# tum-vision/mem

Measured on AMD Instinct MI355X. Metric: pretrain samples/sec (ViT-B, 224^2 event voxels), higher is better.
Workload: dtype bf16

## Files before the change

include/memhip.h:

```cpp
#ifndef MEMHIP_H
#define MEMHIP_H

#include <stddef.h>
#include <stdint.h>

#ifdef __cplusplus
extern "C" {
#endif

#define MEMHIP_ABI_VERSION 10

#define MEMHIP_OK 0
#define MEMHIP_EINVAL (-1)
#define MEMHIP_EWORKSPACE (-2)
#define MEMHIP_ELAUNCH (-3)
#define MEMHIP_EUNSUPPORTED (-4)

typedef void* memhip_stream_t;

int memhip_abi_version(void);
const char* memhip_last_error(void);
const char* memhip_arch(void);
const char* memhip_build_flags(void);
int memhip_set_option(const char* name, int value);
// ... 175 lines not shown
typedef struct memhip_tn_problem {
  const void* A; int64_t lda;
  const void* B; int64_t ldb;
  float* out; int64_t ldo;
  int32_t R, N, K;
  int32_t reserved0;
} memhip_tn_problem_t;
size_t memhip_gemm_bf16_tn_group_workspace(const memhip_tn_problem_t* problems, int count);
int memhip_gemm_bf16_tn_group(const memhip_tn_problem_t* problems, int count, int accumulate, void* workspace,
                              size_t workspace_bytes, memhip_stream_t stream);

#define MEMHIP_TN_128 0
#define MEMHIP_TN_P8_ATOMIC 1
#define MEMHIP_TN_P8_WS 2
#define MEMHIP_TN_P8_GROUP 3
typedef struct memhip_tn_part {
  int32_t problem;
  int32_t tiles, splits, rows_per_split;
  int32_t wg_begin, quad_begin;
  int64_t ws_offset;
} memhip_tn_part_t;
typedef struct memhip_tn_launch {
  int32_t kind;
  int32_t count;
  int32_t grid, reduce_grid;
  int32_t memset_first;
  int32_t use_atomics;
  int64_t ws_bytes;
  memhip_tn_part_t p[4];
} memhip_tn_launch_t;
typedef struct memhip_tn_plan { int32_t count; int32_t reserved0; memhip_tn_launch_t l[4]; } memhip_tn_plan_t;
int memhip_gemm_bf16_tn_plan(const memhip_tn_problem_t* problems, int count, int accumulate, const void* workspace,
                             size_t workspace_bytes, int stream_cus, memhip_tn_plan_t* out_plan);
size_t memhip_gemm_bf16_tn_plan_workspace(const memhip_tn_problem_t* problems, int count, int device_cus);
int memhip_colsum_bf16(const void* in, int64_t ld, int R, int C, float* out, memhip_stream_t stream);
int memhip_colsum_fold(float* ws, int copies, int N, float* out, memhip_stream_t stream);

int memhip_residual_rows(const float* x, int64_t ldx, const int32_t* rows, const void* y, int64_t ldy, const float* gamma,
                         const float* rowkeep, float keep_prob, int R, int D, float* out, int64_t ldo,
                         memhip_stream_t stream);
int memhip_scatter_rows_f32(const float* src, int64_t lds, const int32_t* rows, int R, int D, float* dst, int64_t ldd,
                            memhip_stream_t stream);

int memhip_layernorm_fwd(const float* x, int64_t ldx, const int32_t* row_idx, int R, int D,
                         const float* gamma, const float* beta, float eps, void* y_bf16, int64_t ldy,
                         float* mean, float* rstd, memhip_stream_t stream);
int memhip_layernorm_bwd(const void* dy_bf16, int64_t lddy, const float* x, int64_t ldx,
                         const int32_t* row_idx, int R, int D, const float* gamma, const float* mean,
                         const float* rstd, float* dres, int64_t lddres, int accumulate, float* dgamma,
                         float* dbeta, memhip_stream_t stream);

int memhip_layerscale_grad(const void* W_bf16, int64_t ldw, const float* dW, int64_t lddw, const float* bias,
                           const float* dbias, const float* gamma, int N, int K, float* dgamma,
                           memhip_stream_t stream);

typedef struct memhip_branch {
  const void* y; int64_t ldy;
  const float* gamma;
  const float* rowmask;
  float keep_prob;
  int32_t rows_per_sample;
  void* dy; int64_t lddy;
  float* dgamma; float* dbias;
  const int32_t* out_map;
  const memhip_dropout_t* dropout;
} memhip_branch_t;
typedef struct memhip_branch_bwd_args {
  const float* dx; int64_t lddx;
  int32_t M, D;
  memhip_branch_t branch;
} memhip_branch_bwd_args_t;
int memhip_branch_bwd(const memhip_branch_bwd_args_t* args, memhip_stream_t stream);
typedef struct memhip_ln_bwd_branch_args {
  const void* dy; int64_t lddy;
  const float* x; int64_t ldx;
  int32_t R, D;
  const float* gamma; const float* mean; const float* rstd;
  float* dres; int64_t lddres;
  float* dgamma; float* dbeta;
  const int32_t* in_map;
  memhip_branch_t branch;
} memhip_ln_bwd_branch_args_t;
int memhip_layernorm_bwd_branch(const memhip_ln_bwd_branch_args_t* args, memhip_stream_t stream);

int memhip_embed_bwd(const float* dx, int64_t lddx, const uint8_t* mask, int B, int L, int D,
                     void* dy_bf16, int64_t lddy, float* dcls, float* dmask_token, memhip_stream_t stream);

int memhip_cross_entropy(void* logits_bf16, int64_t ld, const int64_t* labels, int M, int V,
                         float grad_scale, float* row_loss, int32_t* row_correct, int write_grad,
                         float* out2, memhip_stream_t stream);

int memhip_attn_tokens_padded(int T);
int memhip_relpos_gather(const float* table, const int32_t* index , int T, int TP, int heads,
                         float* bias_pad, float* biasT_pad ,
                         memhip_stream_t stream);
int memhip_attn_fwd(const void* qkv, int64_t ldqkv, int B, int T, int D, int heads, const float* table,
                    int window_h, int window_w, void* out, int64_t ldo, float* lse, memhip_stream_t stream);
int memhip_attn_delta(const void* dout, const void* out, int64_t ldo, int64_t rows, int heads, float* delta,
                      memhip_stream_t stream);
typedef struct memhip_attn_bwd_args {
  const void* qkv; int64_t ldqkv;
  const void* dout; int64_t ldo;
  const void* out; int64_t ldout;
  const float* lse;
  float* delta;
  const float* table;
  int32_t window_h, window_w, B, T, D, heads;
  float scale;
  int32_t reserved0;
  void* dqkv; int64_t lddqkv;
  float* dtable; float* dq_bias; float* dv_bias;
  void* ws; int64_t ws_bytes;
} memhip_attn_bwd_args_t;
int memhip_attn_bwd(const memhip_attn_bwd_args_t* args, memhip_stream_t stream);
int64_t memhip_attn_bwd_workspace(int B, int T, int heads, int window_h, int window_w);

#define MEMHIP_ATTN_16 1
#define MEMHIP_ATTN_SMALL 2
#define MEMHIP_ATTN_WIN 3
#define MEMHIP_ATTN_WIN_DS 4
#define MEMHIP_ATTN_STREAM 5
enum { MEMHIP_ATTN_K_STATS_ZERO, MEMHIP_ATTN_K_DELTA, MEMHIP_ATTN_K_FWD, MEMHIP_ATTN_K_BWD_KV, MEMHIP_ATTN_K_BWD_Q,
       MEMHIP_ATTN_K_FWD16, MEMHIP_ATTN_K_BWD16,
       MEMHIP_ATTN_K_WIN_STATS, MEMHIP_ATTN_K_FWD_WIN, MEMHIP_ATTN_K_BWD_KV_WIN, MEMHIP_ATTN_K_BWD_Q_WIN,
       MEMHIP_ATTN_K_BWD_KVS_WIN, MEMHIP_ATTN_K_BWD_QS_WIN,
       MEMHIP_ATTN_K_FWD_STREAM, MEMHIP_ATTN_K_BWD_KV_STREAM, MEMHIP_ATTN_K_BWD_Q_STREAM };
typedef struct memhip_attn_launch {
  int32_t kernel;
  int32_t grid_x, grid_y, grid_z;
  int32_t block;
  int32_t lds;
} memhip_attn_launch_t;
typedef struct memhip_attn_plan {
  int32_t family;
  int32_t n;
  int32_t ww;
  int32_t vb, dt, fd;
  int32_t spb;
  int32_t nwg;
  int32_t groups;
  int32_t nbz, nbq, nbs;
  int32_t qgroups, qs;
  int32_t stream_spb;
  int32_t lds_over;
  int32_t count;
  memhip_attn_launch_t l[5];
} memhip_attn_plan_t;
int memhip_attn_plan_fwd(int B, int T, int D, int heads, int window_h, int window_w, int stream_cus, memhip_attn_plan_t* out);
int memhip_attn_plan_bwd(int B, int T, int D, int heads, int window_h, int window_w, int has_dtable, int has_dv_bias,
                         int has_out, const void* ws, int64_t ws_bytes, int stream_cus, memhip_attn_plan_t* out);

int memhip_f32_gemm_nt(const memhip_gemm_args_t* args, memhip_stream_t stream);
int memhip_f32_transpose(const float* in, int64_t ldin, int R, int C, float* out, int64_t ldout, memhip_stream_t stream);
int memhip_f32_layernorm_fwd(const float* x, int64_t ldx, const int32_t* row_idx, int R, int D, const float* gamma,
                             const float* beta, float eps, float* y, int64_t ldy, float* mean, float* rstd,
                             memhip_stream_t stream);
int memhip_f32_layernorm_bwd(const float* dy, int64_t lddy, const float* x, int64_t ldx, const int32_t* row_idx, int R, int D,
                             const float* gamma, const float* mean, const float* rstd, float* dres, int64_t lddres,
                             int accumulate, float* dgamma, float* dbeta, memhip_stream_t stream);
int memhip_f32_branch_bwd(const float* dx, int64_t lddx, const float* y, int64_t ldy, const float* gamma, const float* rowmask,
                          float keep_prob, int rows_per_sample, int M, int D, float* dy, int64_t lddy, float* dgamma,
                          float* dbias, memhip_stream_t stream);
int memhip_f32_embed_bwd(const float* dx, int64_t lddx, const uint8_t* mask, int B, int L, int D, float* dy, int64_t lddy,
                         float* dcls, float* dmask_token, memhip_stream_t stream);
int memhip_f32_cross_entropy(float* logits, int64_t ld, const int64_t* labels, int M, int V, float grad_scale,
                             float* row_loss, int32_t* row_correct, int write_grad, float* out2, memhip_stream_t stream);
// ... 141 lines not shown
```

mem_amd/csrc/common.h:

```cpp
#pragma once
#include <hip/hip_runtime.h>
#include <cstdarg>
#include <cstdio>
#include <cstdint>
#include <type_traits>
#include "../../include/memhip.h"

namespace memhip {

extern thread_local char g_err[512];

inline int fail(int code, const char* fmt, ...) {
  va_list ap;
  va_start(ap, fmt);
  vsnprintf(g_err, sizeof(g_err), fmt, ap);
  va_end(ap);
  return code;
}

inline int check_launch(const char* what) {
  hipError_t e = hipGetLastError();
  if (e != hipSuccess) return fail(MEMHIP_ELAUNCH, "%s: %s", what, hipGetErrorString(e));
  return MEMHIP_OK;
}

enum { OPT_GEMM_P8, OPT_GEMM256, OPT_GEMM_SPLIT, OPT_GEMM_P8_HALF, OPT_GEMM_P8_MIN_N, OPT_GEMM256_MIN_N, OPT_TN_P8,
       OPT_RASTER_LDS, OPT_ATTN16, OPT_ATTN16_STAGGER, OPT_ATTN16_STAGGER_FWD, OPT_GEMM_STAGGER, OPT_GEMM_PREFETCH, OPT_RESERVE_CUS, OPT_LN_BWD_GRID, OPT_ATTN_WIN, OPT_GEMM_P8_PAIR, OPT_TN_GROUP, OPT_CONV_WAVES, OPT_RASTER_BANDS, OPT_COUNT_ };
int opt(int id);
int usable_cus(hipStream_t s = nullptr);
int max_cus();

inline hipStream_t as_stream(memhip_stream_t s) { return reinterpret_cast<hipStream_t>(s); }

inline int cdiv(long long a, long long b) { return (int)((a + b - 1) / b); }

template <typename F>
int dispatch_bool(bool b, F&& f) { return b ? f(std::true_type{}) : f(std::false_type{}); }

}

#define MEMHIP_REQUIRE(cond, ...) \
  do { if (!(cond)) return memhip::fail(MEMHIP_EINVAL, __VA_ARGS__); } while (0)
#define MEMHIP_HIP(call) \
  do { hipError_t e_ = (call); if (e_ != hipSuccess) \
    return memhip::fail(MEMHIP_ELAUNCH, "%s: %s", #call, hipGetErrorString(e_)); } while (0)
```

mem_amd/csrc/core.cpp:

```cpp
#include "common.h"
#include <atomic>
#include <mutex>
#include <cstring>

namespace memhip {
thread_local char g_err[512] = "";

static std::atomic<int> g_opt[OPT_COUNT_] = {
     {1},  {1},  {1},  {1},  {512},
     {1024},  {1},  {1},  {1},  {40000},  {0},  {0},  {0},
     {0},  {2048},
     {1},
     {1},
     {1},
     {16},
     {0}};
static const char* const g_opt_name[OPT_COUNT_] = {"gemm_p8", "gemm256", "gemm_split", "gemm_p8_half", "gemm_p8_min_n",
                                                   "gemm256_min_n", "tn_p8", "raster_lds", "attn16", "attn16_stagger", "attn16_stagger_fwd", "gemm_stagger", "gemm_prefetch", "reserve_cus", "ln_bwd_grid", "attn_win", "gemm_p8_pair", "tn_group", "conv_waves", "raster_bands"};
int opt(int id) { return g_opt[id].load(std::memory_order_relaxed); }

struct StreamReserve { std::atomic<bool> used{false}; std::atomic<void*> stream{nullptr}; std::atomic<int> cus{0}; };
static StreamReserve g_reserve[32];
static int stream_reserved(hipStream_t s) {
  for (auto& r : g_reserve)
    if (r.used.load(std::memory_order_acquire) && r.stream.load(std::memory_order_relaxed) == (void*)s)
      return r.cus.load(std::memory_order_relaxed);
  return 0;
}

static int device_cu_count() {
  static std::atomic<int> device_cus{0};
  int n = device_cus.load(std::memory_order_relaxed);
  if (!n) {
    int dev = 0;
    hipDeviceProp_t prop;
    if (hipGetDevice(&dev) != hipSuccess || hipGetDeviceProperties(&prop, dev) != hipSuccess) return 0;
    n = prop.multiProcessorCount > 0 ? prop.multiProcessorCount : 256;
    device_cus.store(n, std::memory_order_relaxed);
  }
  return n;
}

int max_cus() { return device_cu_count(); }

int usable_cus(hipStream_t s) {
  const int n = device_cu_count();
  if (!n) return 0;
  int r = opt(OPT_RESERVE_CUS);
  const int rs = stream_reserved(s);
  r = r > rs ? r : rs;
  r = r < 0 ? 0 : (r + 7) / 8 * 8;
  return n - r >= 8 ? n - r : (n >= 8 ? 8 : n);
}
}

extern "C" {
int memhip_abi_version(void) { return MEMHIP_ABI_VERSION; }
const char* memhip_last_error(void) { return memhip::g_err; }
const char* memhip_arch(void) { return "gfx950"; }
#ifndef MEMHIP_BUILD_FLAGS
#define MEMHIP_BUILD_FLAGS ""
#endif
const char* memhip_build_flags(void) { return MEMHIP_BUILD_FLAGS; }

int memhip_stream_reserve_cus(memhip_stream_t stream, int cus) {
  MEMHIP_REQUIRE(cus >= 0, "stream_reserve_cus: negative count");
  using memhip::g_reserve;
  static std::mutex mu;
  std::lock_guard<std::mutex> lock(mu);
  for (auto& r : g_reserve)
    if (r.used.load(std::memory_order_relaxed) && r.stream.load(std::memory_order_relaxed) == stream) {
      r.cus.store(cus, std::memory_order_relaxed);
      if (cus == 0) r.used.store(false, std::memory_order_release);
      return MEMHIP_OK;
    }
  if (cus == 0) return MEMHIP_OK;
  for (auto& r : g_reserve)
    if (!r.used.load(std::memory_order_relaxed)) {
      r.stream.store(stream, std::memory_order_relaxed);
      r.cus.store(cus, std::memory_order_relaxed);
      r.used.store(true, std::memory_order_release);
      return MEMHIP_OK;
    }
  return memhip::fail(MEMHIP_EINVAL, "stream_reserve_cus: more than 32 streams carry a reservation");
}

int memhip_set_option(const char* name, int value) {
  MEMHIP_REQUIRE(name, "set_option: null name");
  for (int i = 0; i < memhip::OPT_COUNT_; ++i)
    if (!strcmp(name, memhip::g_opt_name[i])) {
      if (i == memhip::OPT_LN_BWD_GRID && value < 1)
        return memhip::fail(MEMHIP_EINVAL, "set_option: ln_bwd_grid=%d must be at least 1", value);
      memhip::g_opt[i].store(value, std::memory_order_relaxed);
      return MEMHIP_OK;
    }
  return memhip::fail(MEMHIP_EINVAL, "set_option: unknown option '%s'", name);
}

int memhip_get_option(const char* name, int* value) {
  MEMHIP_REQUIRE(name && value, "get_option: null argument");
  for (int i = 0; i < memhip::OPT_COUNT_; ++i)
// ... 8 lines not shown
```

mem_amd/csrc/gemm_tn.hip:

```cpp
#include "common.h"
#include "gemm_tn_plan.hpp"

namespace {

using namespace memhip;

constexpr int BM = kTn128Tile, BN = kTn128Tile, BR = kTnStageRows;
constexpr int kThreads = 256;
constexpr int kTileBytes = BR * 128 * 2;
constexpr int kStageBytes = 2 * kTileBytes;

typedef __attribute__((ext_vector_type(8))) __bf16 bf16x8;
typedef __attribute__((ext_vector_type(4))) __bf16 bf16x4;
typedef __attribute__((ext_vector_type(4))) short s16x4;
typedef __attribute__((ext_vector_type(4))) float f32x4;

__device__ __attribute__((aligned(256))) unsigned char g_zero_page[256];

__device__ __forceinline__ void glds16(const void* gsrc, void* lds_dst) {
  __builtin_amdgcn_global_load_lds((const __attribute__((address_space(1))) void*)gsrc,
                                   (__attribute__((address_space(3))) void*)lds_dst, 16, 0, 0);
}

__device__ __forceinline__ void stage_rows(const __bf16* __restrict__ src, long long ld, int row0, int rows_valid,
                                           int col0, int cols_valid, char* lds_tile, int wave, int lane) {
#pragma unroll
  for (int j = 0; j < 4; ++j) {
    const int inst = wave * 4 + j;
    const int r = inst * 4 + (lane >> 4);
    const int cpos = lane & 15;
    const int chunk = (((cpos >> 1) ^ (r & 7)) << 1) | (cpos & 1);
    const int grow = row0 + r, gcol = col0 + chunk * 8;
    const void* g = (grow < rows_valid && gcol < cols_valid)
                        ? (const void*)(src + (long long)grow * ld + gcol)
                        : (const void*)(g_zero_page + cpos * 16);
    glds16(g, lds_tile + inst * 1024);
  }
}

__device__ __forceinline__ bf16x8 read_frag_tr(const char* tile, int ks, int col0, int lane) {
  const int g = lane >> 4, q = (lane >> 2) & 3, p = lane & 3;
  const int colb = col0 + 4 * p;
  const int seg = colb >> 4, inb = (colb & 15) * 2;
  const int r0 = ks * 32 + 4 * g + q, r1 = r0 + 16;
  const char* a0 = tile + r0 * 256 + ((seg ^ (r0 & 7)) << 5) + inb;
  const char* a1 = tile + r1 * 256 + ((seg ^ (r1 & 7)) << 5) + inb;
  const s16x4 lo = __builtin_amdgcn_ds_read_tr16_b64_v4i16((__attribute__((address_space(3))) s16x4*)a0);
  const s16x4 hi = __builtin_amdgcn_ds_read_tr16_b64_v4i16((__attribute__((address_space(3))) s16x4*)a1);
  union { struct { s16x4 l, h; } s; bf16x8 v; } u;
  u.s.l = lo;
  u.s.h = hi;
  return u.v;
}

__global__ __launch_bounds__(kThreads, 2) void gemm_tn_kernel(const __bf16* __restrict__ A, long long lda,
                                                              const __bf16* __restrict__ B, long long ldb,
                                                              int R, int N, int K, float* __restrict__ out,
                                                              long long ldo, int splits, int rows_per_split,
                                                              int use_atomics) {
  extern __shared__ __attribute__((aligned(16))) char smem[];
  const int lane = threadIdx.x & 63;
  const int wave = __builtin_amdgcn_readfirstlane(threadIdx.x >> 6);
  const int wr = wave >> 1, wc = wave & 1;
  const int ntk = (K + BN - 1) / BN;
  const int tiles = ((N + BM - 1) / BM) * ntk;
  const int tile = blockIdx.x % tiles, sp = blockIdx.x / tiles;
  const int n0 = (tile / ntk) * BM, k0 = (tile % ntk) * BN;
  const int rbeg = sp * rows_per_split;
  int rend = rbeg + rows_per_split;
  rend = rend < R ? rend : R;
  if (rbeg >= rend) return;
  const int nst = (rend - rbeg + BR - 1) / BR;

  f32x4 acc[4][4];
#pragma unroll
  for (int i = 0; i < 4; ++i)
#pragma unroll
    for (int j = 0; j < 4; ++j) acc[i][j] = f32x4{0.f, 0.f, 0.f, 0.f};

  stage_rows(A, lda, rbeg, rend, n0, N, smem, wave, lane);
  stage_rows(B, ldb, rbeg, rend, k0, K, smem + kTileBytes, wave, lane);
  __syncthreads();
  int cur = 0;
// ... 101 lines not shown
    attr_done = true;
  }
  hipLaunchKernelGGL(gemm_tn_kernel, dim3(l.grid), dim3(kThreads), 2 * kStageBytes, s, (const __bf16*)q.A, (long long)q.lda,
                     (const __bf16*)q.B, (long long)q.ldb, q.R, q.N, q.K, q.out, (long long)q.ldo, l.p[0].splits,
                     l.p[0].rows_per_split, l.use_atomics);
  return check_launch("gemm_bf16_tn");
}

TnPlan plan_now(const memhip_tn_problem_t* pr, int count, int accumulate, const void* ws, size_t ws_bytes, int stream_cus) {
  const TnWorkspace w = {ws != nullptr, ((uintptr_t)ws & 15) == 0, ws_bytes};
  return tn_plan(pr, count, accumulate, w, stream_cus, TnOptions{opt(OPT_TN_P8), opt(OPT_TN_GROUP)});
}

int run(const memhip_tn_problem_t* pr, int count, int accumulate, void* ws, size_t ws_bytes, hipStream_t s) {
  const TnPlan plan = plan_now(pr, count, accumulate, ws, ws_bytes, usable_cus(s));
  for (int i = 0; i < plan.count; ++i) {
    const TnLaunch& l = plan.l[i];
    const memhip_tn_problem_t& q = pr[l.p[0].problem];
    int rc = MEMHIP_OK;
    switch (l.kind) {
      case MEMHIP_TN_128: rc = tn_128_launch(l, q, s); break;
      case MEMHIP_TN_P8_ATOMIC: rc = tn_p8_launch_atomic(l, q, s); break;
      case MEMHIP_TN_P8_WS: rc = tn_p8_launch_ws(l, q, accumulate, (float*)ws, s); break;
      case MEMHIP_TN_P8_GROUP: rc = tn_p8_launch_group(l, pr, accumulate, (float*)ws, s); break;
    }
    if (rc != MEMHIP_OK) return rc;
  }
  return MEMHIP_OK;
}

int validate_group(const memhip_tn_problem_t* problems, int count) {
  MEMHIP_REQUIRE(problems && count >= 1 && count <= kTnGroupMax, "gemm_tn_group: 1..4 problems, got %d", count);
  for (int i = 0; i < count; ++i) {
    const memhip_tn_problem_t& q = problems[i];
    MEMHIP_REQUIRE(q.R >= 0 && q.N > 0 && q.K > 0, "gemm_tn_group[%d]: bad shape R=%d N=%d K=%d", i, q.R, q.N, q.K);
    MEMHIP_REQUIRE(q.R == 0 || (q.A && q.B && q.out), "gemm_tn_group[%d]: null pointer", i);
    MEMHIP_REQUIRE(q.N % 8 == 0 && q.K % 8 == 0 && q.lda % 8 == 0 && q.ldb % 8 == 0 && ((uintptr_t)q.A & 15) == 0 &&
                       ((uintptr_t)q.B & 15) == 0, "gemm_tn_group[%d]: operands must be 16-byte aligned, N/K/ld %% 8 == 0", i);
  }
  return MEMHIP_OK;
}

}

extern "C" size_t memhip_gemm_bf16_tn_workspace(int R, int N, int K) { return tn_workspace_bytes(R, N, K, max_cus()); }

extern "C" int memhip_gemm_bf16_tn(const void* A, int64_t lda, const void* B, int64_t ldb, int R, int N, int K,
                                   float* out, int64_t ldo, int accumulate, void* workspace,
                                   size_t workspace_bytes, memhip_stream_t stream) {
  MEMHIP_REQUIRE(R >= 0 && N > 0 && K > 0, "gemm_tn: bad shape R=%d N=%d K=%d", R, N, K);
  if (R == 0) return MEMHIP_OK;
  MEMHIP_REQUIRE(A && B && out, "gemm_tn: null pointer");
  MEMHIP_REQUIRE(N % 8 == 0 && K % 8 == 0 && lda % 8 == 0 && ldb % 8 == 0 && ((uintptr_t)A & 15) == 0 &&
                     ((uintptr_t)B & 15) == 0, "gemm_tn: operands must be 16-byte aligned, N/K/ld %% 8 == 0");
  const memhip_tn_problem_t q = {A, lda, B, ldb, out, ldo, R, N, K, 0};
  return run(&q, 1, accumulate, workspace, workspace_bytes, as_stream(stream));
}

extern "C" size_t memhip_gemm_bf16_tn_group_workspace(const memhip_tn_problem_t* problems, int count) {
  return memhip_gemm_bf16_tn_plan_workspace(problems, count, max_cus());
}

extern "C" int memhip_gemm_bf16_tn_group(const memhip_tn_problem_t* problems, int count, int accumulate, void* workspace,
                                         size_t workspace_bytes, memhip_stream_t stream) {
  if (const int rc = validate_group(problems, count)) return rc;
  return run(problems, count, accumulate, workspace, workspace_bytes, as_stream(stream));
}

extern "C" int memhip_gemm_bf16_tn_plan(const memhip_tn_problem_t* problems, int count, int accumulate, const void* workspace,
                                        size_t workspace_bytes, int stream_cus, memhip_tn_plan_t* out_plan) {
  MEMHIP_REQUIRE(out_plan, "gemm_tn plan: bad arguments");
  if (const int rc = validate_group(problems, count)) return rc;
  *out_plan = plan_now(problems, count, accumulate, workspace, workspace_bytes, stream_cus >= 0 ? stream_cus : usable_cus());
  return MEMHIP_OK;
}

extern "C" size_t memhip_gemm_bf16_tn_plan_workspace(const memhip_tn_problem_t* problems, int count, int device_cus) {
  if (!problems || count <= 0) return 0;
  return tn_group_workspace_bytes(problems, count, device_cus);
}

namespace {
__global__ __launch_bounds__(256) void colsum_fold_kernel(float* __restrict__ ws, int copies, int N, float* __restrict__ out) {
  const int n = blockIdx.x * 256 + threadIdx.x;
  if (n >= N) return;
  float s = 0.f;
  for (int k = 0; k < copies; ++k) {
    s += ws[(long long)k * N + n];
    ws[(long long)k * N + n] = 0.f;
  }
  out[n] += s;
}
}

extern "C" int memhip_colsum_fold(float* ws, int copies, int N, float* out, memhip_stream_t stream) {
  MEMHIP_REQUIRE(copies >= 1 && N > 0, "colsum_fold: bad shape");
  MEMHIP_REQUIRE(ws && out, "colsum_fold: null pointer");
  hipLaunchKernelGGL(colsum_fold_kernel, dim3(cdiv(N, 256)), dim3(256), 0, as_stream(stream), ws, copies, N, out);
  return check_launch("colsum_fold");
}

extern "C" int memhip_colsum_bf16(const void* in, int64_t ld, int R, int Cc, float* out, memhip_stream_t stream) {
  MEMHIP_REQUIRE(R >= 0 && Cc > 0 && Cc % 8 == 0 && ld % 8 == 0, "colsum: bad shape");
  if (R == 0) return MEMHIP_OK;
  MEMHIP_REQUIRE(in && out, "colsum: null pointer");
  const int chunks = Cc / 8;
  const int tpr = chunks >= 256 ? 256 : chunks;
  const int gx = cdiv(chunks, tpr);
  int gy = 256 / gx;
  if (gy > 128) gy = 128;
  if (gy < 1) gy = 1;
  int rows_per_block = cdiv(R, gy);
  if (rows_per_block < 64) rows_per_block = 64;
  hipLaunchKernelGGL(colsum_kernel, dim3(gx, cdiv(R, rows_per_block)), dim3(256), 0, as_stream(stream),
                     (const __bf16*)in, (long long)ld, R, Cc, rows_per_block, tpr, out);
  return check_launch("colsum_bf16");
}
```

mem_amd/csrc/misc.hip:

```cpp
#include "common.h"

namespace {

using namespace memhip;

typedef __attribute__((ext_vector_type(4))) __bf16 bf16x4;
typedef __attribute__((ext_vector_type(8))) __bf16 bf16x8;

__global__ __launch_bounds__(256) void cast_kernel(const float* __restrict__ in, __bf16* __restrict__ out,
                                                   long long n4) {
  for (long long i = (long long)blockIdx.x * 256 + threadIdx.x; i < n4; i += (long long)gridDim.x * 256) {
    const float4 v = reinterpret_cast<const float4*>(in)[i];
    bf16x4 o;
    o[0] = (__bf16)v.x; o[1] = (__bf16)v.y; o[2] = (__bf16)v.z; o[3] = (__bf16)v.w;
    reinterpret_cast<bf16x4*>(out)[i] = o;
  }
}

template <typename IN>
__global__ __launch_bounds__(256) void transpose_kernel(const IN* __restrict__ in, long long ldin, int R,
                                                        int Cc, __bf16* __restrict__ out, long long ldout,
                                                        int R_pad, float* __restrict__ cs0, int c0b, int c0e,
                                                        float* __restrict__ cs1, int c1b, int c1e) {
  __shared__ __bf16 tile[64][66];
  const int r0 = blockIdx.x * 64, c0 = blockIdx.y * 64;
  const int t = threadIdx.x;
#pragma unroll
  for (int pass = 0; pass < 2; ++pass) {
    const int rl = (t >> 3) + pass * 32, cl = (t & 7) * 8;
    const int r = r0 + rl;
#pragma unroll
    for (int k = 0; k < 8; ++k) {
      const int c = c0 + cl + k;
      __bf16 v = (__bf16)0.f;
      if (r < R && c < Cc) v = (__bf16)(float)in[(long long)r * ldin + c];
      tile[rl][cl + k] = v;
    }
  }
  __syncthreads();
#pragma unroll
  for (int pass = 0; pass < 2; ++pass) {
    const int cl = (t >> 3) + pass * 32, rl = (t & 7) * 8;
    const int c = c0 + cl;
    bf16x8 o;
    float s = 0.f;
#pragma unroll
    for (int k = 0; k < 8; ++k) { o[k] = tile[rl + k][cl]; s += (float)o[k]; }
    if (c < Cc && r0 + rl < R_pad)
      *reinterpret_cast<bf16x8*>(out + (long long)c * ldout + r0 + rl) = o;
    if (cs0 || cs1) {
      s += __shfl_xor(s, 1); s += __shfl_xor(s, 2); s += __shfl_xor(s, 4);
      if ((t & 7) == 0 && c < Cc) {
        if (cs0 && c >= c0b && c < c0e) atomicAdd(cs0 + (c - c0b), s);
        if (cs1 && c >= c1b && c < c1e) atomicAdd(cs1 + (c - c1b), s);
      }
    }
  }
}

struct TransposeDesc { const float* in; long long ldin; long long R; long long Cc; __bf16* out; long long ldout; };
__global__ __launch_bounds__(256) void transpose_cast_batched_kernel(const TransposeDesc* __restrict__ desc,
                                                                     const int* __restrict__ tile_prefix, int n) {
  __shared__ __bf16 tile[64][66];
  int mi = 0;
  while (mi + 1 < n && (int)blockIdx.x >= tile_prefix[mi + 1]) ++mi;
  const TransposeDesc d = desc[mi];
  const int local = blockIdx.x - tile_prefix[mi];
  const int R = (int)d.R, Cc = (int)d.Cc;
  const int tr = (R + 63) / 64;
  const int r0 = (local % tr) * 64, c0 = (local / tr) * 64;
  const int t = threadIdx.x;
  const int R_pad = (int)(d.ldout < (long long)tr * 64 ? d.ldout : (long long)tr * 64);
#pragma unroll
  for (int pass = 0; pass < 2; ++pass) {
    const int rl = (t >> 3) + pass * 32, cl = (t & 7) * 8;
    const int r = r0 + rl, c = c0 + cl;
    const float* src = d.in + (long long)r * d.ldin + c;
    if (r < R && c + 8 <= Cc && ((d.ldin & 3) == 0) && (((unsigned long long)d.in & 15) == 0)) {
      const float4 a = reinterpret_cast<const float4*>(src)[0], b = reinterpret_cast<const float4*>(src)[1];
      const float v[8] = {a.x, a.y, a.z, a.w, b.x, b.y, b.z, b.w};
#pragma unroll
      for (int k = 0; k < 8; ++k) tile[rl][cl + k] = (__bf16)v[k];
    } else {
#pragma unroll
      for (int k = 0; k < 8; ++k) tile[rl][cl + k] = (r < R && c + k < Cc) ? (__bf16)src[k] : (__bf16)0.f;
    }
  }
  __syncthreads();
#pragma unroll
  for (int pass = 0; pass < 2; ++pass) {
    const int cl = (t >> 3) + pass * 32, rl = (t & 7) * 8;
    const int c = c0 + cl;
    bf16x8 o;
#pragma unroll
    for (int k = 0; k < 8; ++k) o[k] = tile[rl + k][cl];
    if (c < Cc && r0 + rl < R_pad) *reinterpret_cast<bf16x8*>(d.out + (long long)c * d.ldout + r0 + rl) = o;
  }
}

__global__ __launch_bounds__(256) void im2col_kernel(const float* __restrict__ x, int B, int C, int H, int W,
                                                     int ph, int pw, __bf16* __restrict__ out) {
  const int gw = W / pw, gh = H / ph;
  const int K = C * ph * pw, K8 = K >> 3;
  const long long total = (long long)B * gh * gw * K8;
  for (long long i = (long long)blockIdx.x * 256 + threadIdx.x; i < total; i += (long long)gridDim.x * 256) {
    const int k8 = (int)(i % K8);
    const long long row = i / K8;
    const int k = k8 * 8;
    const int c = k / (ph * pw), rem = k - c * ph * pw, py = rem / pw, px = rem - py * pw;
    const int gx = (int)(row % gw);
    const long long t = row / gw;
    const int gy = (int)(t % gh), b = (int)(t / gh);
    const float* src = x + (((long long)b * C + c) * H + gy * ph + py) * W + gx * pw + px;
    const float4 a = reinterpret_cast<const float4*>(src)[0], d = reinterpret_cast<const float4*>(src)[1];
    bf16x8 o;
    o[0] = (__bf16)a.x; o[1] = (__bf16)a.y; o[2] = (__bf16)a.z; o[3] = (__bf16)a.w;
    o[4] = (__bf16)d.x; o[5] = (__bf16)d.y; o[6] = (__bf16)d.z; o[7] = (__bf16)d.w;
    reinterpret_cast<bf16x8*>(out)[i] = o;
  }
}

__global__ __launch_bounds__(256) void fill_cls_kernel(float* __restrict__ x, long long ldx, int B, int T, int D,
                                                       const float* __restrict__ cls) {
  const int b = blockIdx.x;
  for (int c = threadIdx.x; c < D; c += 256) x[(long long)b * T * ldx + c] = cls[c];
}

__global__ __launch_bounds__(256) void relpos_gather_kernel(const float* __restrict__ table,
                                                            const int* __restrict__ idx, int T, int TP, int Hh,
                                                            float* __restrict__ bias, float* __restrict__ biasT) {
  const long long total = (long long)Hh * TP * TP;
  for (long long i = (long long)blockIdx.x * 256 + threadIdx.x; i < total; i += (long long)gridDim.x * 256) {
    const int k = (int)(i % TP);
    const long long t = i / TP;
    const int q = (int)(t % TP), h = (int)(t / TP);
    float v = 0.f;
    if (q < T && k < T) v = table[(long long)idx[q * T + k] * Hh + h];
    bias[i] = v;
    if (biasT) biasT[((long long)h * TP + k) * TP + q] = v;
  }
}


__global__ __launch_bounds__(256) void gemv_acc_kernel(const __bf16* __restrict__ W, long long ldw, int N, int K,
                                                       const float* __restrict__ x, float* __restrict__ y,
                                                       float* __restrict__ x_acc, float* __restrict__ zero) {
  const int lane = threadIdx.x & 63;
  const int n = blockIdx.x * 4 + (threadIdx.x >> 6);
  if (n < N) {
    float s = 0.f;
    for (int k = lane * 8; k < K; k += 512) {
      const bf16x8 w = *reinterpret_cast<const bf16x8*>(W + (long long)n * ldw + k);
      const float4 a = *reinterpret_cast<const float4*>(x + k), b = *reinterpret_cast<const float4*>(x + k + 4);
      s += (float)w[0] * a.x + (float)w[1] * a.y + (float)w[2] * a.z + (float)w[3] * a.w + (float)w[4] * b.x +
           (float)w[5] * b.y + (float)w[6] * b.z + (float)w[7] * b.w;
    }
    for (int o = 32; o > 0; o >>= 1) s += __shfl_xor(s, o);
    if (lane == 0) y[n] += s;
  }
  if (blockIdx.x == 0) {
    for (int k = threadIdx.x; k < K; k += blockDim.x) {
      if (x_acc) x_acc[k] += x[k];
      if (zero) zero[k] = 0.f;
    }
  }
}

}

extern "C" int memhip_cast_f32_bf16(const float* in, void* out, int64_t n, memhip_stream_t stream) {
  MEMHIP_REQUIRE(n >= 0 && n % 4 == 0, "cast: n must be a multiple of 4");
  if (n == 0) return MEMHIP_OK;
  MEMHIP_REQUIRE(in && out, "cast: null pointer");
  const long long n4 = n / 4;
  int blocks = (int)((n4 + 255) / 256);
  if (blocks > 4096) blocks = 4096;
  hipLaunchKernelGGL(cast_kernel, dim3(blocks), dim3(256), 0, as_stream(stream), in, (__bf16*)out, n4);
  return check_launch("cast_f32_bf16");
}

extern "C" int memhip_transpose_cast_f32_bf16(const float* in, int64_t ldin, int R, int Cc, void* out,
                                              int64_t ldout, memhip_stream_t stream) {
  MEMHIP_REQUIRE(R > 0 && Cc > 0 && in && out, "transpose_cast: bad arguments");
  MEMHIP_REQUIRE(ldout % 8 == 0 && ldout >= R, "transpose_cast: ldout");
  const int R_pad = (int)(ldout < (int64_t)cdiv(R, 64) * 64 ? ldout : (int64_t)cdiv(R, 64) * 64);
  hipLaunchKernelGGL(transpose_kernel<float>, dim3(cdiv(R, 64), cdiv(Cc, 64)), dim3(256), 0, as_stream(stream), in,
                     (long long)ldin, R, Cc, (__bf16*)out, (long long)ldout, R_pad, (float*)nullptr, 0, 0,
                     (float*)nullptr, 0, 0);
  return check_launch("transpose_cast");
}

extern "C" int memhip_transpose_cast_batched(const void* desc, const int32_t* tile_prefix, int n, int total_tiles,
                                             memhip_stream_t stream) {
  MEMHIP_REQUIRE(n >= 0 && total_tiles >= 0, "transpose_cast_batched: bad arguments");
  if (n == 0 || total_tiles == 0) return MEMHIP_OK;
  MEMHIP_REQUIRE(desc && tile_prefix, "transpose_cast_batched: null pointer");
  static_assert(sizeof(TransposeDesc) == 48, "descriptor = 6 x 8 bytes");
  hipLaunchKernelGGL(transpose_cast_batched_kernel, dim3(total_tiles), dim3(256), 0, as_stream(stream),
                     (const TransposeDesc*)desc, tile_prefix, n);
  return check_launch("transpose_cast_batched");
}

extern "C" int memhip_transpose_bf16(const void* in, int64_t ldin, int R, int Cc, void* out, int64_t ldout,
                                     int R_pad, float* colsum0, int c0_begin, int c0_end, float* colsum1,
                                     int c1_begin, int c1_end, memhip_stream_t stream) {
  MEMHIP_REQUIRE(R >= 0 && Cc > 0 && in && out, "transpose: bad arguments");
  MEMHIP_REQUIRE(R_pad >= R && R_pad % 64 == 0 && ldout >= R_pad && ldout % 8 == 0,
                 "transpose: R_pad=%d must be a multiple of 64 and <= ldout", R_pad);
  if (R_pad == 0) return MEMHIP_OK;
  hipLaunchKernelGGL(transpose_kernel<__bf16>, dim3(R_pad / 64, cdiv(Cc, 64)), dim3(256), 0, as_stream(stream),
                     (const __bf16*)in, (long long)ldin, R, Cc, (__bf16*)out, (long long)ldout, R_pad, colsum0,
                     c0_begin, c0_end, colsum1, c1_begin, c1_end);
  return check_launch("transpose_bf16");
}

extern "C" int memhip_im2col_bf16(const float* x, int B, int C, int H, int W, int ph, int pw, void* out,
                                  memhip_stream_t stream) {
  MEMHIP_REQUIRE(B >= 0 && C > 0 && ph > 0 && pw > 0 && H % ph == 0 && W % pw == 0, "im2col: bad shape");
  MEMHIP_REQUIRE(pw % 8 == 0 && W % 4 == 0, "im2col: patch width must be a multiple of 8");
  if (B == 0) return MEMHIP_OK;
  MEMHIP_REQUIRE(x && out, "im2col: null pointer");
  const long long total = (long long)B * (H / ph) * (W / pw) * (C * ph * pw / 8);
  int blocks = (int)((total + 255) / 256);
  if (blocks > 8192) blocks = 8192;
  hipLaunchKernelGGL(im2col_kernel, dim3(blocks), dim3(256), 0, as_stream(stream), x, B, C, H, W, ph, pw,
                     (__bf16*)out);
  return check_launch("im2col");
}

__global__ __launch_bounds__(256) void copy_samples_kernel(const float* __restrict__ src, float* __restrict__ dst,
                                                           const int* __restrict__ ids, long long n_per_sample) {
  const long long base = (long long)ids[blockIdx.y] * n_per_sample;
  const float4* s4 = reinterpret_cast<const float4*>(src + base);
  float4* d4 = reinterpret_cast<float4*>(dst + base);
  for (long long i = (long long)blockIdx.x * 256 + threadIdx.x; i < n_per_sample / 4; i += (long long)gridDim.x * 256) d4[i] = s4[i];
}

extern "C" int memhip_copy_samples_f32(const float* src, float* dst, const int32_t* ids, int n, int64_t n_per_sample,
                                       memhip_stream_t stream) {
  MEMHIP_REQUIRE(n >= 0 && n_per_sample > 0 && n_per_sample % 4 == 0, "copy_samples: bad shape");
  if (n == 0) return MEMHIP_OK;
  MEMHIP_REQUIRE(src && dst && ids, "copy_samples: null pointer");
  int gx = (int)((n_per_sample / 4 + 255) / 256);
  if (gx > 64) gx = 64;
  hipLaunchKernelGGL(copy_samples_kernel, dim3(gx, n), dim3(256), 0, as_stream(stream), src, dst, (const int*)ids,
                     (long long)n_per_sample);
  return check_launch("copy_samples");
}

__global__ __launch_bounds__(256) void zero_kernel(uint4* __restrict__ p, long long n16) {
  const long long step = (long long)gridDim.x * 256;
  for (long long i = (long long)blockIdx.x * 256 + threadIdx.x; i < n16; i += step) p[i] = uint4{0u, 0u, 0u, 0u};
}
__global__ __launch_bounds__(256) void zero_ranges_kernel(char* __restrict__ base, const long long* __restrict__ ranges, int n) {
  const long long step = (long long)gridDim.x * 256;
  for (int r = 0; r < n; ++r) {
    uint4* p = reinterpret_cast<uint4*>(base + ranges[2 * r]);
    const long long n16 = ranges[2 * r + 1] >> 4;
    for (long long i = (long long)blockIdx.x * 256 + threadIdx.x; i < n16; i += step) p[i] = uint4{0u, 0u, 0u, 0u};
  }
}

extern "C" int memhip_zero(void* p, int64_t bytes, memhip_stream_t stream) {
  MEMHIP_REQUIRE(bytes >= 0 && bytes % 16 == 0 && ((uintptr_t)p & 15) == 0, "zero: pointer and size must be multiples of 16 bytes");
  if (bytes == 0) return MEMHIP_OK;
  MEMHIP_REQUIRE(p, "zero: null pointer");
  long long g = (bytes / 16 + 255) / 256;
  if (g > 2048) g = 2048;
  hipLaunchKernelGGL(zero_kernel, dim3((unsigned)g), dim3(256), 0, as_stream(stream), (uint4*)p, (long long)(bytes / 16));
  return check_launch("zero");
}

extern "C" int memhip_zero_ranges(void* base, const int64_t* ranges, int n, int64_t total_bytes, memhip_stream_t stream) {
  MEMHIP_REQUIRE(n >= 0 && total_bytes >= 0, "zero_ranges: bad count");
  if (n == 0 || total_bytes == 0) return MEMHIP_OK;
  MEMHIP_REQUIRE(base && ranges && ((uintptr_t)base & 15) == 0, "zero_ranges: null / unaligned pointer");
  long long g = (total_bytes / 16 + 255) / 256;
  if (g > 1024) g = 1024;
  if (g < 1) g = 1;
  hipLaunchKernelGGL(zero_ranges_kernel, dim3((unsigned)g), dim3(256), 0, as_stream(stream), (char*)base, (const long long*)ranges, n);
  return check_launch("zero_ranges");
}

__global__ __launch_bounds__(256) void residual_rows_kernel(const float* __restrict__ x, long long ldx, const int* __restrict__ rows,
                                                            const __bf16* __restrict__ y, long long ldy,
                                                            const float* __restrict__ gamma, const float* __restrict__ rowkeep,
                                                            float keep_prob, int R, int D, float* __restrict__ out, long long ldo) {
  const int per_row = D / 4;
  const float kp = rowkeep ? keep_prob : 1.0f;
  const float rk = __frcp_rn(kp);
  for (long long i = (long long)blockIdx.x * 256 + threadIdx.x; i < (long long)R * per_row; i += (long long)gridDim.x * 256) {
    const int r = (int)(i / per_row), c = (int)(i % per_row) * 4;
    const float rm = rowkeep ? rowkeep[r] : 1.0f;
    const float4 xv = *reinterpret_cast<const float4*>(x + (long long)rows[r] * ldx + c);
    const float xs[4] = {xv.x, xv.y, xv.z, xv.w};
    float o[4];
#pragma unroll
    for (int k = 0; k < 4; ++k) {
      float br = __fmul_rn(gamma ? gamma[c + k] : 1.0f, (float)y[(long long)r * ldy + c + k]);
      const float q0 = br * rk;
      const float q = fmaf(fmaf(-q0, kp, br), rk, q0);
      br = __fmul_rn(q, rm);
      o[k] = __fadd_rn(xs[k], br);
    }
    *reinterpret_cast<float4*>(out + (long long)r * ldo + c) = float4{o[0], o[1], o[2], o[3]};
  }
}

__global__ __launch_bounds__(256) void scatter_rows_kernel(const float* __restrict__ src, long long lds, const int* __restrict__ rows,
                                                           int R, int D, float* __restrict__ dst, long long ldd) {
  const int per_row = D / 4;
  for (long long i = (long long)blockIdx.x * 256 + threadIdx.x; i < (long long)R * per_row; i += (long long)gridDim.x * 256) {
    const int r = (int)(i / per_row), c = (int)(i % per_row) * 4;
    *reinterpret_cast<float4*>(dst + (long long)rows[r] * ldd + c) = *reinterpret_cast<const float4*>(src + (long long)r * lds + c);
  }
}

extern "C" int memhip_residual_rows(const float* x, int64_t ldx, const int32_t* rows, const void* y, int64_t ldy, const float* gamma,
                                    const float* rowkeep, float keep_prob, int R, int D, float* out, int64_t ldo,
                                    memhip_stream_t stream) {
  MEMHIP_REQUIRE(R >= 0 && D > 0 && D % 4 == 0 && ldx % 4 == 0 && ldo % 4 == 0, "residual_rows: bad shape");
  if (R == 0) return MEMHIP_OK;
  MEMHIP_REQUIRE(x && rows && y && out, "residual_rows: null pointer");
  long long n = (long long)R * (D / 4);
  int grid = (int)((n + 255) / 256);
  if (grid > 2048) grid = 2048;
  hipLaunchKernelGGL(residual_rows_kernel, dim3(grid), dim3(256), 0, as_stream(stream), x, (long long)ldx, (const int*)rows,
                     (const __bf16*)y, (long long)ldy, gamma, rowkeep, keep_prob, R, D, out, (long long)ldo);
  return check_launch("residual_rows");
}

extern "C" int memhip_scatter_rows_f32(const float* src, int64_t lds, const int32_t* rows, int R, int D, float* dst, int64_t ldd,
                                       memhip_stream_t stream) {
  MEMHIP_REQUIRE(R >= 0 && D > 0 && D % 4 == 0 && lds % 4 == 0 && ldd % 4 == 0, "scatter_rows: bad shape");
  if (R == 0) return MEMHIP_OK;
  MEMHIP_REQUIRE(src && rows && dst, "scatter_rows: null pointer");
  long long n = (long long)R * (D / 4);
  int grid = (int)((n + 255) / 256);
  if (grid > 2048) grid = 2048;
  hipLaunchKernelGGL(scatter_rows_kernel, dim3(grid), dim3(256), 0, as_stream(stream), src, (long long)lds, (const int*)rows, R, D,
                     dst, (long long)ldd);
  return check_launch("scatter_rows");
}

extern "C" int memhip_fill_cls(float* x, int64_t ldx, int B, int T, int D, const float* cls,
                               memhip_stream_t stream) {
  MEMHIP_REQUIRE(B >= 0 && T > 0 && D > 0, "fill_cls: bad shape");
  if (B == 0) return MEMHIP_OK;
  MEMHIP_REQUIRE(x && cls, "fill_cls: null pointer");
  hipLaunchKernelGGL(fill_cls_kernel, dim3(B), dim3(256), 0, as_stream(stream), x, (long long)ldx, B, T, D, cls);
  return check_launch("fill_cls");
}

extern "C" int memhip_relpos_gather(const float* table, const int32_t* index, int T, int TP, int heads,
                                    float* bias, float* biasT, memhip_stream_t stream) {
  MEMHIP_REQUIRE(T > 0 && TP >= T && heads > 0 && table && index && bias, "relpos_gather: bad arguments");
  const long long total = (long long)heads * TP * TP;
  int blocks = (int)((total + 255) / 256);
  if (blocks > 4096) blocks = 4096;
  hipLaunchKernelGGL(relpos_gather_kernel, dim3(blocks), dim3(256), 0, as_stream(stream), table, index, T, TP,
                     heads, bias, biasT);
  return check_launch("relpos_gather");
}

extern "C" int memhip_gemv_bf16_acc(const void* W, int64_t ldw, int N, int K, const float* x, float* y, float* x_acc,
                                    float* zero, memhip_stream_t stream) {
  MEMHIP_REQUIRE(N >= 0 && K >= 0 && K % 8 == 0 && ldw % 8 == 0, "gemv: K and ldw must be multiples of 8");
  if (N == 0 || K == 0) return MEMHIP_OK;
  MEMHIP_REQUIRE(W && x && y, "gemv: null pointer");
  hipLaunchKernelGGL(gemv_acc_kernel, dim3((N + 3) / 4), dim3(256), 0, as_stream(stream), (const __bf16*)W,
                     (long long)ldw, N, K, x, y, x_acc, zero);
  return check_launch("gemv_bf16_acc");
}
```

mem_amd/csrc/rowops.hip:

```cpp
#include "common.h"
#include "dropout.hpp"

#include <type_traits>

namespace {

using namespace memhip;

typedef __attribute__((ext_vector_type(4))) __bf16 bf16x4;
typedef __attribute__((ext_vector_type(8))) __bf16 bf16x8;

__device__ __forceinline__ float wsum(float v) {
  for (int o = 32; o > 0; o >>= 1) v += __shfl_xor(v, o);
  return v;
}
__device__ __forceinline__ float wmax(float v) {
  for (int o = 32; o > 0; o >>= 1) v = fmaxf(v, __shfl_xor(v, o));
  return v;
}

__device__ __forceinline__ float div_newton(float a, float b, float r) {
  const float q0 = a * r;
  return fmaf(fmaf(-q0, b, a), r, q0);
}

constexpr int kMaxChunks = 8;

template <bool FULL>
__device__ __forceinline__ bool chunk_ok(int i, int nch) {
  if constexpr (FULL) return true;
  else return i < nch;
}

__device__ __forceinline__ int wave_id() { return __builtin_amdgcn_readfirstlane((int)(threadIdx.x >> 6)); }

struct RowWalk {
  int r, smp, off, stride, q, rem, rps;
  __device__ __forceinline__ RowWalk(int r0, int stride_, int rps_) : r(r0), stride(stride_), rps(rps_) {
    smp = r0 / rps; off = r0 - smp * rps;
    q = stride / rps; rem = stride - q * rps;
  }
  __device__ __forceinline__ void next() {
    r += stride; smp += q; off += rem;
    if (off >= rps) { off -= rps; ++smp; }
  }
};

__device__ __forceinline__ void stage_columns(float4* dst, const float* a, const float* b, int nch) {
  for (int i = threadIdx.x; i < nch; i += 256) {
    dst[i] = reinterpret_cast<const float4*>(a)[i];
    dst[nch + i] = b ? reinterpret_cast<const float4*>(b)[i] : float4{1.f, 1.f, 1.f, 1.f};
  }
  __syncthreads();
}

__device__ __forceinline__ int opaque(int v) {
  asm volatile("" : "+v"(v));
  return v;
}

__device__ __forceinline__ float mul_rn(float a, float b) {
#pragma clang fp contract(off)
  return a * b;
}
__device__ __forceinline__ float sub_rn(float a, float b) {
#pragma clang fp contract(off)
  return a - b;
}
__device__ __forceinline__ float ln_dx(float gg, float xh, float m1, float m2) { return __fmaf_rn(-xh, m2, sub_rn(gg, m1)); }
__device__ __forceinline__ float sq2(float a, float b) { return __fmaf_rn(a, a, mul_rn(b, b)); }

template <int NCH, bool FULL>
__global__ __launch_bounds__(256) void ln_fwd_kernel(const float* __restrict__ x, long long ldx,
                                                     const int* __restrict__ row_idx, int R, int D,
                                                     const float* __restrict__ gamma,
                                                     const float* __restrict__ beta, float eps,
                                                     __bf16* __restrict__ y, long long ldy,
                                                     float* __restrict__ mean, float* __restrict__ rstd) {
  extern __shared__ float red[];
  const int lane = threadIdx.x & 63;
  const int r0 = blockIdx.x * 4 + wave_id();
  const bool act = r0 < R;
  const int r = act ? r0 : R - 1;
  const long long src = row_idx ? row_idx[r] : r;
  const float4* xr = reinterpret_cast<const float4*>(x + src * ldx);
  const int nch = D >> 2;
  float4 v[NCH];
#pragma unroll
  for (int c = 0; c < NCH; ++c) {
    const int i = lane + c * 64;
    if (chunk_ok<FULL>(i, nch)) v[c] = xr[i];
  }
  constexpr int NST = (64 * NCH + 255) / 256;
  float4 sg[NST], sb[NST];
#pragma unroll
  for (int k = 0; k < NST; ++k) {
    const int i = min((int)threadIdx.x + k * 256, nch - 1);
    sg[k] = reinterpret_cast<const float4*>(gamma)[i];
    sb[k] = reinterpret_cast<const float4*>(beta)[i];
  }
  __builtin_amdgcn_sched_barrier(0);
  float s = 0.f;
#pragma unroll
  for (int c = 0; c < NCH; ++c)
    if (chunk_ok<FULL>(lane + c * 64, nch)) s += (v[c].x + v[c].y) + (v[c].z + v[c].w);
  const float mu = wsum(s) / (float)D;
  float4* lgb = reinterpret_cast<float4*>(red);
#pragma unroll
  for (int k = 0; k < NST; ++k) {
    const int i = min((int)threadIdx.x + k * 256, nch - 1);
    lgb[i] = sg[k];
    lgb[nch + i] = sb[k];
  }
  float q = 0.f;
#pragma unroll
  for (int c = 0; c < NCH; ++c) {
    if (chunk_ok<FULL>(lane + c * 64, nch)) {
      const float a = v[c].x - mu, b = v[c].y - mu, cc = v[c].z - mu, d = v[c].w - mu;
      q += sq2(a, b) + sq2(cc, d);
    }
  }
  const float var = wsum(q) / (float)D;
  const float rs = 1.0f / sqrtf(var + eps);
  __syncthreads();
  if (!act) return;
  if (lane == 0) { mean[r] = mu; rstd[r] = rs; }
  bf16x4* yr = reinterpret_cast<bf16x4*>(y + (long long)r * ldy);
#pragma unroll
  for (int c = 0; c < NCH; ++c) {
    const int i = lane + c * 64;
    if (chunk_ok<FULL>(i, nch)) {
      const float4 g = lgb[i], b = lgb[nch + i];
      bf16x4 o;
      o[0] = (__bf16)__fmaf_rn(mul_rn(v[c].x - mu, rs), g.x, b.x);
      o[1] = (__bf16)__fmaf_rn(mul_rn(v[c].y - mu, rs), g.y, b.y);
      o[2] = (__bf16)__fmaf_rn(mul_rn(v[c].z - mu, rs), g.z, b.z);
      o[3] = (__bf16)__fmaf_rn(mul_rn(v[c].w - mu, rs), g.w, b.w);
      yr[i] = o;
    }
  }
}

__device__ __forceinline__ void vm_drain() { __builtin_amdgcn_s_waitcnt(0x0F70); }

template <int NCH, bool FULL, bool ACC>
__global__ __launch_bounds__(256) void ln_bwd_kernel(const __bf16* __restrict__ dy, long long lddy,
                                                     const float* __restrict__ x, long long ldx,
                                                     const int* __restrict__ row_idx, int R, int D,
                                                     const float* __restrict__ gamma,
                                                     const float* __restrict__ mean,
                                                     const float* __restrict__ rstd,
                                                     float* __restrict__ dres, long long lddres,
                                                     float* __restrict__ dgamma, float* __restrict__ dbeta) {
  extern __shared__ float red[];
  const int lane = threadIdx.x & 63, wave = wave_id();
  const int nch = D >> 2;
  float4 ag[NCH], ab[NCH];
#pragma unroll
  for (int c = 0; c < NCH; ++c) {
    ag[c] = float4{0, 0, 0, 0};
    ab[c] = float4{0, 0, 0, 0};
  }
  const int rstride = gridDim.x * 4;
  float4 xn[NCH], prev[NCH];
  bf16x4 dn[NCH];
  auto issue = [&](int r, long long src, int lane) {
    const float4* xr = reinterpret_cast<const float4*>(x + src * ldx);
    const bf16x4* dyr = reinterpret_cast<const bf16x4*>(dy + (long long)r * lddy);
#pragma unroll
    for (int c = 0; c < NCH; ++c) {
      const int i = lane + c * 64;
      if (chunk_ok<FULL>(i, nch)) {
        xn[c] = xr[i];
        dn[c] = dyr[i];
      }
    }
  };
  auto issue_prev = [&](long long src, int lane) {
    const float4* o = reinterpret_cast<const float4*>(dres + src * lddres);
#pragma unroll
    for (int c = 0; c < NCH; ++c) {
      const int i = lane + c * 64;
      if (chunk_ok<FULL>(i, nch)) prev[c] = o[i];
    }
  };
  int r = blockIdx.x * 4 + wave;
  long long src = 0;
  float mu = 0.f, rs = 0.f;
  if (r < R) {
    src = row_idx ? row_idx[r] : r;
    issue(r, src, lane);
    if constexpr (ACC) issue_prev(src, lane);
    mu = mean[r]; rs = rstd[r];
  }
  float4* lg = reinterpret_cast<float4*>(red);
  for (int i = threadIdx.x; i < nch; i += 256) lg[i] = reinterpret_cast<const float4*>(gamma)[i];
  __syncthreads();
  int r1 = r + rstride;
  long long src1 = 0;
  if (r1 < R) src1 = row_idx ? row_idx[r1] : r1;
  int r2 = r1 + rstride;
  vm_drain();
  while (r < R) {
    float4 xh[NCH], gg[NCH];
    float s1 = 0.f, s2 = 0.f;
    const int ol = opaque(lane);
    const float4* lgl = lg + ol;
#pragma unroll
    for (int c = 0; c < NCH; ++c) {
      const int i = lane + c * 64;
      if (chunk_ok<FULL>(i, nch)) {
        const float4 xv = xn[c];
        const bf16x4 d4 = dn[c];
        const float4 g = lgl[c * 64];
        const float d0 = (float)d4[0], d1 = (float)d4[1], d2 = (float)d4[2], d3 = (float)d4[3];
        xh[c] = float4{mul_rn(xv.x - mu, rs), mul_rn(xv.y - mu, rs), mul_rn(xv.z - mu, rs), mul_rn(xv.w - mu, rs)};
        gg[c] = float4{mul_rn(d0, g.x), mul_rn(d1, g.y), mul_rn(d2, g.z), mul_rn(d3, g.w)};
        s1 += (gg[c].x + gg[c].y) + (gg[c].z + gg[c].w);
        s2 += (mul_rn(gg[c].x, xh[c].x) + mul_rn(gg[c].y, xh[c].y)) + (mul_rn(gg[c].z, xh[c].z) + mul_rn(gg[c].w, xh[c].w));
        ag[c].x += d0 * xh[c].x; ag[c].y += d1 * xh[c].y; ag[c].z += d2 * xh[c].z; ag[c].w += d3 * xh[c].w;
        ab[c].x += d0; ab[c].y += d1; ab[c].z += d2; ab[c].w += d3;
      }
    }
// ... 99 lines not shown
  int m, mo, smp;
  float k = 1.f;
  find(m, mo, smp);
  if (m < M) {
    issue(m, lane);
    if (rowmask) k = rowmask[smp];
  }
  float4* lg = reinterpret_cast<float4*>(red);
  for (int i = threadIdx.x; i < nch; i += 256)
    lg[i] = gamma ? reinterpret_cast<const float4*>(gamma)[i] : float4{1.f, 1.f, 1.f, 1.f};
  __syncthreads();
  int m1, mo1, smp1;
  find(m1, mo1, smp1);
  vm_drain();
  while (m < M) {
    const int ol = opaque(lane);
    float4 dv[NCH];
    bf16x4 yv[HAS_Y ? NCH : 1];
#pragma unroll
    for (int c = 0; c < NCH; ++c) {
      if (chunk_ok<FULL>(lane + c * 64, nch)) {
        dv[c] = dn[c];
        if constexpr (HAS_Y) yv[c] = yn[c];
      }
    }
    float k1 = 1.f;
    const bool next = m1 < M;
    issue(next ? m1 : m, ol);
    if (next && rowmask) k1 = rowmask[smp1];
    int m2, mo2, smp2;
    find(m2, mo2, smp2);
    bf16x4* orow = reinterpret_cast<bf16x4*>(dyo + (long long)mo * lddy);
    const float4* lgl = lg + ol;
#pragma unroll
    for (int c = 0; c < NCH; ++c) {
      const int i = ol + c * 64;
      if (chunk_ok<FULL>(i, nch)) {
        float4 d = dv[c];
        if (rowmask || out_map) {
          d.x = div_newton(d.x * k, keep, rk); d.y = div_newton(d.y * k, keep, rk);
          d.z = div_newton(d.z * k, keep, rk); d.w = div_newton(d.w * k, keep, rk);
        }
        if constexpr (sizeof...(Drop) > 0) {
          const DropParams dp = (drop, ...);
          const unsigned kb = dropout_keep8(dp, (unsigned)(dp.row0 + m), (unsigned)(i >> 1)) >> ((i & 1) * 4);
          d.x = __fmul_rn(d.x, dropout_mul(dp, kb, 0)); d.y = __fmul_rn(d.y, dropout_mul(dp, kb, 1));
          d.z = __fmul_rn(d.z, dropout_mul(dp, kb, 2)); d.w = __fmul_rn(d.w, dropout_mul(dp, kb, 3));
        }
        if constexpr (HAS_Y) {
          const bf16x4 yy = yv[c];
          ag[c].x += d.x * (float)yy[0]; ag[c].y += d.y * (float)yy[1];
          ag[c].z += d.z * (float)yy[2]; ag[c].w += d.w * (float)yy[3];
        }
        const float4 g = lgl[c * 64];
        bf16x4 o;
        o[0] = (__bf16)(d.x * g.x); o[1] = (__bf16)(d.y * g.y);
        o[2] = (__bf16)(d.z * g.z); o[3] = (__bf16)(d.w * g.w);
        orow[i] = o;
        ab[c].x += (float)o[0]; ab[c].y += (float)o[1]; ab[c].z += (float)o[2]; ab[c].w += (float)o[3];
      }
    }
    m = m1; mo = mo1; k = k1;
    m1 = m2; mo1 = mo2; smp1 = smp2;
  }
  __syncthreads();
  float4* rg = reinterpret_cast<float4*>(red + (size_t)wave * 2 * D);
  float4* rb = reinterpret_cast<float4*>(red + (size_t)wave * 2 * D + D);
#pragma unroll
  for (int c = 0; c < NCH; ++c) {
    const int i = lane + c * 64;
    if (chunk_ok<FULL>(i, nch)) { rg[i] = ag[c]; rb[i] = ab[c]; }
  }
  __syncthreads();
  for (int n = threadIdx.x; n < D; n += 256) {
    float a = 0.f, b = 0.f;
#pragma unroll
    for (int w2 = 0; w2 < 4; ++w2) { a += red[(size_t)w2 * 2 * D + n]; b += red[(size_t)w2 * 2 * D + D + n]; }
    if (dgamma) atomicAdd(dgamma + n, a);
    if (dbias) atomicAdd(dbias + n, b);
  }
}

template <int NCH, bool FULL, bool HAS_Y, class... Drop>
__global__ __launch_bounds__(256) void ln_bwd_branch_kernel(const __bf16* __restrict__ dy, long long lddy,
                                                            const float* __restrict__ x, long long ldx, int R, int D,
                                                            const float* __restrict__ gamma,
                                                            const float* __restrict__ mean, const float* __restrict__ rstd,
                                                            float* __restrict__ dres, long long lddres,
                                                            float* __restrict__ dgamma, float* __restrict__ dbeta,
                                                            const __bf16* __restrict__ yb, long long ldyb,
                                                            const float* __restrict__ gb, const float* __restrict__ rowmask,
                                                            float keep, int rps, __bf16* __restrict__ dyo, long long lddyo,
                                                            float* __restrict__ dgb, float* __restrict__ dbiasb,
                                                            const int* __restrict__ in_map, const int* __restrict__ out_map,
                                                            Drop... drop) {
  extern __shared__ float red[];
  const int lane = threadIdx.x & 63, wave = wave_id();
  const int nch = D >> 2;
  float4 ag[NCH], ab[NCH], bg[HAS_Y ? NCH : 1], bb[NCH];
  const float rk = __frcp_rn(keep);
#pragma unroll
  for (int c = 0; c < NCH; ++c) {
    ag[c] = ab[c] = bb[c] = float4{0, 0, 0, 0};
    if (HAS_Y) bg[c] = float4{0, 0, 0, 0};
  }
  float4 xn[NCH], prev[NCH];
  bf16x4 dn[NCH], yn[HAS_Y ? NCH : 1];
  auto issue_x = [&](int r, int rin, int lane) {
    const float4* xr = reinterpret_cast<const float4*>(x + (long long)r * ldx);
    const bf16x4* dyr = reinterpret_cast<const bf16x4*>(dy + (long long)rin * lddy);
#pragma unroll
    for (int c = 0; c < NCH; ++c) {
      const int i = lane + c * 64;
      if (chunk_ok<FULL>(i, nch)) {
        xn[c] = xr[i];
        dn[c] = dyr[i];
      }
    }
  };
  auto issue_y = [&](int r, int lane) {
    if constexpr (HAS_Y) {
#pragma unroll
      for (int c = 0; c < NCH; ++c) {
        const int i = lane + c * 64;
        if (chunk_ok<FULL>(i, nch)) yn[c] = reinterpret_cast<const bf16x4*>(yb + (long long)r * ldyb)[i];
      }
    }
  };
  auto issue_prev = [&](int r, int lane) {
    const float4* o = reinterpret_cast<const float4*>(dres + (long long)r * lddres);
#pragma unroll
    for (int c = 0; c < NCH; ++c) {
      const int i = lane + c * 64;
      if (chunk_ok<FULL>(i, nch)) prev[c] = o[i];
    }
  };
  const int row0 = blockIdx.x * 4 + wave, rstride = gridDim.x * 4;
  auto resolve = [&](const RowWalk& t, int& rin, int& rout) {
    rin = rout = t.r;
    if (in_map) { const int ci = in_map[t.smp]; rin = ci < 0 ? -1 : ci * t.rps + t.off; }
    if (out_map) { const int co = out_map[t.smp]; rout = co < 0 ? -1 : co * t.rps + t.off; }
  };
  int r, rin, rout;
  float mu = 0.f, rs = 0.f, km = 1.f;
  float4 xh[NCH], gg[NCH];
  bf16x4 yv[HAS_Y ? NCH : 1];
  float s1, s2;
  float4 *lg = reinterpret_cast<float4*>(red), *lgb = lg + nch;
  auto reduce_row = [&](bool has_in, int ol) {
    s1 = s2 = 0.f;
    const float4* lgl = lg + ol;
    if (has_in) {
#pragma unroll
      for (int c = 0; c < NCH; ++c) {
        if (chunk_ok<FULL>(lane + c * 64, nch)) {
          if constexpr (HAS_Y) yv[c] = yn[c];
          const float4 xv = xn[c];
          const bf16x4 d4 = dn[c];
          const float d0 = (float)d4[0], d1 = (float)d4[1], d2 = (float)d4[2], d3 = (float)d4[3];
          xh[c] = float4{mul_rn(xv.x - mu, rs), mul_rn(xv.y - mu, rs), mul_rn(xv.z - mu, rs), mul_rn(xv.w - mu, rs)};
          const float4 gmc = lgl[c * 64];
          gg[c] = float4{mul_rn(d0, gmc.x), mul_rn(d1, gmc.y), mul_rn(d2, gmc.z), mul_rn(d3, gmc.w)};
          s1 += (gg[c].x + gg[c].y) + (gg[c].z + gg[c].w);
          s2 += (mul_rn(gg[c].x, xh[c].x) + mul_rn(gg[c].y, xh[c].y)) + (mul_rn(gg[c].z, xh[c].z) + mul_rn(gg[c].w, xh[c].w));
          ag[c].x += d0 * xh[c].x; ag[c].y += d1 * xh[c].y; ag[c].z += d2 * xh[c].z; ag[c].w += d3 * xh[c].w;
          ab[c].x += d0; ab[c].y += d1; ab[c].z += d2; ab[c].w += d3;
        }
      }
    } else {
#pragma unroll
      for (int c = 0; c < NCH; ++c) {
        if (chunk_ok<FULL>(lane + c * 64, nch)) {
          if constexpr (HAS_Y) yv[c] = yn[c];
          xh[c] = gg[c] = float4{0.f, 0.f, 0.f, 0.f};
        }
      }
    }
  };
  auto store_row = [&](bool has_in, bool has_out, int ol) {
    const float m1 = wsum(s1) / (float)D, m2 = wsum(s2) / (float)D;
    float4* o = reinterpret_cast<float4*>(dres + (long long)r * lddres);
    bf16x4* orow = reinterpret_cast<bf16x4*>(dyo + (long long)(has_out ? rout : 0) * lddyo);
    const float4* lgbl = lgb + ol;
#pragma unroll
    for (int c = 0; c < NCH; ++c) {
      const int i = ol + c * 64;
      if (chunk_ok<FULL>(i, nch)) {
        float4 d{__fmaf_rn(rs, ln_dx(gg[c].x, xh[c].x, m1, m2), prev[c].x), __fmaf_rn(rs, ln_dx(gg[c].y, xh[c].y, m1, m2), prev[c].y),
                 __fmaf_rn(rs, ln_dx(gg[c].z, xh[c].z, m1, m2), prev[c].z), __fmaf_rn(rs, ln_dx(gg[c].w, xh[c].w, m1, m2), prev[c].w)};
        if (has_in) o[i] = d;
        if (!has_out) continue;
        if (rowmask || out_map) {
          d.x = div_newton(d.x * km, keep, rk); d.y = div_newton(d.y * km, keep, rk);
          d.z = div_newton(d.z * km, keep, rk); d.w = div_newton(d.w * km, keep, rk);
        }
        if constexpr (sizeof...(Drop) > 0) {
          const DropParams dp = (drop, ...);
          const unsigned kb = dropout_keep8(dp, (unsigned)(dp.row0 + r), (unsigned)(i >> 1)) >> ((i & 1) * 4);
          d.x = __fmul_rn(d.x, dropout_mul(dp, kb, 0)); d.y = __fmul_rn(d.y, dropout_mul(dp, kb, 1));
          d.z = __fmul_rn(d.z, dropout_mul(dp, kb, 2)); d.w = __fmul_rn(d.w, dropout_mul(dp, kb, 3));
        }
        if constexpr (HAS_Y) {
          bg[c].x += d.x * (float)yv[c][0]; bg[c].y += d.y * (float)yv[c][1];
          bg[c].z += d.z * (float)yv[c][2]; bg[c].w += d.w * (float)yv[c][3];
        }
        const float4 gbc = lgbl[c * 64];
        bf16x4 q;
        q[0] = (__bf16)(d.x * gbc.x); q[1] = (__bf16)(d.y * gbc.y);
        q[2] = (__bf16)(d.z * gbc.z); q[3] = (__bf16)(d.w * gbc.w);
        orow[i] = q;
        bb[c].x += (float)q[0]; bb[c].y += (float)q[1]; bb[c].z += (float)q[2]; bb[c].w += (float)q[3];
      }
    }
  };
  RowWalk w(row0, rstride, rps);
  auto find = [&](int& fr, int& frin, int& frout, int& fsmp) {
    for (;;) {
      fr = w.r; fsmp = w.smp; frin = frout = -1;
      if (fr >= R) return;
      resolve(w, frin, frout);
      w.next();
      if ((frin | frout) >= 0) return;
    }
  };
  int smp;
  find(r, rin, rout, smp);
  if (r < R) {
    issue_x(r, rin, lane); issue_y(r, lane); issue_prev(r, lane);
    mu = mean[rin]; rs = rstd[rin];
    if (rowmask) km = rowmask[smp];
  }
  stage_columns(lg, gamma, gb, nch);
  int r1, rin1, rout1, smp1;
  find(r1, rin1, rout1, smp1);
  vm_drain();
  while (r < R) {
    const int ol = opaque(lane);
    reduce_row(true, ol);
    float mu1 = 0.f, rs1 = 0.f, km1 = 1.f;
    const bool next = r1 < R;
    const int rl = next ? r1 : r, rinl = next ? rin1 : rin;
    issue_x(rl, rinl, ol); issue_y(rl, ol);
    if (next) {
      mu1 = mean[rin1]; rs1 = rstd[rin1];
      if (rowmask) km1 = rowmask[smp1];
    }
    int r2, rin2, rout2, smp2;
    find(r2, rin2, rout2, smp2);
    store_row(true, true, ol);
    __builtin_amdgcn_sched_barrier(0);
    issue_prev(rl, ol);
    r = r1; rin = rin1; rout = rout1; mu = mu1; rs = rs1; km = km1;
    r1 = r2; rin1 = rin2; rout1 = rout2; smp1 = smp2;
  }
  if (in_map || out_map) {
    for (RowWalk v(row0, rstride, rps); v.r < R; v.next()) {
      resolve(v, rin, rout);
      if ((rin >= 0) == (rout >= 0)) continue;
      r = v.r;
      const int ol = opaque(lane);
      issue_prev(r, ol); issue_y(r, ol);
      mu = rs = 0.f;
      if (rin >= 0) {
        issue_x(r, rin, ol);
        mu = mean[rin]; rs = rstd[rin];
      }
      km = rowmask ? rowmask[v.smp] : 1.f;
      reduce_row(rin >= 0, ol);
      store_row(rin >= 0, rout >= 0, ol);
    }
  }
  __syncthreads();
  float4* r0 = reinterpret_cast<float4*>(red + (size_t)wave * 4 * D);
#pragma unroll
  for (int c = 0; c < NCH; ++c) {
    const int i = lane + c * 64;
    if (chunk_ok<FULL>(i, nch)) { r0[i] = ag[c]; r0[nch + i] = ab[c]; r0[2 * nch + i] = HAS_Y ? bg[HAS_Y ? c : 0] : float4{0, 0, 0, 0}; r0[3 * nch + i] = bb[c]; }
  }
  __syncthreads();
  for (int n = threadIdx.x; n < D; n += 256) {
    float a = 0.f, b = 0.f, c2 = 0.f, d2 = 0.f;
#pragma unroll
    for (int w2 = 0; w2 < 4; ++w2) {
      const float* rw = red + (size_t)w2 * 4 * D;
      a += rw[n]; b += rw[D + n]; c2 += rw[2 * D + n]; d2 += rw[3 * D + n];
    }
    atomicAdd(dgamma + n, a);
    atomicAdd(dbeta + n, b);
    if (dgb) atomicAdd(dgb + n, c2);
    if (dbiasb) atomicAdd(dbiasb + n, d2);
  }
}


__global__ __launch_bounds__(256) void layerscale_grad_kernel(const __bf16* __restrict__ W, long long ldw,
                                                              const float* __restrict__ dW, long long lddw,
                                                              const float* __restrict__ b, const float* __restrict__ db,
                                                              const float* __restrict__ gamma, int N, int K,
                                                              float* __restrict__ dgamma) {
  __shared__ float red[4][4];
  const int lane = threadIdx.x & 63, wave = threadIdx.x >> 6;
  const int n0 = blockIdx.x * 4;
  float s[4] = {0.f, 0.f, 0.f, 0.f};
  for (int k0 = 0; k0 < K; k0 += 4096) {
#pragma unroll
    for (int c = 0; c < 4; ++c) {
      const int n = n0 + c < N ? n0 + c : N - 1;
      const __bf16* wr = W + (long long)n * ldw;
      const float* gr = dW + (long long)n * lddw;
#pragma unroll
      for (int u = 0; u < 4; ++u) {
        const int k = k0 + u * 1024 + (int)threadIdx.x * 4;
        if (k < K) {
          const bf16x4 w = *reinterpret_cast<const bf16x4*>(wr + k);
          const float4 g = *reinterpret_cast<const float4*>(gr + k);
          s[c] += (float)w[0] * g.x + (float)w[1] * g.y + (float)w[2] * g.z + (float)w[3] * g.w;
        }
      }
    }
  }
#pragma unroll
  for (int c = 0; c < 4; ++c) {
    const float t = wsum(s[c]);
    if (lane == 0) red[wave][c] = t;
  }
  __syncthreads();
  if (threadIdx.x < 4 && n0 + (int)threadIdx.x < N) {
    const int n = n0 + threadIdx.x;
    float t = (red[0][threadIdx.x] + red[1][threadIdx.x]) + (red[2][threadIdx.x] + red[3][threadIdx.x]);
    if (b && db) t += b[n] * db[n];
    const float g = gamma[n];
    dgamma[n] = g != 0.f ? t / g : 0.f;
  }
}

__global__ __launch_bounds__(256) void embed_bwd_kernel(const float* __restrict__ dx, long long lddx,
                                                        const unsigned char* __restrict__ mask, int B,
                                                        int L, int D, __bf16* __restrict__ dy,
                                                        long long lddy, float* __restrict__ dcls,
                                                        float* __restrict__ dmask) {
  constexpr int U = 7;
  for (int c = threadIdx.x * 4; c < D; c += 256 * 4) {
    float4 cls{0, 0, 0, 0}, am{0, 0, 0, 0};
    for (int b = blockIdx.x; b < B; b += gridDim.x) {
      const float* row0 = dx + (long long)b * (L + 1) * lddx + c;
      const float4 dc = *reinterpret_cast<const float4*>(row0);
      cls.x += dc.x; cls.y += dc.y; cls.z += dc.z; cls.w += dc.w;
      const unsigned char* mk = mask + (long long)b * L;
      __bf16* out = dy + (long long)b * L * lddy + c;
      int p = 0;
      for (; p + U <= L; p += U) {
        float4 d[U];
#pragma unroll
        for (int u = 0; u < U; ++u) d[u] = *reinterpret_cast<const float4*>(row0 + (long long)(1 + p + u) * lddx);
#pragma unroll
        for (int u = 0; u < U; ++u) {
          const float w = (float)mk[p + u], q = 1.0f - w;
          am.x += d[u].x * w; am.y += d[u].y * w; am.z += d[u].z * w; am.w += d[u].w * w;
          bf16x4 o;
          o[0] = (__bf16)(d[u].x * q); o[1] = (__bf16)(d[u].y * q); o[2] = (__bf16)(d[u].z * q); o[3] = (__bf16)(d[u].w * q);
          *reinterpret_cast<bf16x4*>(out + (long long)(p + u) * lddy) = o;
        }
      }
      for (; p < L; ++p) {
        const float4 d = *reinterpret_cast<const float4*>(row0 + (long long)(1 + p) * lddx);
        const float w = (float)mk[p], q = 1.0f - w;
        am.x += d.x * w; am.y += d.y * w; am.z += d.z * w; am.w += d.w * w;
        bf16x4 o;
        o[0] = (__bf16)(d.x * q); o[1] = (__bf16)(d.y * q); o[2] = (__bf16)(d.z * q); o[3] = (__bf16)(d.w * q);
        *reinterpret_cast<bf16x4*>(out + (long long)p * lddy) = o;
      }
    }
    atomicAdd(dcls + c, cls.x); atomicAdd(dcls + c + 1, cls.y);
    atomicAdd(dcls + c + 2, cls.z); atomicAdd(dcls + c + 3, cls.w);
    atomicAdd(dmask + c, am.x); atomicAdd(dmask + c + 1, am.y);
    atomicAdd(dmask + c + 2, am.z); atomicAdd(dmask + c + 3, am.w);
// ... 41 lines not shown
  __syncthreads();
  mx = bc[0];
  amax = si[0];
  float s = 0.f;
#pragma unroll
  for (int c = 0; c < VPT; ++c) {
    const int i = tid + c * 256;
    if (i < nch) {
#pragma unroll
      for (int k = 0; k < 8; ++k) { v[c][k] = __expf(v[c][k] - mx); s += v[c][k]; }
    }
  }
  s = wsum(s);
  __syncthreads();
  if (lane == 0) sm[wave] = s;
  __syncthreads();
  if (tid == 0) bc[1] = (sm[0] + sm[1]) + (sm[2] + sm[3]);
  __syncthreads();
  const float sum = bc[1];
  const long long lab = labels[r];
  if (tid == 0) {
    const bool lab_ok = lab >= 0 && lab < V;
    const float zl = lab_ok ? (float)logits[(long long)r * ld + lab] : __builtin_nanf("");
    row_loss[r] = (mx + __logf(sum)) - zl;
    row_correct[r] = (amax == (int)lab) ? 1 : 0;
  }
  if (write_grad) {
    const float inv = 1.0f / sum;
    __syncthreads();
#pragma unroll
    for (int c = 0; c < VPT; ++c) {
      const int i = tid + c * 256;
      if (i < nch) {
        bf16x8 o;
#pragma unroll
        for (int k = 0; k < 8; ++k) {
          float p = v[c][k] * inv;
          if ((long long)(i * 8 + k) == lab) p -= 1.0f;
          o[k] = (__bf16)(p * grad_scale);
        }
        row[i] = o;
      }
    }
  }
}

__global__ __launch_bounds__(256) void ce_reduce_kernel(const float* __restrict__ row_loss,
                                                        const int* __restrict__ row_correct, int M,
                                                        float* __restrict__ out) {
  __shared__ double sd[4];
  __shared__ int sc[4];
  double s = 0.0;
  int c = 0;
  for (int i = threadIdx.x; i < M; i += 256) { s += (double)row_loss[i]; c += row_correct[i]; }
  for (int o = 32; o > 0; o >>= 1) { s += __shfl_xor(s, o); c += __shfl_xor(c, o); }
  if ((threadIdx.x & 63) == 0) { sd[threadIdx.x >> 6] = s; sc[threadIdx.x >> 6] = c; }
  __syncthreads();
  if (threadIdx.x == 0) {
    const double t = (sd[0] + sd[1]) + (sd[2] + sd[3]);
    const int k = sc[0] + sc[1] + sc[2] + sc[3];
    out[0] = (float)(t / (double)M);
    out[1] = (float)k / (float)M;
  }
}

}

template <int MAXN, class F>
void dispatch_width(int D, F&& f) {
  const int nch = cdiv(D / 4, 64);
  const bool full = D % 256 == 0;
  const auto either = [&](auto N) { if (full) f(N, std::true_type{}); else f(N, std::false_type{}); };
  if (nch <= 1) either(std::integral_constant<int, 1>{});
  else if (nch <= 2) either(std::integral_constant<int, 2>{});
  else if (nch <= 3) either(std::integral_constant<int, 3>{});
  else if (MAXN == 4 || nch <= 4) either(std::integral_constant<int, 4>{});
  else if constexpr (MAXN == 8) {
    if (nch == 5 && full) f(std::integral_constant<int, 5>{}, std::true_type{});
    else if (nch == 8 && full) f(std::integral_constant<int, 8>{}, std::true_type{});
    else f(std::integral_constant<int, 8>{}, std::false_type{});
  }
}

extern "C" int memhip_layernorm_fwd(const float* x, int64_t ldx, const int32_t* row_idx, int R, int D,
                                    const float* gamma, const float* beta, float eps, void* y,
                                    int64_t ldy, float* mean, float* rstd, memhip_stream_t stream) {
  MEMHIP_REQUIRE(R >= 0 && D > 0 && D % 4 == 0 && D <= 64 * 4 * kMaxChunks, "layernorm_fwd: bad R=%d D=%d", R, D);
  if (R == 0) return MEMHIP_OK;
  MEMHIP_REQUIRE(x && gamma && beta && y && mean && rstd, "layernorm_fwd: null pointer");
  MEMHIP_REQUIRE(ldx % 4 == 0 && ldy % 4 == 0, "layernorm_fwd: ld must be a multiple of 4");
  dispatch_width<kMaxChunks>(D, [&](auto N, auto F) {
    hipLaunchKernelGGL((ln_fwd_kernel<decltype(N)::value, decltype(F)::value>), dim3(cdiv(R, 4)), dim3(256), (size_t)2 * D * sizeof(float), as_stream(stream),
                       x, (long long)ldx, row_idx, R, D, gamma, beta, eps, (__bf16*)y, (long long)ldy, mean, rstd);
  });
  return check_launch("layernorm_fwd");
}

extern "C" int memhip_layernorm_bwd(const void* dy, int64_t lddy, const float* x, int64_t ldx,
                                    const int32_t* row_idx, int R, int D, const float* gamma,
                                    const float* mean, const float* rstd, float* dres, int64_t lddres,
                                    int accumulate, float* dgamma, float* dbeta, memhip_stream_t stream) {
  MEMHIP_REQUIRE(R >= 0 && D > 0 && D % 4 == 0 && D <= 64 * 4 * kMaxChunks, "layernorm_bwd: bad R=%d D=%d", R, D);
  if (R == 0) return MEMHIP_OK;
  MEMHIP_REQUIRE(dy && x && gamma && mean && rstd && dres && dgamma && dbeta, "layernorm_bwd: null pointer");
  MEMHIP_REQUIRE(ldx % 4 == 0 && lddy % 4 == 0 && lddres % 4 == 0, "layernorm_bwd: ld must be a multiple of 4");
  int grid = cdiv(R, 4);
  const int cap = opt(OPT_LN_BWD_GRID) * 4 / 3;
  if (grid > cap) grid = cap;
  dispatch_width<kMaxChunks>(D, [&](auto N, auto F) {
    dispatch_bool(accumulate, [&](auto A) {
      hipLaunchKernelGGL((ln_bwd_kernel<decltype(N)::value, decltype(F)::value, decltype(A)::value>), dim3(grid), dim3(256), (size_t)8 * D * sizeof(float), as_stream(stream),
                         (const __bf16*)dy, (long long)lddy, x, (long long)ldx, row_idx, R, D, gamma, mean, rstd, dres,
                         (long long)lddres, dgamma, dbeta);
      return 0;
    });
  });
  return check_launch("layernorm_bwd");
}

template <int NCH, bool FULL, bool HAS_Y, class... Drop>
static void branch_bwd_launch(const memhip_branch_bwd_args_t& a, int grid, memhip_stream_t stream, Drop... drop) {
  const memhip_branch_t& b = a.branch;
  hipLaunchKernelGGL((branch_bwd_kernel<NCH, FULL, HAS_Y, Drop...>), dim3(grid), dim3(256), (size_t)8 * a.D * sizeof(float),
                     as_stream(stream), a.dx, (long long)a.lddx, (const __bf16*)b.y, (long long)b.ldy, b.gamma, b.rowmask,
                     b.keep_prob, b.rows_per_sample > 0 ? b.rows_per_sample : 1, a.M, a.D, (__bf16*)b.dy, (long long)b.lddy,
                     b.dgamma, b.dbias, (const int*)b.out_map, drop...);
}

extern "C" int memhip_branch_bwd(const memhip_branch_bwd_args_t* args, memhip_stream_t stream) {
  MEMHIP_REQUIRE(args, "branch_bwd: null args");
  const memhip_branch_t& b = args->branch;
  const int M = args->M, D = args->D;
  MEMHIP_REQUIRE(M >= 0 && D > 0 && D % 4 == 0, "branch_bwd: bad M=%d D=%d", M, D);
  MEMHIP_REQUIRE(!b.dropout || D % 8 == 0, "branch_bwd_drop: D=%d must be a multiple of 8", D);
  MEMHIP_REQUIRE(!b.out_map || (!b.rowmask && !b.y && b.rows_per_sample > 0), "branch_bwd: out_map excludes rowmask / y");
  if (M == 0) return MEMHIP_OK;
  MEMHIP_REQUIRE(args->dx && b.dy, "branch_bwd: null pointer");
  MEMHIP_REQUIRE(b.y || !b.dgamma, "branch_bwd: dgamma needs y (or use memhip_layerscale_grad)");
  MEMHIP_REQUIRE(args->lddx % 4 == 0 && b.ldy % 4 == 0 && b.lddy % 4 == 0, "branch_bwd: ld must be a multiple of 4");
  MEMHIP_REQUIRE(D <= 64 * 4 * kBrMaxChunks, "branch_bwd: D=%d too large", D);
  int grid = cdiv(M, 4);
  if (grid > 1024) grid = 1024;
  dispatch_width<kBrMaxChunks>(D, [&](auto N, auto F) {
    dispatch_bool(b.y, [&](auto Y) {
      if (b.dropout) branch_bwd_launch<decltype(N)::value, decltype(F)::value, decltype(Y)::value>(*args, grid, stream, drop_params(*b.dropout));
      else branch_bwd_launch<decltype(N)::value, decltype(F)::value, decltype(Y)::value>(*args, grid, stream);
      return 0;
    });
  });
  return check_launch("branch_bwd");
}

extern "C" int memhip_embed_bwd(const float* dx, int64_t lddx, const uint8_t* mask, int B, int L, int D,
                                void* dy, int64_t lddy, float* dcls, float* dmask_token,
                                memhip_stream_t stream) {
  MEMHIP_REQUIRE(B >= 0 && L > 0 && D > 0 && D % 4 == 0, "embed_bwd: bad shape");
  if (B == 0) return MEMHIP_OK;
  MEMHIP_REQUIRE(dx && mask && dy && dcls && dmask_token, "embed_bwd: null pointer");
  hipLaunchKernelGGL(embed_bwd_kernel, dim3(B < 128 ? B : 128), dim3(256), 0, as_stream(stream), dx, (long long)lddx, mask, B,
                     L, D, (__bf16*)dy, (long long)lddy, dcls, dmask_token);
  return check_launch("embed_bwd");
}

extern "C" int memhip_cross_entropy(void* logits, int64_t ld, const int64_t* labels, int M, int V,
                                    float grad_scale, float* row_loss, int32_t* row_correct,
                                    int write_grad, float* out2, memhip_stream_t stream) {
  MEMHIP_REQUIRE(M >= 0 && V > 0 && V % 8 == 0 && V <= 256 * 8 * 8, "cross_entropy: V=%d unsupported", V);
  if (M == 0) return MEMHIP_OK;
  MEMHIP_REQUIRE(logits && labels && row_loss && row_correct && out2, "cross_entropy: null pointer");
  MEMHIP_REQUIRE(ld % 8 == 0, "cross_entropy: ld must be a multiple of 8");
  hipStream_t s = as_stream(stream);
  const int nch = V / 8, vpt = cdiv(nch, 256);
  __bf16* lg = (__bf16*)logits;
  const long long* lab = (const long long*)labels;
#define CE_LAUNCH(N) hipLaunchKernelGGL(ce_kernel<N>, dim3(M), dim3(256), 0, s, lg, (long long)ld, lab, V, \
                                        grad_scale, row_loss, row_correct, write_grad)
  if (vpt <= 1) CE_LAUNCH(1);
  else if (vpt <= 2) CE_LAUNCH(2);
  else if (vpt <= 4) CE_LAUNCH(4);
  else CE_LAUNCH(8);
#undef CE_LAUNCH
  hipLaunchKernelGGL(ce_reduce_kernel, dim3(1), dim3(256), 0, s, row_loss, row_correct, M, out2);
  return check_launch("cross_entropy");
}

template <int NCH, bool FULL, bool HAS_Y, class... Drop>
static void ln_bwd_branch_launch(const memhip_ln_bwd_branch_args_t& a, int grid, memhip_stream_t stream, Drop... drop) {
  const memhip_branch_t& b = a.branch;
  hipLaunchKernelGGL((ln_bwd_branch_kernel<NCH, FULL, HAS_Y, Drop...>), dim3(grid), dim3(256), (size_t)16 * a.D * sizeof(float),
                     as_stream(stream), (const __bf16*)a.dy, (long long)a.lddy, a.x, (long long)a.ldx, a.R, a.D, a.gamma, a.mean,
                     a.rstd, a.dres, (long long)a.lddres, a.dgamma, a.dbeta, (const __bf16*)b.y, (long long)b.ldy, b.gamma,
                     b.rowmask, b.keep_prob, b.rows_per_sample > 0 ? b.rows_per_sample : 1, (__bf16*)b.dy, (long long)b.lddy,
                     b.dgamma, b.dbias, (const int*)a.in_map, (const int*)b.out_map, drop...);
}

extern "C" int memhip_layernorm_bwd_branch(const memhip_ln_bwd_branch_args_t* args, memhip_stream_t stream) {
  MEMHIP_REQUIRE(args, "layernorm_bwd_branch: null args");
  const memhip_ln_bwd_branch_args_t& a = *args;
  const memhip_branch_t& b = a.branch;
  const int R = a.R, D = a.D;
  MEMHIP_REQUIRE(R >= 0 && D > 0 && D % 4 == 0 && D <= 64 * 4 * 4, "layernorm_bwd_branch: D=%d unsupported (<= 1024)", D);
  MEMHIP_REQUIRE(!b.dropout || D % 8 == 0, "layernorm_bwd_branch_drop: D=%d must be a multiple of 8", D);
  MEMHIP_REQUIRE(!(a.in_map || b.out_map) || (!b.rowmask && !b.y && b.rows_per_sample > 0),
                 "layernorm_bwd_branch: sample maps exclude rowmask / y_branch");
  if (R == 0) return MEMHIP_OK;
  MEMHIP_REQUIRE(a.dy && a.x && a.gamma && a.mean && a.rstd && a.dres && a.dgamma && a.dbeta && b.dy,
                 "layernorm_bwd_branch: null pointer");
  MEMHIP_REQUIRE(b.y || !b.dgamma, "layernorm_bwd_branch: dgamma_branch needs y_branch");
  MEMHIP_REQUIRE(a.ldx % 4 == 0 && a.lddy % 4 == 0 && a.lddres % 4 == 0 && b.ldy % 4 == 0 && b.lddy % 4 == 0,
                 "layernorm_bwd_branch: ld must be a multiple of 4");
  int grid = cdiv(R, 4);
  int cap = opt(OPT_LN_BWD_GRID);
  if (D > 768 && cap > 512) cap = 512;
  if (grid > cap) grid = cap;
  dispatch_width<4>(D, [&](auto N, auto F) {
    if (b.dropout)
      dispatch_bool(b.y, [&](auto Y) {
        ln_bwd_branch_launch<decltype(N)::value, decltype(F)::value, decltype(Y)::value>(a, grid, stream, drop_params(*b.dropout));
        return 0;
      });
    else
      dispatch_bool(b.y, [&](auto Y) {
        ln_bwd_branch_launch<decltype(N)::value, decltype(F)::value, decltype(Y)::value>(a, grid, stream);
        return 0;
      });
  });
  return check_launch("layernorm_bwd_branch");
}

extern "C" int memhip_layerscale_grad(const void* W_bf16, int64_t ldw, const float* dW, int64_t lddw, const float* bias,
                                      const float* dbias, const float* gamma, int N, int K, float* dgamma,
                                      memhip_stream_t stream) {
  MEMHIP_REQUIRE(N >= 0 && K > 0 && K % 4 == 0 && ldw % 4 == 0 && lddw % 4 == 0, "layerscale_grad: bad shape");
  if (N == 0) return MEMHIP_OK;
  MEMHIP_REQUIRE(W_bf16 && dW && gamma && dgamma && (!bias == !dbias), "layerscale_grad: null pointer");
  hipLaunchKernelGGL(layerscale_grad_kernel, dim3((N + 3) / 4), dim3(256), 0, as_stream(stream), (const __bf16*)W_bf16,
                     (long long)ldw, dW, (long long)lddw, bias, dbias, gamma, N, K, dgamma);
  return check_launch("layerscale_grad");
}
```

mem_amd/ops.py:

```python
import ctypes as C

import torch

from ._lib import check, declare, f32, f64, i32, i64, lib, ptr, stream_ptr, sz, vp

EPI_BIAS_BF16, EPI_BIAS_GELU, EPI_RESIDUAL, EPI_DGELU, EPI_F32, EPI_PATCH_EMBED, EPI_BIAS_GELU_DG, EPI_MUL_AUX = range(8)
EPI_RESIDUAL_DROP = 8


class Dropout(C.Structure):
    _fields_ = [("key0", C.c_uint32), ("key1", C.c_uint32), ("site", C.c_uint32), ("thr", C.c_uint32), ("scale", f32),
                ("row0", i32)]


def dropout_params(key0, key1, site, p, row0=0):
    assert 0.0 <= p < 1.0, p
    return Dropout(int(key0) & 0xFFFFFFFF, int(key1) & 0xFFFFFFFF, int(site), int(round(p * 65536)), 1.0 / (1.0 - p), int(row0))


def with_row0(d, row0):
    return None if d is None else Dropout(d.key0, d.key1, d.site, d.thr, d.scale, int(row0))


class GemmArgs(C.Structure):
    _fields_ = [("A", vp), ("B", vp), ("lda", i64), ("ldb", i64),
                ("M", i32), ("N", i32), ("K", i32), ("epilogue", i32),
                ("out0", vp), ("ldo0", i64), ("out1", vp), ("ldo1", i64),
                ("bias", vp), ("vec1", vp), ("resid", vp), ("ldr", i64),
                ("aux", vp), ("ldaux", i64), ("rowmask", vp), ("keep_prob", f32),
                ("colscale", f32), ("colscale_n", i32), ("rows_per_sample", i32), ("accumulate", i32),
                ("colsum", vp), ("sample_map", vp), ("colsum_copies", i32), ("reserved0", i32),
                ("dropout", vp)]


class Branch(C.Structure):
    _fields_ = [("y", vp), ("ldy", i64), ("gamma", vp), ("rowmask", vp), ("keep_prob", f32), ("rows_per_sample", i32),
                ("dy", vp), ("lddy", i64), ("dgamma", vp), ("dbias", vp), ("out_map", vp), ("dropout", vp)]


class BranchBwdArgs(C.Structure):
    _fields_ = [("dx", vp), ("lddx", i64), ("M", i32), ("D", i32), ("branch", Branch)]


class LnBwdBranchArgs(C.Structure):
    _fields_ = [("dy", vp), ("lddy", i64), ("x", vp), ("ldx", i64), ("R", i32), ("D", i32), ("gamma", vp), ("mean", vp),
                ("rstd", vp), ("dres", vp), ("lddres", i64), ("dgamma", vp), ("dbeta", vp), ("in_map", vp), ("branch", Branch)]


class AttnBwdArgs(C.Structure):
    _fields_ = [("qkv", vp), ("ldqkv", i64), ("dout", vp), ("ldo", i64), ("out", vp), ("ldout", i64), ("lse", vp), ("delta", vp),
                ("table", vp), ("window_h", i32), ("window_w", i32), ("B", i32), ("T", i32), ("D", i32), ("heads", i32),
                ("scale", f32), ("reserved0", i32), ("dqkv", vp), ("lddqkv", i64), ("dtable", vp), ("dq_bias", vp),
                ("dv_bias", vp), ("ws", vp), ("ws_bytes", i64)]


class NtLaunch(C.Structure):
    _fields_ = [(n, i32) for n in ("kind", "row0", "rows", "tail_rows", "guard", "copy", "grid", "tail_grid")]


class NtPlan(C.Structure):
    _fields_ = [("count", i32), ("l", NtLaunch * 2)]


declare({"memhip_gemm_bf16_nt": (i32, [C.POINTER(GemmArgs), vp]),
         "memhip_branch_bwd": (i32, [C.POINTER(BranchBwdArgs), vp]),
         "memhip_layernorm_bwd_branch": (i32, [C.POINTER(LnBwdBranchArgs), vp]),
         "memhip_attn_bwd": (i32, [C.POINTER(AttnBwdArgs), vp]),
         "memhip_gemm_bf16_nt_plan": (i32, [C.POINTER(GemmArgs), i32, i32, C.POINTER(NtPlan)])})


def _p(t):
    return None if t is None else t.data_ptr()


GEMM_TIMER = None
GEMM_EVENT_POOL = []


def _timer_event():
    return GEMM_EVENT_POOL.pop() if GEMM_EVENT_POOL else torch.cuda.Event(enable_timing=True)


def _timed(code, flops, fn):
    if GEMM_TIMER is None:
        fn()
        return
    e0, e1 = _timer_event(), _timer_event()
    e0.record()
    fn()
    e1.record()
    GEMM_TIMER.append((e0, e1, flops, code))


def gemm_args(A, B, M, N, K, epi, out0=None, out1=None, bias=None, vec1=None, resid=None, aux=None,
              rowmask=None, keep_prob=1.0, colscale=1.0, colscale_n=0, rows_per_sample=1, accumulate=False, colsum=None,
              lda=None, ldb=None, ldo0=None, ldo1=None, ldr=None, ldaux=None, sample_map=None, colsum_copies=0, dropout=None):
    a = GemmArgs()
    a.A, a.B = _p(A), _p(B)
    a.lda = A.stride(0) if lda is None else lda
    a.ldb = B.stride(0) if ldb is None else ldb
    a.M, a.N, a.K, a.epilogue = M, N, K, epi
    a.out0 = _p(out0)
    a.ldo0 = (out0.stride(0) if out0 is not None else 0) if ldo0 is None else ldo0
    a.out1 = _p(out1)
    a.ldo1 = (out1.stride(0) if out1 is not None else 0) if ldo1 is None else ldo1
    a.bias, a.vec1, a.resid = _p(bias), _p(vec1), _p(resid)
    a.ldr = (resid.stride(0) if resid is not None else 0) if ldr is None else ldr
    a.aux = _p(aux)
    a.ldaux = (aux.stride(0) if (aux is not None and aux.dim() > 1) else 0) if ldaux is None else ldaux
    a.rowmask = _p(rowmask)
    a.keep_prob, a.colscale, a.colscale_n = keep_prob, colscale, colscale_n
    a.rows_per_sample, a.accumulate = rows_per_sample, int(accumulate)
    a.colsum = _p(colsum)
    a.sample_map = _p(sample_map)
    a.colsum_copies = colsum_copies
    a.dropout = None if dropout is None else C.addressof(dropout)
    return a


def gemm_nt(A, B, M, N, K, epi, *args, **kw):
    a = gemm_args(A, B, M, N, K, epi, *args, **kw)
    _timed(epi, 2.0 * M * N * K, lambda: check(lib.memhip_gemm_bf16_nt(C.byref(a), stream_ptr()), "gemm_bf16_nt"))


NT_128, NT_G256, NT_P8_256, NT_P8_128, NT_P8_PAIR = range(5)


def gemm_nt_plan(a, stream_cus=None, device_cus=None):
    if stream_cus is None or device_cus is None:
        cus = torch.cuda.get_device_properties(torch.cuda.current_device()).multi_processor_count
        stream_cus = cus if stream_cus is None else stream_cus
        device_cus = cus if device_cus is None else device_cus
    plan = NtPlan()
    check(lib.memhip_gemm_bf16_nt_plan(C.byref(a), stream_cus, device_cus, C.byref(plan)), "gemm_bf16_nt_plan")
    return [plan.l[i] for i in range(plan.count)]


declare({
    "memhip_layernorm_fwd": (i32, [vp, i64, vp, i32, i32, vp, vp, f32, vp, i64, vp, vp, vp]),
    "memhip_layernorm_bwd": (i32, [vp, i64, vp, i64, vp, i32, i32, vp, vp, vp, vp, i64, i32, vp, vp, vp]),
    "memhip_layerscale_grad": (i32, [vp, i64, vp, i64, vp, vp, vp, i32, i32, vp, vp]),
    "memhip_embed_bwd": (i32, [vp, i64, vp, i32, i32, i32, vp, i64, vp, vp, vp]),
    "memhip_cross_entropy": (i32, [vp, i64, vp, i32, i32, f32, vp, vp, i32, vp, vp]),
    "memhip_attn_tokens_padded": (i32, [i32]),
    "memhip_relpos_gather": (i32, [vp, vp, i32, i32, i32, vp, vp, vp]),
    "memhip_attn_fwd": (i32, [vp, i64, i32, i32, i32, i32, vp, i32, i32, vp, i64, vp, vp]),
    "memhip_attn_delta": (i32, [vp, vp, i64, i64, i32, vp, vp]),
    "memhip_attn_bwd_workspace": (i64, [i32, i32, i32, i32, i32]),
    "memhip_cast_f32_bf16": (i32, [vp, vp, i64, vp]),
    "memhip_copy_samples_f32": (i32, [vp, vp, vp, i32, i64, vp]),
    "memhip_zero": (i32, [vp, i64, vp]),
    "memhip_stream_reserve_cus": (i32, [vp, i32]),
    "memhip_zero_ranges": (i32, [vp, vp, i32, i64, vp]),
    "memhip_transpose_cast_f32_bf16": (i32, [vp, i64, i32, i32, vp, i64, vp]),
    "memhip_transpose_bf16": (i32, [vp, i64, i32, i32, vp, i64, i32, vp, i32, i32, vp, i32, i32, vp]),
    "memhip_im2col_bf16": (i32, [vp, i32, i32, i32, i32, i32, i32, vp, vp]),
    "memhip_fill_cls": (i32, [vp, i64, i32, i32, i32, vp, vp]),
    "memhip_gemv_bf16_acc": (i32, [vp, i64, i32, i32, vp, vp, vp, vp, vp]),
    "memhip_nchw_to_padded_nhwc4": (i32, [vp, i32, i32, i32, i32, vp, vp, vp, i64, i32, vp]),
    "memhip_argmax_rows": (i32, [vp, i32, i64, i32, i32, vp, vp, vp, vp, i32, vp]),
    "memhip_tok_flag_samples": (i32, [vp, vp, i32, i32, f32, vp, vp, vp, vp]),
    "memhip_tok_gather_images_f32": (i32, [vp, i32, i32, i32, vp, vp, vp, vp, i32, i32, vp, vp, vp]),
    "memhip_tok_scatter_ids": (i32, [vp, vp, vp, i32, i32, i32, vp, vp]),
    "memhip_grad_norm_workspace": (sz, []),
    "memhip_grad_norm": (i32, [vp, i64, vp, vp, sz, vp]),
    "memhip_adamw": (i32, [vp, vp, vp, vp, i64, vp, f64, f64, f64, f64, f64, i32, vp, f64, vp]),
    "memhip_transpose_cast_batched": (i32, [vp, vp, i32, i32, vp]),
    "memhip_adamw_groups": (i32, [vp, vp, vp, vp, i64, vp, vp, i32, f64, f64, f64, i32, vp, f64, vp]),
    "memhip_dropout_mask": (i32, [C.POINTER(Dropout), i32, i32, i32, vp, vp]),
    "memhip_dropout_rows_f32": (i32, [C.POINTER(Dropout), vp, i64, i32, i32, vp]),
})


def dropout_mask(d, row0, rows, cols, out):
    check(lib.memhip_dropout_mask(C.byref(d), row0, rows, cols, ptr(out), stream_ptr()), "dropout_mask")


def dropout_rows(d, x, rows, D):
    check(lib.memhip_dropout_rows_f32(C.byref(d), ptr(x), x.stride(0), rows, D, stream_ptr()), "dropout_rows_f32")


def layernorm_fwd(x, gamma, beta, y, mean, rstd, R, D, eps=1e-6, row_idx=None):
    check(lib.memhip_layernorm_fwd(ptr(x), x.stride(0), ptr(row_idx), R, D, ptr(gamma), ptr(beta), eps,
                                   ptr(y), y.stride(0), ptr(mean), ptr(rstd), stream_ptr()), "layernorm_fwd")


def layernorm_bwd(dy, x, gamma, mean, rstd, dres, dgamma, dbeta, R, D, accumulate=True, row_idx=None):
    check(lib.memhip_layernorm_bwd(ptr(dy), dy.stride(0), ptr(x), x.stride(0), ptr(row_idx), R, D, ptr(gamma),
                                   ptr(mean), ptr(rstd), ptr(dres), dres.stride(0), int(accumulate),
                                   ptr(dgamma), ptr(dbeta), stream_ptr()), "layernorm_bwd")


def _branch(y, gamma, rowmask, keep_prob, rows_per_sample, dy, dgamma, dbias, out_map, dropout):
    return Branch(_p(y), y.stride(0) if y is not None else 0, _p(gamma), _p(rowmask), keep_prob, rows_per_sample, _p(dy),
                  dy.stride(0), _p(dgamma), _p(dbias), _p(out_map), None if dropout is None else C.addressof(dropout))


def layernorm_bwd_branch(dy, x, gamma, mean, rstd, dres, dgamma, dbeta, R, D, y_b, gamma_b, dy_b, dgamma_b, dbias_b,
                         rowmask=None, keep_prob=1.0, rows_per_sample=1, in_map=None, out_map=None, dropout=None):
    a = LnBwdBranchArgs(_p(dy), dy.stride(0), _p(x), x.stride(0), R, D, _p(gamma), _p(mean), _p(rstd), _p(dres), dres.stride(0),
                        _p(dgamma), _p(dbeta), _p(in_map),
                        _branch(y_b, gamma_b, rowmask, keep_prob, rows_per_sample, dy_b, dgamma_b, dbias_b, out_map, dropout))
    check(lib.memhip_layernorm_bwd_branch(C.byref(a), stream_ptr()), "layernorm_bwd_branch")


def layerscale_grad(W16, dW, bias, dbias, gamma, N, K, dgamma):
    check(lib.memhip_layerscale_grad(ptr(W16), W16.stride(0), ptr(dW), dW.stride(0), ptr(bias), ptr(dbias), ptr(gamma),
                                     N, K, ptr(dgamma), stream_ptr()), "layerscale_grad")


def branch_bwd(dx, y, gamma, dy, dgamma, dbias, M, D, rowmask=None, keep_prob=1.0, rows_per_sample=1, out_map=None, dropout=None):
    a = BranchBwdArgs(_p(dx), dx.stride(0), M, D,
                      _branch(y, gamma, rowmask, keep_prob, rows_per_sample, dy, dgamma, dbias, out_map, dropout))
    check(lib.memhip_branch_bwd(C.byref(a), stream_ptr()), "branch_bwd")


def gemv_acc(W, N, K, x, y, x_acc=None, zero=None):
    check(lib.memhip_gemv_bf16_acc(ptr(W), W.stride(0), N, K, ptr(x), ptr(y), ptr(x_acc), ptr(zero), stream_ptr()),
          "gemv_bf16_acc")


CONV_MODES = ("bf16", "fp32", "fp16x2")
_CONV_MODE = {torch.bfloat16: 0, torch.float32: 1, torch.float16: 2}
_F16X2 = 2


class ConvArgs(C.Structure):
    _fields_ = [("mode", i32), ("reserved0", i32), ("in", vp), ("in_plane", i64), ("weight", vp), ("w_plane", i64),
                ("bias", vp), ("add", vp), ("add_plane", i64), ("out", vp), ("out_plane", i64)] + \
               [(n, i32) for n in ("B", "H", "W", "Cin", "Cout", "ksize", "stride", "pad", "relu", "out_padded", "out_f32",
                                   "reserved1")] + [("n_active", vp)]


declare({"memhip_conv2d_nhwc": (i32, [C.POINTER(ConvArgs), vp])})


def conv_args(mode, B, H, W, Cin, Cout, ksize, stride, pad, x=None, weight=None, bias=None, out=None, relu=False, add=None,
              out_padded=True, out_f32=False, n_active=None, planes=(0, 0, 0, 0)):
    return ConvArgs(mode, 0, x, planes[0], weight, planes[1], bias, add, planes[2], out, planes[3], B, H, W, Cin, Cout, ksize,
                    stride, pad, int(relu), int(out_padded), int(out_f32), 0, n_active)


def conv2d_nhwc(x_pad, weight, bias, out, B, H, W, Cin, Cout, ksize, stride, pad, relu=False, add=None, out_padded=True,
                n_active=None):
    mode = _CONV_MODE[x_pad.dtype]
    out_f32 = mode == _F16X2 and out.dtype == torch.float32
    assert weight.dtype == x_pad.dtype and (out_f32 or out.dtype == x_pad.dtype) and (add is None or add.dtype == x_pad.dtype)
    planes = (0, 0, 0, 0) if mode != _F16X2 else (x_pad.stride(0), weight.stride(0), 0 if add is None else add.stride(0),
                                             0 if out_f32 else out.stride(0))
    a = conv_args(mode, B, H, W, Cin, Cout, ksize, stride, pad, _p(x_pad), _p(weight), _p(bias), _p(out), relu, _p(add),
                  out_padded and not out_f32, out_f32, _p(n_active), planes)
    check(lib.memhip_conv2d_nhwc(C.byref(a), stream_ptr()), "conv2d_nhwc")


def nchw_to_padded_nhwc4(x, out, mean=None, std=None):
    B, Cc, H, W = x.shape
    mode = _CONV_MODE[out.dtype]
    check(lib.memhip_nchw_to_padded_nhwc4(ptr(x), B, Cc, H, W, ptr(mean), ptr(std), ptr(out), out.stride(0) if mode == _F16X2 else 0,
                                          mode, stream_ptr()), "nchw_to_padded_nhwc4")


def argmax_rows(logits, M, N, ids, gap=None, rms=None, n_samples=None, rows_per_sample=0):
    check(lib.memhip_argmax_rows(ptr(logits), _CONV_MODE[logits.dtype], logits.stride(0), M, N, ptr(ids), ptr(gap), ptr(rms),
                                 ptr(n_samples), rows_per_sample, stream_ptr()), "argmax_rows")


def tok_flag_samples(gap, rms, B, hw, kappa, lst, count, stats=None):
    check(lib.memhip_tok_flag_samples(ptr(gap), ptr(rms), B, hw, float(kappa), ptr(lst), ptr(count), ptr(stats), stream_ptr()),
          "tok_flag_samples")


def tok_gather_images(x, mean, std, lst, count, offset, R, out, n_round):
    _, Cc, H, W = x.shape
    check(lib.memhip_tok_gather_images_f32(ptr(x), Cc, H, W, ptr(mean), ptr(std), ptr(lst), ptr(count), offset, R, ptr(out),
                                           ptr(n_round), stream_ptr()), "tok_gather_images_f32")


def tok_scatter_ids(ids_in, lst, n_round, offset, R, hw, ids_out):
    check(lib.memhip_tok_scatter_ids(ptr(ids_in), ptr(lst), ptr(n_round), offset, R, hw, ptr(ids_out), stream_ptr()),
          "tok_scatter_ids")


def embed_bwd(dx, mask_u8, B, L, D, dy, dcls, dmask_token):
    check(lib.memhip_embed_bwd(ptr(dx), dx.stride(0), ptr(mask_u8), B, L, D, ptr(dy), dy.stride(0), ptr(dcls),
                               ptr(dmask_token), stream_ptr()), "embed_bwd")
# ... 593 lines not shown
```

mem_amd/vit_engine.py:

```python
import math
from collections import namedtuple

import torch

from . import ops

ALIGN = 1024

Branch = namedtuple("Branch", "n rows gemm_rows ridx smap cmap rowmask keep_prob")


def _pad(n, a):
    return (n + a - 1) // a * a


def flat_layout(shapes, skip, order, aliases=()):
    decays = lambda n: not (len(shapes[n]) == 1 or n.endswith(".bias") or n in skip)
    segs, buckets, flags, off = {}, [], [], 0
    for bname, entries in order:
        b0 = off
        for e in entries:
            if isinstance(e, tuple):
                (n, k), flag = e, 0
            elif e in shapes:
                n, k, flag = e, math.prod(shapes[e]), int(decays(e))
            else:
                continue
            segs[n] = (off, k)
            size = _pad(k, ALIGN)
            flags += [flag] * (size // ALIGN)
            off += size
        buckets.append((bname, b0, off))
    for alias, seg, o, k in aliases:
        segs[alias] = (segs[seg][0] + o, k)
    missing = [n for n in shapes if n not in segs]
    assert not missing, f"parameters not placed in the flat buffer: {missing}"
    return segs, buckets, off, flags, [n for n in shapes if decays(n)]


def check_export(export, depth, what="export"):
    if export is None:
        return ()
    export = tuple(int(i) for i in export)
    for k, i in enumerate(export):
        if not 0 <= i < depth:
            raise ValueError(f"{what}: block index {i} outside [0, {depth})")
        if i in export[:k]:
            raise ValueError(f"{what}: block index {i} given twice")
        if k and i < export[k - 1]:
            raise ValueError(f"{what}: block indices must ascend, {i} follows {export[k - 1]}")
    return export


class FlatParams:

    def _pack_flat(self, named, skip, order, aliases=()):
        self.segs, self.buckets, self.nflat, flags, self.decay_names = flat_layout(
            {n: tuple(p.shape) for n, p in named.items()}, skip, order, aliases)
        self.flat_p = torch.zeros(self.nflat, dtype=torch.float32, device=self.dev)
        self.flat_g = torch.zeros(self.nflat, dtype=torch.float32, device=self.dev)
        self.wd_flags = torch.tensor(flags, dtype=torch.uint8, device=self.dev)
        self.named = named
        for n, p in named.items():
            o, k = self.segs[n]
            view = self.flat_p[o:o + k].view(p.shape)
            view.copy_(p.data)
            p.data = view
        self.attach_grads()

    def attach_grads(self):
        for n, p in self.named.items():
            o, k = self.segs[n]
            g = p.grad
            if g is None or g.data_ptr() != self.flat_g.data_ptr() + 4 * o:
                p.grad = self.flat_g[o:o + k].view(p.shape)

    def P(self, name):
        o, k = self.segs[name]
        return self.flat_p[o:o + k]

    def G(self, name):
        o, k = self.segs[name]
        return self.flat_g[o:o + k]


class ViTEngine(FlatParams):
    def __init__(self, model):
        self.model = model
# ... 16 lines not shown
        self.Kpe = self.C * self.ph * self.pw
        assert self.D % 64 == 0 and self.hidden % 64 == 0 and self.Kpe % 64 == 0, "GEMM K dims must be multiples of 64"
        self.has_pos = model.pos_embed is not None
        self.drop_rate = float(getattr(model, "drop_rate", 0.0))
        self.window = tuple(pe.patch_shape)
        self.nrd = (2 * self.window[0] - 1) * (2 * self.window[1] - 1) + 3
        if model.rel_pos_bias is not None:
            self.rel = "shared"
        elif getattr(model.blocks[0].attn, "relative_position_bias_table", None) is not None:
            self.rel = "block"
        else:
            self.rel = "none"
        self.TP = ops.attn_tokens_padded(self.T)
        self._pack_parameters()
        self._build_static()
        if hasattr(model, "register_state_dict_pre_hook"):
            model.register_state_dict_pre_hook(lambda *_a, **_k: self.wait_optimizer())
        self.B = 0
        self.Mm_cap = 0
        self.cur = None
        self.B_stash = 0
        self.step_masks = None
        self.weights_dirty = True
        self.w16_version = 0
        self._zero_plans = {}
        self.grad_hook = None
        self.hook_on_side = True
        self.accumulate_grads = False
        self.overlap_optimizer = False
        self._opt_stream = None
        self._opt_ev = None
        self._opt_done = None
        self.wgrad_side_stream = True
        self.wgrad_group = 2
        self.fwd_two_streams = False
        self._side = None
        self._ev_pool, self._ev_i = [], 0
        self.dp_skip = True
        self.tail_rows = True
        self._dp_stage = None

    def _pack_parameters(self):
        m, D = self.model, self.D
        order, aliases = [], []
        head = ["lm_head.weight", "lm_head.bias", "head.weight", "head.bias", "fc_norm.weight", "fc_norm.bias", "norm.weight",
                "norm.bias"]
        head += [n for n, _ in m.named_parameters() if n.startswith(tuple(getattr(m, "_TAIL_PREFIXES", ()))) and n not in head]
        order.append(("head", head))
        for i in reversed(range(self.depth)):
            pre = f"blocks.{i}."
            qkvb = pre + "attn.qkvbias3"
            aliases += [(pre + "attn.q_bias", qkvb, 0, D), (pre + "attn.v_bias", qkvb, 2 * D, D)]
            names = [pre + n for n in ("mlp.fc2.weight", "mlp.fc2.bias", "gamma_2", "mlp.fc1.weight", "mlp.fc1.bias",
                                       "norm2.weight", "norm2.bias", "attn.proj.weight", "attn.proj.bias", "gamma_1",
                                       "attn.qkv.weight")]
            names += [(qkvb, 3 * D)] + [pre + n for n in ("attn.relative_position_bias_table", "norm1.weight", "norm1.bias")]
            order.append((f"block{i}", names))
        order.append(("embed", ["rel_pos_bias.relative_position_bias_table", "patch_embed.proj.weight",
                                "patch_embed.proj.bias", "mask_token", "cls_token", "pos_embed"]))
        self._pack_flat(dict(m.named_parameters()), m.no_weight_decay(), order, aliases)
        self.flat_w16 = torch.zeros(self.nflat, dtype=torch.bfloat16, device=self.dev)
        self.no_decay_names = [n for n in self.named if n not in set(self.decay_names)]

    def W16(self, name, rows, cols):
        o, k = self.segs[name]
        return self.flat_w16[o:o + k].view(rows, cols)

    def _build_static(self):
        D, Hd, V, dev = self.D, self.hidden, self.V, self.dev
        bf = torch.bfloat16
        self.wT = {}
        for i in range(self.depth):
            self.wT[i] = dict(qkv=torch.empty((D, 3 * D), dtype=bf, device=dev),
                              proj=torch.empty((D, D), dtype=bf, device=dev),
                              fc1=torch.empty((D, Hd), dtype=bf, device=dev),
                              fc2=torch.empty((Hd, D), dtype=bf, device=dev))
        self.wT_lm = torch.empty((D, V), dtype=bf, device=dev) if self.head_kind == "mlm" else None
        self.zero_table = torch.zeros((self.nrd, self.heads), dtype=torch.float32, device=dev)
        self.zero_vec = torch.zeros(D, dtype=torch.float32, device=dev)
        self.head_end = self.buckets[0][2]
        self._tdesc = None
        self.set_gelu_dg(True)
        self.fuse_ln_branch = True
        self.gn_ws = torch.zeros(1024, dtype=torch.float64, device=dev)
        self.gnorm = torch.zeros(1, dtype=torch.float32, device=dev)
        self.loss_acc = torch.zeros(2, dtype=torch.float32, device=dev)

    def _matrix_grad_names(self):
        names = [f"blocks.{i}.{n}" for i in range(self.depth) for n in ("attn.qkv.weight", "attn.proj.weight", "mlp.fc1.weight",
                                                                       "mlp.fc2.weight")]
        names.append("patch_embed.proj.weight")
        if self.head_kind == "mlm":
            names.append("lm_head.weight")
        return names

    def _zero_small_grads(self, start=0):
        key = ("zr", start)
        if key not in self._zero_plans:
            import numpy as np
            mats = sorted(self.segs[n] for n in self._matrix_grad_names())
            ranges, pos = [], start
            for o, k in mats:
                end = o + _pad(k, ALIGN)
                if end <= start:
                    continue
                if o > pos:
                    ranges.append((pos * 4, (o - pos) * 4))
                pos = max(pos, end)
            if pos < self.nflat:
                ranges.append((pos * 4, (self.nflat - pos) * 4))
            arr = np.asarray(ranges, dtype=np.int64).reshape(-1, 2)
            self._zero_plans[key] = (torch.from_numpy(arr).to(self.dev), len(ranges), int(arr[:, 1].sum()) if len(ranges) else 0)
        dev, n, total = self._zero_plans[key]
        ops.zero_ranges(self.flat_g, dev, n, total)

    def _zero_grad_of(self, name):
        o, k = self.segs[name]
        ops.zero_(self.flat_g[o:o + _pad(k, ALIGN)])

    def set_gelu_dg(self, on):
        self.epi_gelu, self.epi_dgelu = (ops.EPI_BIAS_GELU_DG, ops.EPI_MUL_AUX) if on else (ops.EPI_BIAS_GELU, ops.EPI_DGELU)

    def ensure_batch(self, B, Mm_max, keep=True):
        if B > self.B:
            self._alloc_forward(B)
        if keep and self.B_stash < self.B:
            self._alloc_stash()
        if Mm_max > self.Mm_cap or (self.head_kind == "mlm" and not hasattr(self, "hN")):
            self._alloc_head(min(self.B * self.L, _pad(Mm_max + Mm_max // 16 + 1, 256)))

    def _alloc_head(self, Mm_cap):
        dev, bf, f32 = self.dev, torch.bfloat16, torch.float32
        D, V = self.D, self.V
        e = lambda *s, dt=bf: torch.empty(s, dtype=dt, device=dev)
        if self.head_kind == "mlm":
            self.hN = e(Mm_cap, D)
            self.meanN, self.rstdN = e(Mm_cap, dt=f32), e(Mm_cap, dt=f32)
            self.logits = e(Mm_cap, V)
            self.row_loss, self.row_ok = e(Mm_cap, dt=f32), torch.empty(Mm_cap, dtype=torch.int32, device=dev)
            self.dhN = e(Mm_cap, D)
            self.x_tail, self.dxc = e(max(Mm_cap, 1), D, dt=f32), e(max(Mm_cap, 1), D, dt=f32)
            self.y_tail = torch.zeros((_pad(max(Mm_cap, 1), 256), D), dtype=bf, device=dev)
        self.Mm_cap = Mm_cap

    def _act_set(self, B):
        dev, bf, f32 = self.dev, torch.bfloat16, torch.float32
        D, Hd, M = self.D, self.hidden, B * self.T
        Ma = M + 256
        e = lambda *s, dt=bf: torch.empty(s, dtype=dt, device=dev)
        z = lambda *s, dt=bf: torch.zeros(s, dtype=dt, device=dev)
        return dict(h1=z(Ma, D), qkv=z(Ma, 3 * D), ao=z(Ma, D), h2=z(Ma, D), hpre=z(Ma, Hd),
                    a=z(Ma, Hd), lse=e(B, self.heads, self.TP, dt=f32),
                    mean1=e(M, dt=f32), rstd1=e(M, dt=f32), mean2=e(M, dt=f32), rstd2=e(M, dt=f32))

    def _alloc_forward(self, B):
        dev, f32 = self.dev, torch.float32
        D, T = self.D, self.T
        M = B * T
        self.patches = torch.empty((B * self.L, self.Kpe), dtype=torch.bfloat16, device=dev)
        self.x = [torch.zeros((M + T, D), dtype=f32, device=dev) for _ in range(3)]
        self.act = [self._act_set(B)]
        if self.head_kind != "mlm":
            self.zero_mask = torch.zeros(B * self.L, dtype=torch.uint8, device=dev)
        for name in ("dx", "dY", "dh_small", "dY2", "dbig", "dqkv", "dao", "delta_ws", "_tn_ws", "bias_scr", "cs_ws", "dYpe"):
            if hasattr(self, name):
                delattr(self, name)
# ... 58 lines not shown
        self._tprefix = torch.from_numpy(prefix).to(self.dev)
        self._tn, self._ttiles = len(items), int(prefix[-1])
        self._tbucket = {}
        locs = []
        for i in range(self.depth):
            locs.append((f"block{i}", 4 * i, 4))
        if self.head_kind == "mlm":
            locs.append(("head", 4 * self.depth, 1))
        loc_prefix = []
        for name, k0, n in locs:
            pl = (prefix[k0:k0 + n + 1] - prefix[k0]).astype(np.int32)
            self._tbucket[name] = (k0, n, len(loc_prefix), int(pl[-1]))
            loc_prefix += list(pl)
        self._tprefix_loc = torch.from_numpy(np.asarray(loc_prefix, dtype=np.int32)).to(self.dev)

    def table(self, i):
        if self.rel == "shared":
            return self.P("rel_pos_bias.relative_position_bias_table")
        if self.rel == "block":
            return self.P(f"blocks.{i}.attn.relative_position_bias_table")
        return self.zero_table

    def dtable(self, i):
        if self.rel == "shared":
            return self.G("rel_pos_bias.relative_position_bias_table")
        if self.rel == "block":
            return self.G(f"blocks.{i}.attn.relative_position_bias_table")
        return None

    CS_COPIES = 8

    def _dp_plan(self, dp_masks, B):
        import numpy as np
        if dp_masks is None or not self.dp_skip:
            return None
        probs = [float(b.drop_prob) for b in self.model.blocks for _ in range(2)]
        if max(probs) == 0.0:
            return None
        mk = dp_masks.detach().cpu().numpy() if isinstance(dp_masks, torch.Tensor) else np.asarray(dp_masks)
        mk = mk.reshape(2 * self.depth, B) != 0
        J, T = 2 * self.depth, self.T
        W = 3 * B + 256
        host = np.zeros((J, W), dtype=np.int32)
        host[:, B + 256:2 * B + 256] = -1
        kept_n = []
        for j in range(J):
            if probs[j] == 0.0:
                kept_n.append(None)
                continue
            k = np.flatnonzero(mk[j]).astype(np.int32)
            d = np.flatnonzero(~mk[j]).astype(np.int32)
            host[j, :len(k)] = k
            host[j, len(k):B + 256] = B
            host[j, B + 256 + k] = np.arange(len(k), dtype=np.int32)
            host[j, 2 * B + 256:2 * B + 256 + len(d)] = d
            kept_n.append(len(k))
        if self._dp_stage is None or self._dp_stage_w != J * W:
            from .utils import HostStager
            self._dp_stage, self._dp_stage_w = HostStager(J * W * 4, self.dev), J * W
            self._dp_ar = torch.arange(T, dtype=torch.int32, device=self.dev)
        dev = self._dp_stage.put(host).view(torch.int32).view(J, W)
        ridx = (dev[:, :B, None] * T + self._dp_ar[None, None, :]).view(J, B * T)
        return dict(n=kept_n, kidx=dev[:, :B + 256], cmap=dev[:, B + 256:2 * B + 256], drop=dev[:, 2 * B + 256:], ridx=ridx, B=B)

    def _branches(self, B, plan, dp_masks):
        T, out = self.T, []
        for j in range(2 * self.depth):
            drop_prob = self.model.blocks[j // 2].drop_prob
            if plan is not None and plan["n"][j] is not None:
                n = plan["n"][j]
                out.append(Branch(n, n * T, _pad(n * T, 256), plan["ridx"][j], plan["kidx"][j], plan["cmap"][j], None,
                                  1.0 - drop_prob))
            else:
                rowmask = dp_masks[j] if (dp_masks is not None and drop_prob > 0.0) else None
                out.append(Branch(B, B * T, B * T, None, None, None, rowmask, 1.0 - drop_prob))
        return out

    def _drop(self, site, row0=0):
        key = self.cur["drop_key"] if self.cur else None
        if key is None:
            return None
        return ops.dropout_params(key[0], key[1], site, self.drop_rate, row0)

    def _copy_dropped(self, plan, j, src, dst, B):
        nd = B - plan["n"][j]
        if nd > 0:
            ops.copy_samples(src, dst, plan["drop"][j], nd, self.T * self.D)

    def forward(self, x, mask_u8, rows_idx, labels=None, dp_masks=None, all_tokens=False, labels_event=None):
        assert x.is_cuda and x.dtype == torch.float32 and x.is_contiguous()
        B = x.shape[0]
        assert tuple(x.shape[1:]) == (self.C, self.H, self.W), \
            f"Input image size ({x.shape[2]}*{x.shape[3]}) doesn't match model ({self.H}*{self.W})."
        Mm = rows_idx.numel()
        self.ensure_batch(B, Mm)
        use_tail = (self.tail_rows and not all_tokens and self.depth >= 1 and 0 < Mm and 4 * Mm <= 3 * B * self.T)
        xl = self.forward_trunk(x, mask_u8, dp_masks, tail_rows=rows_idx if use_tail else None)
        D, Hd, T, L, V = self.D, self.hidden, self.T, self.L, self.V
        M = B * T
        self.cur.update(Mm=Mm, rows=rows_idx, labels=labels)
        self._wait_params("head")
        if self.cur.get("tail") is not None:
            ops.layernorm_fwd(self.x_tail, self.P("norm.weight"), self.P("norm.bias"), self.hN, self.meanN, self.rstdN, Mm, D)
        else:
            ops.layernorm_fwd(xl, self.P("norm.weight"), self.P("norm.bias"), self.hN, self.meanN, self.rstdN, Mm, D,
                              row_idx=rows_idx)
        ops.gemm_nt(self.hN, self.W16("lm_head.weight", V, D), Mm, V, D, ops.EPI_BIAS_BF16, out0=self.logits,
                    bias=self.P("lm_head.bias"))
        if labels is not None:
            if labels_event is not None:
                torch.cuda.current_stream().wait_event(labels_event)
            ops.cross_entropy(self.logits, labels, Mm, V, 1.0 / Mm, self.row_loss, self.row_ok, self.loss_acc,
                              write_grad=True)
        return self.logits[:Mm]

    def _split_point(self, B, num_cu=256):
        ntn = max(1, self.D // 256)
        tile_rows = -(-B * self.T // 256)
        rounds = tile_rows * ntn // num_cu
        if rounds < 1:
            return 0
        bs = (rounds * num_cu // ntn) * 256 // self.T
        return bs if 0 < bs < B and (B - bs) * self.T >= 4096 else 0

    def _branch(self, j, b0, b1):
        br = self.cur["branch"][j]
        if b0 == 0 and b1 == self.cur["B"]:
            return br
        assert br.smap is None, "stochastic-depth work skipping runs the whole batch on one stream"
        rows = (b1 - b0) * self.T
        return br._replace(n=b1 - b0, rows=rows, gemm_rows=rows, rowmask=None if br.rowmask is None else br.rowmask[b0:b1])

    def _block_fwd(self, i, b0, b1):
        D, Hd, T = self.D, self.hidden, self.T
        r0, r1 = b0 * T, b1 * T
        pre = f"blocks.{i}."
        xs = self.cur["x"]
        a = self.cur["act"][i]
        B, plan = self.cur["B"], self.cur["plan"]
        ba, bm = self._branch(2 * i, b0, b1), self._branch(2 * i + 1, b0, b1)
        xin, xmid, xout = xs[2 * i][r0:r1], xs[2 * i + 1][r0:r1], xs[2 * i + 2][r0:r1]
        g1 = self.P(pre + "gamma_1") if (pre + "gamma_1") in self.segs else None
        g2 = self.P(pre + "gamma_2") if (pre + "gamma_2") in self.segs else None
        tail = self.cur["tail"] if (i == self.depth - 1 and b0 == 0 and b1 == B) else None
        if ba.smap is not None:
            self._copy_dropped(plan, 2 * i, xin, xmid, B)
        if ba.n > 0:
            rs = slice(r0, r1) if ba.smap is None else slice(None)
            h1, qkv, ao = a["h1"][rs], a["qkv"][rs], a["ao"][rs]
            ops.layernorm_fwd(xin, self.P(pre + "norm1.weight"), self.P(pre + "norm1.bias"), h1, a["mean1"][r0:r1],
                              a["rstd1"][r0:r1], ba.rows, D, row_idx=ba.ridx)
            ops.gemm_nt(h1, self.W16(pre + "attn.qkv.weight", 3 * D, D), ba.gemm_rows, 3 * D, D, ops.EPI_BIAS_BF16,
                        out0=qkv, bias=self.P(pre + "attn.qkvbias3"), colscale=self.scale, colscale_n=D)
            ops.attn_fwd(qkv, ba.n, T, D, self.heads, self.table(i), self.window, ao, a["lse"][b0:b1])
            da = self._drop(2 * i, r0)
            ops.gemm_nt(ao, self.W16(pre + "attn.proj.weight", D, D), ba.gemm_rows, D, D,
                        ops.EPI_RESIDUAL if da is None else ops.EPI_RESIDUAL_DROP, out0=None,
                        bias=self.P(pre + "attn.proj.bias"), vec1=g1, resid=xmid, aux=xin, ldaux=D, rowmask=ba.rowmask,
                        keep_prob=ba.keep_prob, rows_per_sample=T, sample_map=ba.smap, dropout=da)
        if tail is not None:
            self._mlp_fwd_tail(i, a, xs[2 * i + 1], g2, bm.keep_prob, tail)
            return
        if bm.smap is not None:
            self._copy_dropped(plan, 2 * i + 1, xmid, xout, B)
        if bm.n > 0:
            rs = slice(r0, r1) if bm.smap is None else slice(None)
            h2, hpre, aa = a["h2"][rs], a["hpre"][rs], a["a"][rs]
            ops.layernorm_fwd(xmid, self.P(pre + "norm2.weight"), self.P(pre + "norm2.bias"), h2, a["mean2"][r0:r1],
                              a["rstd2"][r0:r1], bm.rows, D, row_idx=bm.ridx)
            ops.gemm_nt(h2, self.W16(pre + "mlp.fc1.weight", Hd, D), bm.gemm_rows, Hd, D, self.epi_gelu, out0=hpre,
                        out1=aa, bias=self.P(pre + "mlp.fc1.bias"))
            dm = self._drop(2 * i + 1, r0)
            ops.gemm_nt(aa, self.W16(pre + "mlp.fc2.weight", D, Hd), bm.gemm_rows, D, Hd,
                        ops.EPI_RESIDUAL if dm is None else ops.EPI_RESIDUAL_DROP, out0=None,
                        bias=self.P(pre + "mlp.fc2.bias"), vec1=g2, resid=xout, aux=xmid, ldaux=D, rowmask=bm.rowmask,
                        keep_prob=bm.keep_prob, rows_per_sample=T, sample_map=bm.smap, dropout=dm)

    def _mlp_fwd_tail(self, i, a, xmid, g2, keep, tail):
        D, Hd = self.D, self.hidden
        pre = f"blocks.{i}."
        rows, Mm = tail["rows"], tail["Mm"]
        Mp = _pad(Mm, 256)
        assert self._drop(0) is None, "the tail-row form of the last block is pretraining-only: no element-wise dropout"
        ops.layernorm_fwd(xmid, self.P(pre + "norm2.weight"), self.P(pre + "norm2.bias"), a["h2"], a["mean2"], a["rstd2"],
                          Mm, D, row_idx=rows)
        ops.gemm_nt(a["h2"], self.W16(pre + "mlp.fc1.weight", Hd, D), Mp, Hd, D, self.epi_gelu, out0=a["hpre"],
                    out1=a["a"], bias=self.P(pre + "mlp.fc1.bias"))
        ops.gemm_nt(a["a"], self.W16(pre + "mlp.fc2.weight", D, Hd), Mp, D, Hd, ops.EPI_BIAS_BF16, out0=self.y_tail,
                    bias=self.P(pre + "mlp.fc2.bias"))
        ops.residual_rows(xmid, rows, self.y_tail, g2, tail["rowkeep"], keep, Mm, D, self.x_tail)

    def forward_trunk(self, x, mask_u8=None, dp_masks=None, tail_rows=None, drop_key=None, keep=True, export=None,
                      streams=None):
        export = check_export(export, self.depth)
        assert (not export and streams is None) or (self.head_kind == "cls" and tail_rows is None), \
            "per-block exports serve the finetuning trunk: no mlm head, no tail-row form"
        assert drop_key is None or (self.drop_rate > 0.0 and tail_rows is None), "dropout: finetuning trunk only"
        assert keep or (self.head_kind == "cls" and tail_rows is None), \
            "forward-only mode (keep=False) serves the finetuning trunk: no mlm head, no tail-row form"
        assert x.is_cuda and x.dtype == torch.float32 and x.is_contiguous()
        B = x.shape[0]
        assert tuple(x.shape[1:]) == (self.C, self.H, self.W), \
            f"Input image size ({x.shape[2]}*{x.shape[3]}) doesn't match model ({self.H}*{self.W})."
        self.ensure_batch(B, self.Mm_cap, keep=keep)
        if self.weights_dirty:
            self.sync_weights()
        if self.fwd_two_streams:
            self.wait_optimizer()
        self._wait_params("embed")
        if mask_u8 is None:
            mask_u8 = self.zero_mask[: B * self.L]
        D, Hd, T, L = self.D, self.hidden, self.T, self.L
        M = B * T
        plan = self._dp_plan(dp_masks, B)
        if plan is not None:
            dp_masks = None
        nx = 2 * self.depth + 1
        self.cur = dict(B=B, M=M, Mm=0, mask=mask_u8, rows=None, dp=dp_masks, labels=None, plan=plan, tail=None, drop_key=drop_key,
                        keep=bool(keep), x=self.x if keep else [self.x[j % 3] for j in range(nx)],
                        act=self.act if keep else [self.act[0]] * self.depth, branch=self._branches(B, plan, dp_masks),
                        maps=dict(zip(export, self._map_buffers(len(export), B))) if export else None, streams=streams, dmaps=None)
        if tail_rows is not None and not self.fwd_two_streams:
            jm, lastb = 2 * self.depth - 1, self.model.blocks[self.depth - 1]
            keepvec = None
            if lastb.drop_prob > 0.0:
                if plan is not None and plan["n"][jm] is not None:
                    keepvec = (plan["cmap"][jm] >= 0).to(torch.float32)
                elif dp_masks is not None:
                    keepvec = dp_masks[jm]
            rowkeep = None
            if keepvec is not None:
                rowkeep = keepvec.index_select(0, torch.div(tail_rows, T, rounding_mode="floor").long()).contiguous()
            self.cur["tail"] = dict(rows=tail_rows, Mm=tail_rows.numel(), rowkeep=rowkeep)
        if self.head_kind == "cls" and not self.accumulate_grads and self.head_end:
            ops.zero_(self.flat_g[: self.head_end])
        ops.im2col(x, B, self.C, self.H, self.W, self.ph, self.pw, self.patches)
        x0 = self.x[0]
        if not keep and plan is not None:
            ops.zero_(x0[M:M + T])
        ops.fill_cls(x0, B, T, D, self.P("cls_token"))
        ops.gemm_nt(self.patches, self.W16("patch_embed.proj.weight", D, self.Kpe), B * L, D, self.Kpe,
                    ops.EPI_PATCH_EMBED, bias=self.P("patch_embed.proj.bias"),
                    vec1=self.P("mask_token") if "mask_token" in self.segs else self.zero_vec,
                    resid=x0, aux=mask_u8, rows_per_sample=L, ldaux=0)
        if self.has_pos:
            x0[:M].view(B, T, D).add_(self.P("pos_embed").view(1, T, D))
        dpos = self._drop(2 * self.depth)
        if dpos is not None:
            ops.dropout_rows(dpos, x0, M, D)
        bs = self._split_point(B) if (self.fwd_two_streams and ops.GEMM_TIMER is None and plan is None) else 0
        split = 0 < bs < B
        if split:
            if self._side is None:
                self._side = torch.cuda.Stream(device=self.dev)
            e0 = torch.cuda.Event()
            e0.record()
            self._side.wait_event(e0)
            for i in range(self.depth):
                self._block_fwd(i, 0, bs)
                self._export_block(i, 0, bs)
                with torch.cuda.stream(self._side):
                    self._block_fwd(i, bs, B)
                    self._export_block(i, bs, B)
            e1 = torch.cuda.Event()
            e1.record(self._side)
            torch.cuda.current_stream().wait_event(e1)
        else:
            for i in range(self.depth):
                self._wait_params(f"block{i}")
                self._block_fwd(i, 0, B)
                self._export_block(i, 0, B)
        return self.cur["x"][2 * self.depth][:M]

    def _export_block(self, i, b0, b1):
        c = self.cur
        if c["maps"] is None and c["streams"] is None:
            return
        xout, T = c["x"][2 * i + 2], self.T
        if c["maps"] is not None and i in c["maps"]:
            ops.tokens_to_maps(xout, c["B"], T, out=c["maps"][i], b0=b0, b1=b1)
        if c["streams"] is not None:
            c["streams"][i][b0 * T:b1 * T].copy_(xout[b0 * T:b1 * T])

    def _tn_ws_at_least(self, need):
        if need > self._tn_ws.numel():
            self._tn_ws = torch.empty(need, dtype=torch.uint8, device=self.dev)

# ... 117 lines not shown
            self.logits[:Mm].copy_(dlogits)
        if not self.accumulate_grads:
            self._zero_small_grads()
        dx = self.dx
        ops.zero_(dx[:M])
        dl = self.logits
        self._side_begin()
        ops.gemm_nt(dl, self.wT_lm, Mm, D, V, ops.EPI_BIAS_BF16, out0=self.dhN)
        self._on_side(lambda: self._wgrad(dl, self.hN, Mm, V, D, "lm_head.weight", bias_grads=((self.G("lm_head.bias"), 0, V),)))
        if c.get("tail") is not None:
            ops.layernorm_bwd(self.dhN, self.x_tail, self.P("norm.weight"), self.meanN, self.rstdN, self.dxc,
                              self.G("norm.weight"), self.G("norm.bias"), Mm, D, accumulate=False)
            ops.scatter_rows(self.dxc, c["rows"], Mm, D, dx)
        else:
            ops.layernorm_bwd(self.dhN, self.x[2 * self.depth], self.P("norm.weight"), self.meanN, self.rstdN, dx,
                              self.G("norm.weight"), self.G("norm.bias"), Mm, D, accumulate=False, row_idx=c["rows"])
        self._backward_trunk()

    def backward_trunk(self, dxl, dmaps=None):
        c = self.cur
        if not c.get("keep", True):
            raise RuntimeError("backward_trunk after forward_trunk(keep=False): a forward-only pass keeps no activations "
                               "(the blocks shared one buffer set); run the forward with keep=True to train the trunk")
        M, D = c["M"], self.D
        if not self.accumulate_grads:
            self._zero_small_grads(self.head_end)
        if dxl is None:
            ops.zero_(self.dx[:M])
        else:
            self.dx[:M].copy_(dxl.reshape(M, D))
        if dmaps is not None:
            B, n = c["B"], c["B"] * D * self.L
            for i, g in dmaps.items():
                if not 0 <= i < self.depth:
                    raise ValueError(f"dmaps: block index {i} outside [0, {self.depth})")
                assert g.is_cuda and g.dtype == torch.float32 and g.is_contiguous() and g.numel() == n, \
                    f"dmaps[{i}]: contiguous fp32 [{B}, {D}, {self.window[0]}, {self.window[1]}]"
        c["dmaps"] = dmaps or None
        self._side_begin()
        self._backward_trunk()

    def _inject_dmap(self, i):
        dm = self.cur.get("dmaps")
        if dm is not None and i in dm:
            ops.maps_to_tokens_add(dm[i], self.dx, self.cur["B"], self.T)

    def _attn_branch_bwd(self, i, scr):
        pre = f"blocks.{i}."
        ba = self.cur["branch"][2 * i]
        self._before_overwrite("dY2")
        ops.branch_bwd(self.dx, None, self.P(pre + "gamma_1") if (pre + "gamma_1") in self.segs else None, self.dY2, None, scr,
                       self.cur["M"], self.D, rowmask=ba.rowmask, keep_prob=ba.keep_prob, rows_per_sample=self.T,
                       out_map=ba.cmap, dropout=self._drop(2 * i))

    def _mlp_bwd_tail(self, i, a, pre, has_g, keep, tail, scr):
        D, Hd = self.D, self.hidden
        rows, Mm, rk = tail["rows"], tail["Mm"], tail["rowkeep"]
        Mp = _pad(Mm, 256)
        assert self._drop(0) is None, "the tail-row form of the last block is pretraining-only: no element-wise dropout"
        dx, dY = self.dx, self.dY
        self._before_overwrite("dY")
        ops.branch_bwd(self.dxc, None, self.P(pre + "gamma_2") if has_g else None, dY, None, self.G(pre + "mlp.fc2.bias"),
                       Mm, D, rowmask=rk, keep_prob=keep, rows_per_sample=1)
        if Mp > Mm:
            ops.zero_(dY[Mm:Mp])
        self._before_overwrite("dbig")
        ops.gemm_nt(dY, self.wT[i]["fc2"], Mp, Hd, D, self.epi_dgelu, out0=self.dbig, aux=a["hpre"],
                    colsum=self.cs_ws, colsum_copies=self.CS_COPIES)
        ops.colsum_fold(self.cs_ws, self.CS_COPIES, Hd, self.G(pre + "mlp.fc1.bias"))
        self._on_side(lambda: self._wg_mlp(pre, a, has_g, Mm, dY))
        ops.gemm_nt(self.dbig, self.wT[i]["fc1"], Mp, D, Hd, ops.EPI_BIAS_BF16, out0=self.dh_small)
        ops.layernorm_bwd(self.dh_small, self.x[2 * i + 1], self.P(pre + "norm2.weight"), a["mean2"], a["rstd2"], dx,
                          self.G(pre + "norm2.weight"), self.G(pre + "norm2.bias"), Mm, D, accumulate=True, row_idx=rows)
        self._attn_branch_bwd(i, scr)

    def _backward_trunk(self):
        c = self.cur
        B, M, br = c["B"], c["M"], c["branch"]
        D, Hd, T = self.D, self.hidden, self.T
        dx, dY, dY2 = self.dx, self.dY, self.dY2
        self._bucket_ready(0)
        ops.zero_(self.bias_scr)
        fuse = D <= 1024 and self.fuse_ln_branch
        self._inject_dmap(self.depth - 1)
        for i in reversed(range(self.depth)):
            pre = f"blocks.{i}."
            a = self.act[i]
            ba, bm = br[2 * i], br[2 * i + 1]
            xin, xmid = self.x[2 * i], self.x[2 * i + 1]
            has_g = (pre + "gamma_1") in self.segs
            table, dtable = self.table(i), self.dtable(i)
            scr = self.bias_scr[i & 1]
            tail = c["tail"] if i == self.depth - 1 else None
            if tail is not None:
                self._mlp_bwd_tail(i, a, pre, has_g, bm.keep_prob, tail, scr)
            else:
                if i == self.depth - 1 or not fuse:
                    self._before_overwrite("dY")
                    ops.branch_bwd(dx, None, self.P(pre + "gamma_2") if has_g else None, dY, None, self.G(pre + "mlp.fc2.bias"),
                                   M, D, rowmask=bm.rowmask, keep_prob=bm.keep_prob, rows_per_sample=T, out_map=bm.cmap,
                                   dropout=self._drop(2 * i + 1))
                if bm.n == 0 and not self.accumulate_grads:
                    self._zero_grad_of(pre + "mlp.fc1.weight")
                    self._zero_grad_of(pre + "mlp.fc2.weight")
                if bm.n > 0:
                    self._before_overwrite("dbig")
                    if bm.gemm_rows > bm.rows:
                        ops.zero_(dY[bm.rows:bm.gemm_rows])
                    ops.gemm_nt(dY, self.wT[i]["fc2"], bm.gemm_rows, Hd, D, self.epi_dgelu, out0=self.dbig, aux=a["hpre"],
                                colsum=self.cs_ws, colsum_copies=self.CS_COPIES)
                    ops.colsum_fold(self.cs_ws, self.CS_COPIES, Hd, self.G(pre + "mlp.fc1.bias"))
                    self._on_side(lambda: self._wg_mlp(pre, a, has_g, bm.rows, dY))
                    ops.gemm_nt(self.dbig, self.wT[i]["fc1"], bm.gemm_rows, D, Hd, ops.EPI_BIAS_BF16, out0=self.dh_small)
                if fuse:
                    self._before_overwrite("dY2")
                    ops.layernorm_bwd_branch(self.dh_small, xmid, self.P(pre + "norm2.weight"), a["mean2"], a["rstd2"], dx,
                                             self.G(pre + "norm2.weight"), self.G(pre + "norm2.bias"), M, D, None,
                                             self.P(pre + "gamma_1") if has_g else None, dY2, None, scr,
                                             rowmask=ba.rowmask, keep_prob=ba.keep_prob, rows_per_sample=T,
                                             in_map=bm.cmap, out_map=ba.cmap, dropout=self._drop(2 * i))
                else:
                    if bm.n > 0:
                        ops.layernorm_bwd(self.dh_small, xmid, self.P(pre + "norm2.weight"), a["mean2"], a["rstd2"], dx,
                                          self.G(pre + "norm2.weight"), self.G(pre + "norm2.bias"), bm.rows, D, accumulate=True,
                                          row_idx=bm.ridx)
                    self._attn_branch_bwd(i, scr)
            if ba.n == 0 and not self.accumulate_grads:
                self._zero_grad_of(pre + "attn.proj.weight")
                self._zero_grad_of(pre + "attn.qkv.weight")
            if ba.n > 0:
                ops.gemm_nt(dY2, self.wT[i]["proj"], ba.gemm_rows, D, D, ops.EPI_BIAS_BF16, out0=self.dao)
            ops.gemv_acc(self.wT[i]["proj"], D, D, scr, self.G(pre + "attn.v_bias"),
                         x_acc=self.G(pre + "attn.proj.bias"), zero=self.bias_scr[(i & 1) ^ 1])
            if ba.n > 0:
                def wg_proj(grouped=False):
                    if not grouped:
                        self._wgrad(dY2, a["ao"], ba.rows, D, D, pre + "attn.proj.weight")
                    self._side_read_done("dY2")
                    if has_g:
                        ops.layerscale_grad(self.W16(pre + "attn.proj.weight", D, D), self.G(pre + "attn.proj.weight").view(D, D),
                                            self.P(pre + "attn.proj.bias"), self.G(pre + "attn.proj.bias"),
                                            self.P(pre + "gamma_1"), D, D, self.G(pre + "gamma_1"))
                if not self.wgrad_group:
                    self._on_side(wg_proj)
                self._before_overwrite("dqkv")
                ops.attn_bwd(a["qkv"], self.dao, a["lse"], self.delta_ws, table, self.window, ba.n, T, D, self.heads,
                             self.scale, self.dqkv, dtable, dq_bias=self.G(pre + "attn.q_bias"), out=a["ao"],
                             ws=self._attn_ws(ba.n))

                def wg_qkv():
                    if self.wgrad_group:
                        self._wgrad_group([(dY2, a["ao"], ba.rows, D, D, pre + "attn.proj.weight"),
                                           (self.dqkv, a["h1"], ba.rows, 3 * D, D, pre + "attn.qkv.weight")])
                        wg_proj(grouped=True)
                    else:
                        self._wgrad(self.dqkv, a["h1"], ba.rows, 3 * D, D, pre + "attn.qkv.weight")
                    self._side_read_done("dqkv")
                self._on_side(wg_qkv)
                ops.gemm_nt(self.dqkv, self.wT[i]["qkv"], ba.gemm_rows, D, 3 * D, ops.EPI_BIAS_BF16, out0=self.dh_small)
            if i > 0:
                self._inject_dmap(i - 1)
            if fuse and i > 0:
                pb, bb = f"blocks.{i - 1}.", br[2 * i - 1]
                self._before_overwrite("dY")
                ops.layernorm_bwd_branch(self.dh_small, xin, self.P(pre + "norm1.weight"), a["mean1"], a["rstd1"], dx,
                                         self.G(pre + "norm1.weight"), self.G(pre + "norm1.bias"), M, D, None,
                                         self.P(pb + "gamma_2") if (pb + "gamma_2") in self.segs else None, dY, None,
                                         self.G(pb + "mlp.fc2.bias"), rowmask=bb.rowmask, keep_prob=bb.keep_prob,
                                         rows_per_sample=T, in_map=ba.cmap, out_map=bb.cmap, dropout=self._drop(2 * i - 1))
            elif ba.n > 0:
                ops.layernorm_bwd(self.dh_small, xin, self.P(pre + "norm1.weight"), a["mean1"], a["rstd1"], dx,
                                  self.G(pre + "norm1.weight"), self.G(pre + "norm1.bias"), ba.rows, D, accumulate=True,
                                  row_idx=ba.ridx)
            self._bucket_ready(self.depth - i)
        self._backward_embed(c, B, M)

    def _backward_embed(self, c, B, M):
        D, T, L = self.D, self.T, self.L
        dx = self.dx
        dpos = self._drop(2 * self.depth)
        if dpos is not None:
            ops.dropout_rows(dpos, dx, M, D)
        if self.has_pos:
            if self.accumulate_grads:
                self.G("pos_embed").view(T, D).add_(dx[:M].view(B, T, D).sum(0))
            else:
                self.G("pos_embed").view(T, D).copy_(dx[:M].view(B, T, D).sum(0))
        ops.embed_bwd(dx, c["mask"], B, L, D, self.dYpe, self.G("cls_token"),
                      self.G("mask_token") if "mask_token" in self.segs else self.zero_vec)
        self._on_side(lambda: self._wgrad(self.dYpe, self.patches, B * L, D, self.Kpe, "patch_embed.proj.weight",
                                          bias_grads=((self.G("patch_embed.proj.bias"), 0, D),)))
        self._side_join()
        if self.grad_hook:
            self.grad_hook(self.depth + 1)

    def grad_norm(self, end=None):
        n = self.nflat if end is None else end
        ops.grad_norm(self.flat_g[:n], n, self.gnorm, self.gn_ws)
        return self.gnorm

    def weights_updated(self, end=None):
        if end is None or end >= self.nflat:
            self.weights_dirty = True
        elif not self.weights_dirty:
            assert end <= self.head_end, "partial weight update: the head bucket only (no transposed copies to refresh)"
            ops.cast_f32_bf16(self.flat_p[:end], self.flat_w16[:end], end)
            self.w16_version += 1

    def adamw_step(self, m, v, lr, wd, step, betas=(0.9, 0.95), eps=1e-8, max_norm=0.0):
        if not (self.overlap_optimizer and self.head_kind == "mlm" and not self.fwd_two_streams):
            self.wait_optimizer()
            ops.adamw(self.flat_p, self.flat_g, m, v, self.nflat, self.wd_flags, lr, betas[0], betas[1], eps, wd, step,
                      gnorm=self.gnorm, max_norm=max_norm or 0.0)
            self.weights_dirty = True
            return
        self.wait_optimizer()
        if self._tdesc is None:
            self._build_transpose_descs()
        if self._opt_stream is None:
            self._opt_stream = torch.cuda.Stream(device=self.dev)
            self._opt_events = {b[0]: torch.cuda.Event() for b in self.buckets}
            self._opt_events["__done__"] = torch.cuda.Event()
            self._opt_start = torch.cuda.Event()
        main, st = torch.cuda.current_stream(), self._opt_stream
        self._opt_start.record(main)
        with torch.cuda.stream(st):
            st.wait_event(self._opt_start)
            for name, b0, b1 in reversed(self.buckets):
                if b1 == b0:
                    self._opt_events[name].record(st)
                    continue
                ops.adamw(self.flat_p[b0:b1], self.flat_g[b0:b1], m[b0:b1], v[b0:b1], b1 - b0,
                          self.wd_flags[b0 // ALIGN: b1 // ALIGN], lr, betas[0], betas[1], eps, wd, step,
                          gnorm=self.gnorm, max_norm=max_norm or 0.0)
                ops.cast_f32_bf16(self.flat_p[b0:b1], self.flat_w16[b0:b1], b1 - b0)
                self._opt_events[name].record(st)
            for name, (k0, n, p0, tiles) in self._tbucket.items():
                ops.transpose_cast_batched(self._tdesc[k0:k0 + n], self._tprefix_loc[p0:p0 + n + 1], n, tiles)
            self._opt_events["__done__"].record(st)
        self._opt_ev = self._opt_events
        self._opt_done = self._opt_events["__done__"]
        self.weights_dirty = False
        self.w16_version += 1

    def _wait_params(self, bucket):
        if self._opt_ev is not None:
            torch.cuda.current_stream().wait_event(self._opt_ev[bucket])

    def wait_optimizer(self):
        if self._opt_done is not None:
            torch.cuda.current_stream().wait_event(self._opt_done)
            self._opt_ev = None
# ... 2 lines not shown
```

Measured before the change: 7565.

## Piggyback small row tasks onto layernorm kernels as extra blocks

Introduces a row-task list (copy samples, zero, colsum fold, gemv accumulate) that executes in extra blocks appended to the layernorm forward and layernorm-backward-branch grids. In the forward pass, copies of dropped samples ride along with the layernorm launch. In the backward pass, colsum folding, the bias gemv and pad zeroing can ride along under an opt-in option value. The aim is to remove separate small kernel launches and their serialization gaps, at the cost of more kernel variants and divergent block roles.

```diff
diff --git a/include/memhip.h b/include/memhip.h
--- a/include/memhip.h
+++ b/include/memhip.h
@@ -281,6 +281,29 @@
   memhip_branch_t branch;
 } memhip_ln_bwd_branch_args_t;
 int memhip_layernorm_bwd_branch(const memhip_ln_bwd_branch_args_t* args, memhip_stream_t stream);
+
+enum { MEMHIP_ROW_TASK_COPY_SAMPLES = 0, MEMHIP_ROW_TASK_ZERO = 1, MEMHIP_ROW_TASK_COLSUM_FOLD = 2, MEMHIP_ROW_TASK_GEMV_ACC = 3 };
+#define MEMHIP_ROW_TASKS_MAX 4
+struct memhip_row_task {
+  int32_t kind;
+  int32_t nblocks;
+  const void* src;
+  void* dst;
+  const void* vec;
+  void* acc;
+  void* clear;
+  int64_t n;
+  int64_t ld;
+  int32_t count;
+  int32_t reserved0;
+};
+typedef struct memhip_row_task memhip_row_task_t;
+int memhip_row_task_blocks(const memhip_row_task_t* task);
+int memhip_layernorm_fwd_tasks(const float* x, int64_t ldx, const int32_t* row_idx, int R, int D,
+                               const float* gamma, const float* beta, float eps, void* y_bf16, int64_t ldy,
+                               float* mean, float* rstd, const memhip_row_task_t* tasks, int ntasks, memhip_stream_t stream);
+int memhip_layernorm_bwd_branch_tasks(const memhip_ln_bwd_branch_args_t* args, const memhip_row_task_t* tasks, int ntasks,
+                                      memhip_stream_t stream);
 
 int memhip_embed_bwd(const float* dx, int64_t lddx, const uint8_t* mask, int B, int L, int D,
                      void* dy_bf16, int64_t lddy, float* dcls, float* dmask_token, memhip_stream_t stream);
diff --git a/mem_amd/csrc/common.h b/mem_amd/csrc/common.h
--- a/mem_amd/csrc/common.h
+++ b/mem_amd/csrc/common.h
@@ -25,7 +25,7 @@
 }
 
 enum { OPT_GEMM_P8, OPT_GEMM256, OPT_GEMM_SPLIT, OPT_GEMM_P8_HALF, OPT_GEMM_P8_MIN_N, OPT_GEMM256_MIN_N, OPT_TN_P8,
-       OPT_RASTER_LDS, OPT_ATTN16, OPT_ATTN16_STAGGER, OPT_ATTN16_STAGGER_FWD, OPT_GEMM_STAGGER, OPT_GEMM_PREFETCH, OPT_RESERVE_CUS, OPT_LN_BWD_GRID, OPT_ATTN_WIN, OPT_GEMM_P8_PAIR, OPT_TN_GROUP, OPT_CONV_WAVES, OPT_RASTER_BANDS, OPT_COUNT_ };
+       OPT_RASTER_LDS, OPT_ATTN16, OPT_ATTN16_STAGGER, OPT_ATTN16_STAGGER_FWD, OPT_GEMM_STAGGER, OPT_GEMM_PREFETCH, OPT_RESERVE_CUS, OPT_LN_BWD_GRID, OPT_ATTN_WIN, OPT_GEMM_P8_PAIR, OPT_TN_GROUP, OPT_CONV_WAVES, OPT_RASTER_BANDS, OPT_ROW_TASKS, OPT_COUNT_ };
 int opt(int id);
 int usable_cus(hipStream_t s = nullptr);
 int max_cus();
diff --git a/mem_amd/csrc/core.cpp b/mem_amd/csrc/core.cpp
--- a/mem_amd/csrc/core.cpp
+++ b/mem_amd/csrc/core.cpp
@@ -14,9 +14,10 @@
      {1},
      {1},
      {16},
-     {0}};
+     {0},
+     {1}};
 static const char* const g_opt_name[OPT_COUNT_] = {"gemm_p8", "gemm256", "gemm_split", "gemm_p8_half", "gemm_p8_min_n",
-                                                   "gemm256_min_n", "tn_p8", "raster_lds", "attn16", "attn16_stagger", "attn16_stagger_fwd", "gemm_stagger", "gemm_prefetch", "reserve_cus", "ln_bwd_grid", "attn_win", "gemm_p8_pair", "tn_group", "conv_waves", "raster_bands"};
+                                                   "gemm256_min_n", "tn_p8", "raster_lds", "attn16", "attn16_stagger", "attn16_stagger_fwd", "gemm_stagger", "gemm_prefetch", "reserve_cus", "ln_bwd_grid", "attn_win", "gemm_p8_pair", "tn_group", "conv_waves", "raster_bands", "row_tasks"};
 int opt(int id) { return g_opt[id].load(std::memory_order_relaxed); }
 
 struct StreamReserve { std::atomic<bool> used{false}; std::atomic<void*> stream{nullptr}; std::atomic<int> cus{0}; };
diff --git a/mem_amd/csrc/gemm_tn.hip b/mem_amd/csrc/gemm_tn.hip
--- a/mem_amd/csrc/gemm_tn.hip
+++ b/mem_amd/csrc/gemm_tn.hip
@@ -1,4 +1,5 @@
 #include "common.h"
+#include "row_tasks.hpp"
 #include "gemm_tn_plan.hpp"
 
 namespace {
@@ -266,21 +267,14 @@
 
 namespace {
 __global__ __launch_bounds__(256) void colsum_fold_kernel(float* __restrict__ ws, int copies, int N, float* __restrict__ out) {
-  const int n = blockIdx.x * 256 + threadIdx.x;
-  if (n >= N) return;
-  float s = 0.f;
-  for (int k = 0; k < copies; ++k) {
-    s += ws[(long long)k * N + n];
-    ws[(long long)k * N + n] = 0.f;
-  }
-  out[n] += s;
+  colsum_fold_block(blockIdx.x, ws, copies, N, out);
 }
 }
 
 extern "C" int memhip_colsum_fold(float* ws, int copies, int N, float* out, memhip_stream_t stream) {
   MEMHIP_REQUIRE(copies >= 1 && N > 0, "colsum_fold: bad shape");
   MEMHIP_REQUIRE(ws && out, "colsum_fold: null pointer");
-  hipLaunchKernelGGL(colsum_fold_kernel, dim3(cdiv(N, 256)), dim3(256), 0, as_stream(stream), ws, copies, N, out);
+  hipLaunchKernelGGL(colsum_fold_kernel, dim3(colsum_fold_blocks(N)), dim3(256), 0, as_stream(stream), ws, copies, N, out);
   return check_launch("colsum_fold");
 }
 
diff --git a/mem_amd/csrc/misc.hip b/mem_amd/csrc/misc.hip
--- a/mem_amd/csrc/misc.hip
+++ b/mem_amd/csrc/misc.hip
@@ -1,4 +1,5 @@
 #include "common.h"
+#include "row_tasks.hpp"
 
 namespace {
 
@@ -145,25 +146,7 @@
 __global__ __launch_bounds__(256) void gemv_acc_kernel(const __bf16* __restrict__ W, long long ldw, int N, int K,
                                                        const float* __restrict__ x, float* __restrict__ y,
                                                        float* __restrict__ x_acc, float* __restrict__ zero) {
-  const int lane = threadIdx.x & 63;
-  const int n = blockIdx.x * 4 + (threadIdx.x >> 6);
-  if (n < N) {
-    float s = 0.f;
-    for (int k = lane * 8; k < K; k += 512) {
-      const bf16x8 w = *reinterpret_cast<const bf16x8*>(W + (long long)n * ldw + k);
-      const float4 a = *reinterpret_cast<const float4*>(x + k), b = *reinterpret_cast<const float4*>(x + k + 4);
-      s += (float)w[0] * a.x + (float)w[1] * a.y + (float)w[2] * a.z + (float)w[3] * a.w + (float)w[4] * b.x +
-           (float)w[5] * b.y + (float)w[6] * b.z + (float)w[7] * b.w;
-    }
-    for (int o = 32; o > 0; o >>= 1) s += __shfl_xor(s, o);
-    if (lane == 0) y[n] += s;
-  }
-  if (blockIdx.x == 0) {
-    for (int k = threadIdx.x; k < K; k += blockDim.x) {
-      if (x_acc) x_acc[k] += x[k];
-      if (zero) zero[k] = 0.f;
-    }
-  }
+  gemv_acc_block(blockIdx.x, W, ldw, N, K, x, y, x_acc, zero);
 }
 
 }
@@ -230,10 +213,7 @@
 
 __global__ __launch_bounds__(256) void copy_samples_kernel(const float* __restrict__ src, float* __restrict__ dst,
                                                            const int* __restrict__ ids, long long n_per_sample) {
-  const long long base = (long long)ids[blockIdx.y] * n_per_sample;
-  const float4* s4 = reinterpret_cast<const float4*>(src + base);
-  float4* d4 = reinterpret_cast<float4*>(dst + base);
-  for (long long i = (long long)blockIdx.x * 256 + threadIdx.x; i < n_per_sample / 4; i += (long long)gridDim.x * 256) d4[i] = s4[i];
+  copy_samples_block(blockIdx.x, gridDim.x, blockIdx.y, src, dst, ids, n_per_sample);
 }
 
 extern "C" int memhip_copy_samples_f32(const float* src, float* dst, const int32_t* ids, int n, int64_t n_per_sample,
@@ -241,16 +221,13 @@
   MEMHIP_REQUIRE(n >= 0 && n_per_sample > 0 && n_per_sample % 4 == 0, "copy_samples: bad shape");
   if (n == 0) return MEMHIP_OK;
   MEMHIP_REQUIRE(src && dst && ids, "copy_samples: null pointer");
-  int gx = (int)((n_per_sample / 4 + 255) / 256);
-  if (gx > 64) gx = 64;
-  hipLaunchKernelGGL(copy_samples_kernel, dim3(gx, n), dim3(256), 0, as_stream(stream), src, dst, (const int*)ids,
+  hipLaunchKernelGGL(copy_samples_kernel, dim3(copy_samples_gx(n_per_sample), n), dim3(256), 0, as_stream(stream), src, dst, (const int*)ids,
                      (long long)n_per_sample);
   return check_launch("copy_samples");
 }
 
 __global__ __launch_bounds__(256) void zero_kernel(uint4* __restrict__ p, long long n16) {
-  const long long step = (long long)gridDim.x * 256;
-  for (long long i = (long long)blockIdx.x * 256 + threadIdx.x; i < n16; i += step) p[i] = uint4{0u, 0u, 0u, 0u};
+  zero_block(blockIdx.x, gridDim.x, p, n16);
 }
 __global__ __launch_bounds__(256) void zero_ranges_kernel(char* __restrict__ base, const long long* __restrict__ ranges, int n) {
   const long long step = (long long)gridDim.x * 256;
@@ -265,9 +242,7 @@
   MEMHIP_REQUIRE(bytes >= 0 && bytes % 16 == 0 && ((uintptr_t)p & 15) == 0, "zero: pointer and size must be multiples of 16 bytes");
   if (bytes == 0) return MEMHIP_OK;
   MEMHIP_REQUIRE(p, "zero: null pointer");
-  long long g = (bytes / 16 + 255) / 256;
-  if (g > 2048) g = 2048;
-  hipLaunchKernelGGL(zero_kernel, dim3((unsigned)g), dim3(256), 0, as_stream(stream), (uint4*)p, (long long)(bytes / 16));
+  hipLaunchKernelGGL(zero_kernel, dim3(zero_blocks(bytes)), dim3(256), 0, as_stream(stream), (uint4*)p, (long long)(bytes / 16));
   return check_launch("zero");
 }
 
@@ -368,7 +343,7 @@
   MEMHIP_REQUIRE(N >= 0 && K >= 0 && K % 8 == 0 && ldw % 8 == 0, "gemv: K and ldw must be multiples of 8");
   if (N == 0 || K == 0) return MEMHIP_OK;
   MEMHIP_REQUIRE(W && x && y, "gemv: null pointer");
-  hipLaunchKernelGGL(gemv_acc_kernel, dim3((N + 3) / 4), dim3(256), 0, as_stream(stream), (const __bf16*)W,
+  hipLaunchKernelGGL(gemv_acc_kernel, dim3(gemv_acc_blocks(N)), dim3(256), 0, as_stream(stream), (const __bf16*)W,
                      (long long)ldw, N, K, x, y, x_acc, zero);
   return check_launch("gemv_bf16_acc");
 }
diff --git a/mem_amd/csrc/row_tasks.hpp b/mem_amd/csrc/row_tasks.hpp
--- /dev/null
+++ b/mem_amd/csrc/row_tasks.hpp
@@ -0,0 +1,104 @@
+#pragma once
+#include "common.h"
+
+namespace memhip {
+
+typedef __attribute__((ext_vector_type(8))) __bf16 task_bf16x8;
+
+__device__ __forceinline__ void copy_samples_block(int bx, int gx, int by, const float* __restrict__ src, float* __restrict__ dst,
+                                                   const int* __restrict__ ids, long long n_per_sample) {
+  const long long base = (long long)ids[by] * n_per_sample;
+  const float4* s4 = reinterpret_cast<const float4*>(src + base);
+  float4* d4 = reinterpret_cast<float4*>(dst + base);
+  for (long long i = (long long)bx * 256 + threadIdx.x; i < n_per_sample / 4; i += (long long)gx * 256) d4[i] = s4[i];
+}
+
+__device__ __forceinline__ void zero_block(int b, int nb, uint4* __restrict__ p, long long n16) {
+  const long long step = (long long)nb * 256;
+  for (long long i = (long long)b * 256 + threadIdx.x; i < n16; i += step) p[i] = uint4{0u, 0u, 0u, 0u};
+}
+
+__device__ __forceinline__ void colsum_fold_block(int b, float* __restrict__ ws, int copies, int N, float* __restrict__ out) {
+  const int n = b * 256 + threadIdx.x;
+  if (n >= N) return;
+  float s = 0.f;
+  for (int k = 0; k < copies; ++k) {
+    s += ws[(long long)k * N + n];
+    ws[(long long)k * N + n] = 0.f;
+  }
+  out[n] += s;
+}
+
+__device__ __forceinline__ void gemv_acc_block(int b, const __bf16* __restrict__ W, long long ldw, int N, int K,
+                                               const float* __restrict__ x, float* __restrict__ y,
+                                               float* __restrict__ x_acc, float* __restrict__ zero) {
+  const int lane = threadIdx.x & 63;
+  const int n = b * 4 + (threadIdx.x >> 6);
+  if (n < N) {
+    float s = 0.f;
+    for (int k = lane * 8; k < K; k += 512) {
+      const task_bf16x8 w = *reinterpret_cast<const task_bf16x8*>(W + (long long)n * ldw + k);
+      const float4 a = *reinterpret_cast<const float4*>(x + k), b2 = *reinterpret_cast<const float4*>(x + k + 4);
+      s += (float)w[0] * a.x + (float)w[1] * a.y + (float)w[2] * a.z + (float)w[3] * a.w + (float)w[4] * b2.x +
+           (float)w[5] * b2.y + (float)w[6] * b2.z + (float)w[7] * b2.w;
+    }
+    for (int o = 32; o > 0; o >>= 1) s += __shfl_xor(s, o);
+    if (lane == 0) y[n] += s;
+  }
+  if (b == 0) {
+    for (int k = threadIdx.x; k < K; k += 256) {
+      if (x_acc) x_acc[k] += x[k];
+      if (zero) zero[k] = 0.f;
+    }
+  }
+}
+
+struct RowTaskList {
+  memhip_row_task_t t[MEMHIP_ROW_TASKS_MAX];
+  int n;
+};
+
+__device__ __forceinline__ void run_row_task(const memhip_row_task_t& t, int b) {
+  switch (t.kind) {
+    case MEMHIP_ROW_TASK_COPY_SAMPLES: {
+      const int gx = t.nblocks / t.count, by = b / gx;
+      copy_samples_block(b - by * gx, gx, by, (const float*)t.src, (float*)t.dst, (const int*)t.vec, t.n);
+      break;
+    }
+    case MEMHIP_ROW_TASK_ZERO: zero_block(b, t.nblocks, (uint4*)t.dst, t.n >> 4); break;
+    case MEMHIP_ROW_TASK_COLSUM_FOLD: colsum_fold_block(b, (float*)t.dst, t.count, (int)t.n, (float*)t.acc); break;
+    case MEMHIP_ROW_TASK_GEMV_ACC:
+      gemv_acc_block(b, (const __bf16*)t.src, t.ld, t.count, (int)t.n, (const float*)t.vec, (float*)t.dst, (float*)t.acc,
+                     (float*)t.clear);
+      break;
+    default: break;
+  }
+}
+
+__device__ __forceinline__ void run_row_tasks(const RowTaskList& L, int b) {
+  static_assert(MEMHIP_ROW_TASKS_MAX == 4, "one step per task below");
+#define MEMHIP_ROW_TASK_STEP(k)                                      \
+  if (k >= L.n) return;                                              \
+  if (b < L.t[k].nblocks) { run_row_task(L.t[k], b); return; }       \
+  b -= L.t[k].nblocks;
+  MEMHIP_ROW_TASK_STEP(0)
+  MEMHIP_ROW_TASK_STEP(1)
+  MEMHIP_ROW_TASK_STEP(2)
+  MEMHIP_ROW_TASK_STEP(3)
+#undef MEMHIP_ROW_TASK_STEP
+}
+
+inline int copy_samples_gx(long long n_per_sample) {
+  const long long gx = (n_per_sample / 4 + 255) / 256;
+  return gx > 64 ? 64 : (int)gx;
+}
+inline int zero_blocks(long long bytes) {
+  const long long g = (bytes / 16 + 255) / 256;
+  return g > 2048 ? 2048 : (int)g;
+}
+inline int colsum_fold_blocks(int N) { return cdiv(N, 256); }
+inline int gemv_acc_blocks(int N) { return (N + 3) / 4; }
+
+int row_task_check(const memhip_row_task_t& t, int* blocks);
+
+}
diff --git a/mem_amd/csrc/rowops.hip b/mem_amd/csrc/rowops.hip
--- a/mem_amd/csrc/rowops.hip
+++ b/mem_amd/csrc/rowops.hip
@@ -1,5 +1,6 @@
 #include "common.h"
 #include "dropout.hpp"
+#include "row_tasks.hpp"
 
 #include <type_traits>
 
@@ -71,15 +72,15 @@
 __device__ __forceinline__ float sq2(float a, float b) { return __fmaf_rn(a, a, mul_rn(b, b)); }
 
 template <int NCH, bool FULL>
-__global__ __launch_bounds__(256) void ln_fwd_kernel(const float* __restrict__ x, long long ldx,
-                                                     const int* __restrict__ row_idx, int R, int D,
-                                                     const float* __restrict__ gamma,
-                                                     const float* __restrict__ beta, float eps,
-                                                     __bf16* __restrict__ y, long long ldy,
-                                                     float* __restrict__ mean, float* __restrict__ rstd) {
+__device__ __forceinline__ void ln_fwd_body(int bid, const float* __restrict__ x, long long ldx,
+                                            const int* __restrict__ row_idx, int R, int D,
+                                            const float* __restrict__ gamma,
+                                            const float* __restrict__ beta, float eps,
+                                            __bf16* __restrict__ y, long long ldy,
+                                            float* __restrict__ mean, float* __restrict__ rstd) {
   extern __shared__ float red[];
   const int lane = threadIdx.x & 63;
-  const int r0 = blockIdx.x * 4 + wave_id();
+  const int r0 = bid * 4 + wave_id();
   const bool act = r0 < R;
   const int r = act ? r0 : R - 1;
   const long long src = row_idx ? row_idx[r] : r;
@@ -139,6 +140,29 @@
       yr[i] = o;
     }
   }
+}
+
+template <int NCH, bool FULL>
+__global__ __launch_bounds__(256) void ln_fwd_kernel(const float* __restrict__ x, long long ldx,
+                                                     const int* __restrict__ row_idx, int R, int D,
+                                                     const float* __restrict__ gamma,
+                                                     const float* __restrict__ beta, float eps,
+                                                     __bf16* __restrict__ y, long long ldy,
+                                                     float* __restrict__ mean, float* __restrict__ rstd) {
+  ln_fwd_body<NCH, FULL>(blockIdx.x, x, ldx, row_idx, R, D, gamma, beta, eps, y, ldy, mean, rstd);
+}
+
+template <int NCH, bool FULL>
+__global__ __launch_bounds__(256) void ln_fwd_tasks_kernel(const float* __restrict__ x, long long ldx,
+                                                           const int* __restrict__ row_idx, int R, int D,
+                                                           const float* __restrict__ gamma,
+                                                           const float* __restrict__ beta, float eps,
+                                                           __bf16* __restrict__ y, long long ldy,
+                                                           float* __restrict__ mean, float* __restrict__ rstd,
+                                                           int main_grid, RowTaskList tasks) {
+  const int bid = blockIdx.x;
+  if (bid >= main_grid) { run_row_tasks(tasks, bid - main_grid); return; }
+  ln_fwd_body<NCH, FULL>(bid, x, ldx, row_idx, R, D, gamma, beta, eps, y, ldy, mean, rstd);
 }
 
 __device__ __forceinline__ void vm_drain() { __builtin_amdgcn_s_waitcnt(0x0F70); }
@@ -404,18 +428,18 @@
 }
 
 template <int NCH, bool FULL, bool HAS_Y, class... Drop>
-__global__ __launch_bounds__(256) void ln_bwd_branch_kernel(const __bf16* __restrict__ dy, long long lddy,
-                                                            const float* __restrict__ x, long long ldx, int R, int D,
-                                                            const float* __restrict__ gamma,
-                                                            const float* __restrict__ mean, const float* __restrict__ rstd,
-                                                            float* __restrict__ dres, long long lddres,
-                                                            float* __restrict__ dgamma, float* __restrict__ dbeta,
-                                                            const __bf16* __restrict__ yb, long long ldyb,
-                                                            const float* __restrict__ gb, const float* __restrict__ rowmask,
-                                                            float keep, int rps, __bf16* __restrict__ dyo, long long lddyo,
-                                                            float* __restrict__ dgb, float* __restrict__ dbiasb,
-                                                            const int* __restrict__ in_map, const int* __restrict__ out_map,
-                                                            Drop... drop) {
+__device__ __forceinline__ void ln_bwd_branch_body(int bid, int nblk, const __bf16* __restrict__ dy, long long lddy,
+                                                   const float* __restrict__ x, long long ldx, int R, int D,
+                                                   const float* __restrict__ gamma,
+                                                   const float* __restrict__ mean, const float* __restrict__ rstd,
+                                                   float* __restrict__ dres, long long lddres,
+                                                   float* __restrict__ dgamma, float* __restrict__ dbeta,
+                                                   const __bf16* __restrict__ yb, long long ldyb,
+                                                   const float* __restrict__ gb, const float* __restrict__ rowmask,
+                                                   float keep, int rps, __bf16* __restrict__ dyo, long long lddyo,
+                                                   float* __restrict__ dgb, float* __restrict__ dbiasb,
+                                                   const int* __restrict__ in_map, const int* __restrict__ out_map,
+                                                   Drop... drop) {
   extern __shared__ float red[];
   const int lane = threadIdx.x & 63, wave = wave_id();
   const int nch = D >> 2;
@@ -457,7 +481,7 @@
       if (chunk_ok<FULL>(i, nch)) prev[c] = o[i];
     }
   };
-  const int row0 = blockIdx.x * 4 + wave, rstride = gridDim.x * 4;
+  const int row0 = bid * 4 + wave, rstride = nblk * 4;
   auto resolve = [&](const RowWalk& t, int& rin, int& rout) {
     rin = rout = t.r;
     if (in_map) { const int ci = in_map[t.smp]; rin = ci < 0 ? -1 : ci * t.rps + t.off; }
@@ -614,6 +638,43 @@
   }
 }
 
+template <int NCH, bool FULL, bool HAS_Y, class... Drop>
+__global__ __launch_bounds__(256) void ln_bwd_branch_kernel(const __bf16* __restrict__ dy, long long lddy,
+                                                            const float* __restrict__ x, long long ldx, int R, int D,
+                                                            const float* __restrict__ gamma,
+                                                            const float* __restrict__ mean, const float* __restrict__ rstd,
+                                                            float* __restrict__ dres, long long lddres,
+                                                            float* __restrict__ dgamma, float* __restrict__ dbeta,
+                                                            const __bf16* __restrict__ yb, long long ldyb,
+                                                            const float* __restrict__ gb, const float* __restrict__ rowmask,
+                                                            float keep, int rps, __bf16* __restrict__ dyo, long long lddyo,
+                                                            float* __restrict__ dgb, float* __restrict__ dbiasb,
+                                                            const int* __restrict__ in_map, const int* __restrict__ out_map,
+                                                            Drop... drop) {
+  ln_bwd_branch_body<NCH, FULL, HAS_Y, Drop...>(blockIdx.x, gridDim.x, dy, lddy, x, ldx, R, D, gamma, mean, rstd, dres, lddres, dgamma,
+                                                dbeta, yb, ldyb, gb, rowmask, keep, rps, dyo, lddyo, dgb, dbiasb, in_map, out_map,
+                                                drop...);
+}
+
+template <int NCH, bool FULL, bool HAS_Y, class... Drop>
+__global__ __launch_bounds__(256) void ln_bwd_branch_tasks_kernel(const __bf16* __restrict__ dy, long long lddy,
+                                                                  const float* __restrict__ x, long long ldx, int R, int D,
+                                                                  const float* __restrict__ gamma,
+                                                                  const float* __restrict__ mean, const float* __restrict__ rstd,
+                                                                  float* __restrict__ dres, long long lddres,
+                                                                  float* __restrict__ dgamma, float* __restrict__ dbeta,
+                                                                  const __bf16* __restrict__ yb, long long ldyb,
+                                                                  const float* __restrict__ gb, const float* __restrict__ rowmask,
+                                                                  float keep, int rps, __bf16* __restrict__ dyo, long long lddyo,
+                                                                  float* __restrict__ dgb, float* __restrict__ dbiasb,
+                                                                  const int* __restrict__ in_map, const int* __restrict__ out_map,
+                                                                  int main_grid, RowTaskList tasks, Drop... drop) {
+  const int bid = blockIdx.x;
+  if (bid >= main_grid) { run_row_tasks(tasks, bid - main_grid); return; }
+  ln_bwd_branch_body<NCH, FULL, HAS_Y, Drop...>(bid, main_grid, dy, lddy, x, ldx, R, D, gamma, mean, rstd, dres, lddres, dgamma, dbeta,
+                                                yb, ldyb, gb, rowmask, keep, rps, dyo, lddyo, dgb, dbiasb, in_map, out_map, drop...);
+}
+
 
 __global__ __launch_bounds__(256) void layerscale_grad_kernel(const __bf16* __restrict__ W, long long ldw,
                                                               const float* __restrict__ dW, long long lddw,
@@ -821,18 +882,118 @@
   }
 }
 
+namespace memhip {
+int row_task_check(const memhip_row_task_t& t, int* blocks) {
+  MEMHIP_REQUIRE(t.n > 0, "row task: n=%lld must be positive", (long long)t.n);
+  switch (t.kind) {
+    case MEMHIP_ROW_TASK_COPY_SAMPLES:
+      MEMHIP_REQUIRE(t.count > 0 && t.n % 4 == 0, "row task copy_samples: bad shape");
+      MEMHIP_REQUIRE(t.src && t.dst && t.vec, "row task copy_samples: null pointer");
+      *blocks = copy_samples_gx(t.n) * t.count;
+      MEMHIP_REQUIRE((long long)copy_samples_gx(t.n) * t.count < (1ll << 24), "row task copy_samples: too many samples");
+      return MEMHIP_OK;
+    case MEMHIP_ROW_TASK_ZERO:
+      MEMHIP_REQUIRE(t.dst, "row task zero: null pointer");
+      MEMHIP_REQUIRE(t.n % 16 == 0 && ((uintptr_t)t.dst & 15) == 0, "row task zero: pointer and size must be multiples of 16 bytes");
+      *blocks = zero_blocks(t.n);
+      return MEMHIP_OK;
+    case MEMHIP_ROW_TASK_COLSUM_FOLD:
+      MEMHIP_REQUIRE(t.count >= 1 && t.n < (1ll << 31), "row task colsum_fold: bad shape");
+      MEMHIP_REQUIRE(t.dst && t.acc, "row task colsum_fold: null pointer");
+      *blocks = colsum_fold_blocks((int)t.n);
+      return MEMHIP_OK;
+    case MEMHIP_ROW_TASK_GEMV_ACC:
+      MEMHIP_REQUIRE(t.count > 0 && t.n < (1ll << 31) && t.n % 8 == 0 && t.ld % 8 == 0, "row task gemv_acc: K and ldw must be multiples of 8");
+      MEMHIP_REQUIRE(t.src && t.vec && t.dst, "row task gemv_acc: null pointer");
+      *blocks = gemv_acc_blocks(t.count);
+      return MEMHIP_OK;
+    default:
+      return fail(MEMHIP_EINVAL, "row task: unknown kind %d", t.kind);
+  }
+}
+}
+
+extern "C" int memhip_row_task_blocks(const memhip_row_task_t* task) {
+  int blocks = 0;
+  if (!task) { fail(MEMHIP_EINVAL, "row_task_blocks: null task"); return 0; }
+  return row_task_check(*task, &blocks) == MEMHIP_OK ? blocks : 0;
+}
+
+static int row_tasks_gather(const char* who, const memhip_row_task_t* tasks, int ntasks, RowTaskList* L, int* extra) {
+  MEMHIP_REQUIRE(ntasks >= 0 && ntasks <= MEMHIP_ROW_TASKS_MAX, "%s: ntasks=%d outside [0, %d]", who, ntasks, MEMHIP_ROW_TASKS_MAX);
+  MEMHIP_REQUIRE(ntasks == 0 || tasks, "%s: null task list", who);
+  *L = RowTaskList{};
+  L->n = ntasks;
+  long long sum = 0;
+  for (int k = 0; k < ntasks; ++k) {
+    int want = 0;
+    MEMHIP_REQUIRE(tasks[k].nblocks > 0, "%s: task %d: nblocks=%d must be positive", who, k, tasks[k].nblocks);
+    if (const int rc = row_task_check(tasks[k], &want)) return rc;
+    MEMHIP_REQUIRE(tasks[k].nblocks == want, "%s: task %d: nblocks=%d, the stand-alone form launches %d (memhip_row_task_blocks)", who, k,
+                   tasks[k].nblocks, want);
+    L->t[k] = tasks[k];
+    sum += want;
+  }
+  MEMHIP_REQUIRE(sum < (1ll << 24), "%s: %lld task workgroups", who, sum);
+  *extra = (int)sum;
+  return MEMHIP_OK;
+}
+
+static int row_tasks_standalone(const RowTaskList& L, memhip_stream_t stream) {
+  for (int k = 0; k < L.n; ++k) {
+    const memhip_row_task_t& t = L.t[k];
+    int rc = MEMHIP_OK;
+    switch (t.kind) {
+      case MEMHIP_ROW_TASK_COPY_SAMPLES:
+        rc = memhip_copy_samples_f32((const float*)t.src, (float*)t.dst, (const int32_t*)t.vec, t.count, t.n, stream);
+        break;
+      case MEMHIP_ROW_TASK_ZERO: rc = memhip_zero(t.dst, t.n, stream); break;
+      case MEMHIP_ROW_TASK_COLSUM_FOLD: rc = memhip_colsum_fold((float*)t.dst, t.count, (int)t.n, (float*)t.acc, stream); break;
+      case MEMHIP_ROW_TASK_GEMV_ACC:
+        rc = memhip_gemv_bf16_acc(t.src, t.ld, t.count, (int)t.n, (const float*)t.vec, (float*)t.dst, (float*)t.acc, (float*)t.clear, stream);
+        break;
+    }
+    if (rc) return rc;
+  }
+  return MEMHIP_OK;
+}
+
+static int layernorm_fwd_launch(const float* x, int64_t ldx, const int32_t* row_idx, int R, int D, const float* gamma, const float* beta,
+                                float eps, void* y, int64_t ldy, float* mean, float* rstd, const RowTaskList* L, int extra,
+                                memhip_stream_t stream) {
+  MEMHIP_REQUIRE(R >= 0 && D > 0 && D % 4 == 0 && D <= 64 * 4 * kMaxChunks, "layernorm_fwd: bad R=%d D=%d", R, D);
+  if (R == 0) return L ? row_tasks_standalone(*L, stream) : MEMHIP_OK;
+  MEMHIP_REQUIRE(x && gamma && beta && y && mean && rstd, "layernorm_fwd: null pointer");
+  MEMHIP_REQUIRE(ldx % 4 == 0 && ldy % 4 == 0, "layernorm_fwd: ld must be a multiple of 4");
+  const int grid = cdiv(R, 4);
+  dispatch_width<kMaxChunks>(D, [&](auto N, auto F) {
+    if (L)
+      hipLaunchKernelGGL((ln_fwd_tasks_kernel<decltype(N)::value, decltype(F)::value>), dim3(grid + extra), dim3(256), (size_t)2 * D * sizeof(float), as_stream(stream),
+                         x, (long long)ldx, row_idx, R, D, gamma, beta, eps, (__bf16*)y, (long long)ldy, mean, rstd, grid, *L);
+    else
+      hipLaunchKernelGGL((ln_fwd_kernel<decltype(N)::value, decltype(F)::value>), dim3(grid), dim3(256), (size_t)2 * D * sizeof(float), as_stream(stream),
+                         x, (long long)ldx, row_idx, R, D, gamma, beta, eps, (__bf16*)y, (long long)ldy, mean, rstd);
+  });
+  return check_launch("layernorm_fwd");
+}
+
 extern "C" int memhip_layernorm_fwd(const float* x, int64_t ldx, const int32_t* row_idx, int R, int D,
                                     const float* gamma, const float* beta, float eps, void* y,
                                     int64_t ldy, float* mean, float* rstd, memhip_stream_t stream) {
-  MEMHIP_REQUIRE(R >= 0 && D > 0 && D % 4 == 0 && D <= 64 * 4 * kMaxChunks, "layernorm_fwd: bad R=%d D=%d", R, D);
-  if (R == 0) return MEMHIP_OK;
-  MEMHIP_REQUIRE(x && gamma && beta && y && mean && rstd, "layernorm_fwd: null pointer");
-  MEMHIP_REQUIRE(ldx % 4 == 0 && ldy % 4 == 0, "layernorm_fwd: ld must be a multiple of 4");
-  dispatch_width<kMaxChunks>(D, [&](auto N, auto F) {
-    hipLaunchKernelGGL((ln_fwd_kernel<decltype(N)::value, decltype(F)::value>), dim3(cdiv(R, 4)), dim3(256), (size_t)2 * D * sizeof(float), as_stream(stream),
-                       x, (long long)ldx, row_idx, R, D, gamma, beta, eps, (__bf16*)y, (long long)ldy, mean, rstd);
-  });
-  return check_launch("layernorm_fwd");
+  return layernorm_fwd_launch(x, ldx, row_idx, R, D, gamma, beta, eps, y, ldy, mean, rstd, nullptr, 0, stream);
+}
+
+extern "C" int memhip_layernorm_fwd_tasks(const float* x, int64_t ldx, const int32_t* row_idx, int R, int D,
+                                          const float* gamma, const float* beta, float eps, void* y, int64_t ldy,
+                                          float* mean, float* rstd, const memhip_row_task_t* tasks, int ntasks,
+                                          memhip_stream_t stream) {
+  RowTaskList L;
+  int extra = 0;
+  if (const int rc = row_tasks_gather("layernorm_fwd_tasks", tasks, ntasks, &L, &extra)) return rc;
+  if (ntasks > 0 && opt(OPT_ROW_TASKS))
+    return layernorm_fwd_launch(x, ldx, row_idx, R, D, gamma, beta, eps, y, ldy, mean, rstd, &L, extra, stream);
+  if (const int rc = layernorm_fwd_launch(x, ldx, row_idx, R, D, gamma, beta, eps, y, ldy, mean, rstd, nullptr, 0, stream)) return rc;
+  return row_tasks_standalone(L, stream);
 }
 
 extern "C" int memhip_layernorm_bwd(const void* dy, int64_t lddy, const float* x, int64_t ldx,
@@ -924,16 +1085,24 @@
 }
 
 template <int NCH, bool FULL, bool HAS_Y, class... Drop>
-static void ln_bwd_branch_launch(const memhip_ln_bwd_branch_args_t& a, int grid, memhip_stream_t stream, Drop... drop) {
+static void ln_bwd_branch_launch(const memhip_ln_bwd_branch_args_t& a, int grid, const RowTaskList* L, int extra, memhip_stream_t stream,
+                                 Drop... drop) {
   const memhip_branch_t& b = a.branch;
-  hipLaunchKernelGGL((ln_bwd_branch_kernel<NCH, FULL, HAS_Y, Drop...>), dim3(grid), dim3(256), (size_t)16 * a.D * sizeof(float),
-                     as_stream(stream), (const __bf16*)a.dy, (long long)a.lddy, a.x, (long long)a.ldx, a.R, a.D, a.gamma, a.mean,
-                     a.rstd, a.dres, (long long)a.lddres, a.dgamma, a.dbeta, (const __bf16*)b.y, (long long)b.ldy, b.gamma,
-                     b.rowmask, b.keep_prob, b.rows_per_sample > 0 ? b.rows_per_sample : 1, (__bf16*)b.dy, (long long)b.lddy,
-                     b.dgamma, b.dbias, (const int*)a.in_map, (const int*)b.out_map, drop...);
-}
-
-extern "C" int memhip_layernorm_bwd_branch(const memhip_ln_bwd_branch_args_t* args, memhip_stream_t stream) {
+  if (L)
+    hipLaunchKernelGGL((ln_bwd_branch_tasks_kernel<NCH, FULL, HAS_Y, Drop...>), dim3(grid + extra), dim3(256), (size_t)16 * a.D * sizeof(float),
+                       as_stream(stream), (const __bf16*)a.dy, (long long)a.lddy, a.x, (long long)a.ldx, a.R, a.D, a.gamma, a.mean,
+                       a.rstd, a.dres, (long long)a.lddres, a.dgamma, a.dbeta, (const __bf16*)b.y, (long long)b.ldy, b.gamma,
+                       b.rowmask, b.keep_prob, b.rows_per_sample > 0 ? b.rows_per_sample : 1, (__bf16*)b.dy, (long long)b.lddy,
+                       b.dgamma, b.dbias, (const int*)a.in_map, (const int*)b.out_map, grid, *L, drop...);
+  else
+    hipLaunchKernelGGL((ln_bwd_branch_kernel<NCH, FULL, HAS_Y, Drop...>), dim3(grid), dim3(256), (size_t)16 * a.D * sizeof(float),
+                       as_stream(stream), (const __bf16*)a.dy, (long long)a.lddy, a.x, (long long)a.ldx, a.R, a.D, a.gamma, a.mean,
+                       a.rstd, a.dres, (long long)a.lddres, a.dgamma, a.dbeta, (const __bf16*)b.y, (long long)b.ldy, b.gamma,
+                       b.rowmask, b.keep_prob, b.rows_per_sample > 0 ? b.rows_per_sample : 1, (__bf16*)b.dy, (long long)b.lddy,
+                       b.dgamma, b.dbias, (const int*)a.in_map, (const int*)b.out_map, drop...);
+}
+
+static int layernorm_bwd_branch_launch(const memhip_ln_bwd_branch_args_t* args, const RowTaskList* L, int extra, memhip_stream_t stream) {
   MEMHIP_REQUIRE(args, "layernorm_bwd_branch: null args");
   const memhip_ln_bwd_branch_args_t& a = *args;
   const memhip_branch_t& b = a.branch;
@@ -942,7 +1111,7 @@
   MEMHIP_REQUIRE(!b.dropout || D % 8 == 0, "layernorm_bwd_branch_drop: D=%d must be a multiple of 8", D);
   MEMHIP_REQUIRE(!(a.in_map || b.out_map) || (!b.rowmask && !b.y && b.rows_per_sample > 0),
                  "layernorm_bwd_branch: sample maps exclude rowmask / y_branch");
-  if (R == 0) return MEMHIP_OK;
+  if (R == 0) return L ? row_tasks_standalone(*L, stream) : MEMHIP_OK;
   MEMHIP_REQUIRE(a.dy && a.x && a.gamma && a.mean && a.rstd && a.dres && a.dgamma && a.dbeta && b.dy,
                  "layernorm_bwd_branch: null pointer");
   MEMHIP_REQUIRE(b.y || !b.dgamma, "layernorm_bwd_branch: dgamma_branch needs y_branch");
@@ -955,16 +1124,30 @@
   dispatch_width<4>(D, [&](auto N, auto F) {
     if (b.dropout)
       dispatch_bool(b.y, [&](auto Y) {
-        ln_bwd_branch_launch<decltype(N)::value, decltype(F)::value, decltype(Y)::value>(a, grid, stream, drop_params(*b.dropout));
+        ln_bwd_branch_launch<decltype(N)::value, decltype(F)::value, decltype(Y)::value>(a, grid, L, extra, stream, drop_params(*b.dropout));
         return 0;
       });
     else
       dispatch_bool(b.y, [&](auto Y) {
-        ln_bwd_branch_launch<decltype(N)::value, decltype(F)::value, decltype(Y)::value>(a, grid, stream);
+        ln_bwd_branch_launch<decltype(N)::value, decltype(F)::value, decltype(Y)::value>(a, grid, L, extra, stream);
         return 0;
       });
   });
   return check_launch("layernorm_bwd_branch");
+}
+
+extern "C" int memhip_layernorm_bwd_branch(const memhip_ln_bwd_branch_args_t* args, memhip_stream_t stream) {
+  return layernorm_bwd_branch_launch(args, nullptr, 0, stream);
+}
+
+extern "C" int memhip_layernorm_bwd_branch_tasks(const memhip_ln_bwd_branch_args_t* args, const memhip_row_task_t* tasks, int ntasks,
+                                                 memhip_stream_t stream) {
+  RowTaskList L;
+  int extra = 0;
+  if (const int rc = row_tasks_gather("layernorm_bwd_branch_tasks", tasks, ntasks, &L, &extra)) return rc;
+  if (ntasks > 0 && opt(OPT_ROW_TASKS)) return layernorm_bwd_branch_launch(args, &L, extra, stream);
+  if (const int rc = layernorm_bwd_branch_launch(args, nullptr, 0, stream)) return rc;
+  return row_tasks_standalone(L, stream);
 }
 
 extern "C" int memhip_layerscale_grad(const void* W_bf16, int64_t ldw, const float* dW, int64_t lddw, const float* bias,
diff --git a/mem_amd/ops.py b/mem_amd/ops.py
--- a/mem_amd/ops.py
+++ b/mem_amd/ops.py
@@ -62,7 +62,19 @@
     _fields_ = [("count", i32), ("l", NtLaunch * 2)]
 
 
+class RowTask(C.Structure):
+    _fields_ = [("kind", i32), ("nblocks", i32), ("src", vp), ("dst", vp), ("vec", vp), ("acc", vp), ("clear", vp), ("n", i64),
+                ("ld", i64), ("count", i32), ("reserved0", i32)]
+
+
+ROW_TASK_COPY_SAMPLES, ROW_TASK_ZERO, ROW_TASK_COLSUM_FOLD, ROW_TASK_GEMV_ACC = range(4)
+ROW_TASKS_MAX = 4
+
+
 declare({"memhip_gemm_bf16_nt": (i32, [C.POINTER(GemmArgs), vp]),
+         "memhip_row_task_blocks": (i32, [C.POINTER(RowTask)]),
+         "memhip_layernorm_fwd_tasks": (i32, [vp, i64, vp, i32, i32, vp, vp, f32, vp, i64, vp, vp, C.POINTER(RowTask), i32, vp]),
+         "memhip_layernorm_bwd_branch_tasks": (i32, [C.POINTER(LnBwdBranchArgs), C.POINTER(RowTask), i32, vp]),
          "memhip_branch_bwd": (i32, [C.POINTER(BranchBwdArgs), vp]),
          "memhip_layernorm_bwd_branch": (i32, [C.POINTER(LnBwdBranchArgs), vp]),
          "memhip_attn_bwd": (i32, [C.POINTER(AttnBwdArgs), vp]),
@@ -180,7 +192,40 @@
     check(lib.memhip_dropout_rows_f32(C.byref(d), ptr(x), x.stride(0), rows, D, stream_ptr()), "dropout_rows_f32")
 
 
-def layernorm_fwd(x, gamma, beta, y, mean, rstd, R, D, eps=1e-6, row_idx=None):
+def _row_task(kind, src=None, dst=None, vec=None, acc=None, clear=None, n=0, ld=0, count=0):
+    t = RowTask(kind, 0, _p(src), _p(dst), _p(vec), _p(acc), _p(clear), n, ld, count, 0)
+    t.nblocks = lib.memhip_row_task_blocks(C.byref(t))
+    if t.nblocks <= 0:
+        check(-1, "row_task_blocks")
+    return t
+
+
+def task_copy_samples(src, dst, ids_i32, n, n_per_sample):
+    return _row_task(ROW_TASK_COPY_SAMPLES, src=src, dst=dst, vec=ids_i32, n=n_per_sample, count=n)
+
+
+def task_zero(t):
+    assert t.is_contiguous()
+    return _row_task(ROW_TASK_ZERO, dst=t, n=t.numel() * t.element_size())
+
+
+def task_colsum_fold(ws, copies, N, out):
+    return _row_task(ROW_TASK_COLSUM_FOLD, dst=ws, acc=out, n=N, count=copies)
+
+
+def task_gemv_acc(W, N, K, x, y, x_acc=None, zero=None):
+    return _row_task(ROW_TASK_GEMV_ACC, src=W, dst=y, vec=x, acc=x_acc, clear=zero, n=K, ld=W.stride(0), count=N)
+
+
+def _task_array(tasks):
+    return (RowTask * len(tasks))(*tasks)
+
+
+def layernorm_fwd(x, gamma, beta, y, mean, rstd, R, D, eps=1e-6, row_idx=None, tasks=None):
+    if tasks:
+        check(lib.memhip_layernorm_fwd_tasks(ptr(x), x.stride(0), ptr(row_idx), R, D, ptr(gamma), ptr(beta), eps, ptr(y), y.stride(0),
+                                             ptr(mean), ptr(rstd), _task_array(tasks), len(tasks), stream_ptr()), "layernorm_fwd_tasks")
+        return
     check(lib.memhip_layernorm_fwd(ptr(x), x.stride(0), ptr(row_idx), R, D, ptr(gamma), ptr(beta), eps,
                                    ptr(y), y.stride(0), ptr(mean), ptr(rstd), stream_ptr()), "layernorm_fwd")
 
@@ -197,10 +242,14 @@
 
 
 def layernorm_bwd_branch(dy, x, gamma, mean, rstd, dres, dgamma, dbeta, R, D, y_b, gamma_b, dy_b, dgamma_b, dbias_b,
-                         rowmask=None, keep_prob=1.0, rows_per_sample=1, in_map=None, out_map=None, dropout=None):
+                         rowmask=None, keep_prob=1.0, rows_per_sample=1, in_map=None, out_map=None, dropout=None, tasks=None):
     a = LnBwdBranchArgs(_p(dy), dy.stride(0), _p(x), x.stride(0), R, D, _p(gamma), _p(mean), _p(rstd), _p(dres), dres.stride(0),
                         _p(dgamma), _p(dbeta), _p(in_map),
                         _branch(y_b, gamma_b, rowmask, keep_prob, rows_per_sample, dy_b, dgamma_b, dbias_b, out_map, dropout))
+    if tasks:
+        check(lib.memhip_layernorm_bwd_branch_tasks(C.byref(a), _task_array(tasks), len(tasks), stream_ptr()),
+              "layernorm_bwd_branch_tasks")
+        return
     check(lib.memhip_layernorm_bwd_branch(C.byref(a), stream_ptr()), "layernorm_bwd_branch")
 
 
diff --git a/mem_amd/vit_engine.py b/mem_amd/vit_engine.py
--- a/mem_amd/vit_engine.py
+++ b/mem_amd/vit_engine.py
@@ -3,7 +3,7 @@
 
 import torch
 
-from . import ops
+from . import _lib, ops
 
 ALIGN = 1024
 
@@ -186,6 +186,7 @@
         self._tdesc = None
         self.set_gelu_dg(True)
         self.fuse_ln_branch = True
+        self._row_tasks = True
         self.gn_ws = torch.zeros(1024, dtype=torch.float64, device=dev)
         self.gnorm = torch.zeros(1, dtype=torch.float32, device=dev)
         self.loss_acc = torch.zeros(2, dtype=torch.float32, device=dev)
@@ -410,10 +411,13 @@
             return None
         return ops.dropout_params(key[0], key[1], site, self.drop_rate, row0)
 
-    def _copy_dropped(self, plan, j, src, dst, B):
+    def _copy_dropped(self, plan, j, src, dst, B, ride=False):
         nd = B - plan["n"][j]
         if nd > 0:
+            if ride:
+                return [ops.task_copy_samples(src, dst, plan["drop"][j], nd, self.T * self.D)]
             ops.copy_samples(src, dst, plan["drop"][j], nd, self.T * self.D)
+        return None
 
     def forward(self, x, mask_u8, rows_idx, labels=None, dp_masks=None, all_tokens=False, labels_event=None):
         assert x.is_cuda and x.dtype == torch.float32 and x.is_contiguous()
@@ -471,13 +475,14 @@
         g1 = self.P(pre + "gamma_1") if (pre + "gamma_1") in self.segs else None
         g2 = self.P(pre + "gamma_2") if (pre + "gamma_2") in self.segs else None
         tail = self.cur["tail"] if (i == self.depth - 1 and b0 == 0 and b1 == B) else None
+        ride = None
         if ba.smap is not None:
-            self._copy_dropped(plan, 2 * i, xin, xmid, B)
+            ride = self._copy_dropped(plan, 2 * i, xin, xmid, B, ride=self._row_tasks and ba.n > 0)
         if ba.n > 0:
             rs = slice(r0, r1) if ba.smap is None else slice(None)
             h1, qkv, ao = a["h1"][rs], a["qkv"][rs], a["ao"][rs]
             ops.layernorm_fwd(xin, self.P(pre + "norm1.weight"), self.P(pre + "norm1.bias"), h1, a["mean1"][r0:r1],
-                              a["rstd1"][r0:r1], ba.rows, D, row_idx=ba.ridx)
+                              a["rstd1"][r0:r1], ba.rows, D, row_idx=ba.ridx, tasks=ride)
             ops.gemm_nt(h1, self.W16(pre + "attn.qkv.weight", 3 * D, D), ba.gemm_rows, 3 * D, D, ops.EPI_BIAS_BF16,
                         out0=qkv, bias=self.P(pre + "attn.qkvbias3"), colscale=self.scale, colscale_n=D)
             ops.attn_fwd(qkv, ba.n, T, D, self.heads, self.table(i), self.window, ao, a["lse"][b0:b1])
@@ -489,13 +494,14 @@
         if tail is not None:
             self._mlp_fwd_tail(i, a, xs[2 * i + 1], g2, bm.keep_prob, tail)
             return
+        ride = None
         if bm.smap is not None:
-            self._copy_dropped(plan, 2 * i + 1, xmid, xout, B)
+            ride = self._copy_dropped(plan, 2 * i + 1, xmid, xout, B, ride=self._row_tasks and bm.n > 0)
         if bm.n > 0:
             rs = slice(r0, r1) if bm.smap is None else slice(None)
             h2, hpre, aa = a["h2"][rs], a["hpre"][rs], a["a"][rs]
             ops.layernorm_fwd(xmid, self.P(pre + "norm2.weight"), self.P(pre + "norm2.bias"), h2, a["mean2"][r0:r1],
-                              a["rstd2"][r0:r1], bm.rows, D, row_idx=bm.ridx)
+                              a["rstd2"][r0:r1], bm.rows, D, row_idx=bm.ridx, tasks=ride)
             ops.gemm_nt(h2, self.W16(pre + "mlp.fc1.weight", Hd, D), bm.gemm_rows, Hd, D, self.epi_gelu, out0=hpre,
                         out1=aa, bias=self.P(pre + "mlp.fc1.bias"))
             dm = self._drop(2 * i + 1, r0)
@@ -531,6 +537,7 @@
         assert tuple(x.shape[1:]) == (self.C, self.H, self.W), \
             f"Input image size ({x.shape[2]}*{x.shape[3]}) doesn't match model ({self.H}*{self.W})."
         self.ensure_batch(B, self.Mm_cap, keep=keep)
+        self._row_tasks = _lib.get_option("row_tasks") != 0
         if self.weights_dirty:
             self.sync_weights()
         if self.fwd_two_streams:
@@ -814,6 +821,8 @@
         self._bucket_ready(0)
         ops.zero_(self.bias_scr)
         fuse = D <= 1024 and self.fuse_ln_branch
+        ride = fuse and _lib.get_option("row_tasks") == 2
+        pad_zeroed = False
         self._inject_dmap(self.depth - 1)
         for i in reversed(range(self.depth)):
             pre = f"blocks.{i}."
@@ -835,13 +844,17 @@
                 if bm.n == 0 and not self.accumulate_grads:
                     self._zero_grad_of(pre + "mlp.fc1.weight")
                     self._zero_grad_of(pre + "mlp.fc2.weight")
+                tasks2 = []
                 if bm.n > 0:
                     self._before_overwrite("dbig")
-                    if bm.gemm_rows > bm.rows:
+                    if bm.gemm_rows > bm.rows and not pad_zeroed:
                         ops.zero_(dY[bm.rows:bm.gemm_rows])
                     ops.gemm_nt(dY, self.wT[i]["fc2"], bm.gemm_rows, Hd, D, self.epi_dgelu, out0=self.dbig, aux=a["hpre"],
                                 colsum=self.cs_ws, colsum_copies=self.CS_COPIES)
-                    ops.colsum_fold(self.cs_ws, self.CS_COPIES, Hd, self.G(pre + "mlp.fc1.bias"))
+                    if ride:
+                        tasks2.append(ops.task_colsum_fold(self.cs_ws, self.CS_COPIES, Hd, self.G(pre + "mlp.fc1.bias")))
+                    else:
+                        ops.colsum_fold(self.cs_ws, self.CS_COPIES, Hd, self.G(pre + "mlp.fc1.bias"))
                     self._on_side(lambda: self._wg_mlp(pre, a, has_g, bm.rows, dY))
                     ops.gemm_nt(self.dbig, self.wT[i]["fc1"], bm.gemm_rows, D, Hd, ops.EPI_BIAS_BF16, out0=self.dh_small)
                 if fuse:
@@ -850,7 +863,7 @@
                                              self.G(pre + "norm2.weight"), self.G(pre + "norm2.bias"), M, D, None,
                                              self.P(pre + "gamma_1") if has_g else None, dY2, None, scr,
                                              rowmask=ba.rowmask, keep_prob=ba.keep_prob, rows_per_sample=T,
-                                             in_map=bm.cmap, out_map=ba.cmap, dropout=self._drop(2 * i))
+                                             in_map=bm.cmap, out_map=ba.cmap, dropout=self._drop(2 * i), tasks=tasks2)
                 else:
                     if bm.n > 0:
                         ops.layernorm_bwd(self.dh_small, xmid, self.P(pre + "norm2.weight"), a["mean2"], a["rstd2"], dx,
@@ -862,8 +875,11 @@
                 self._zero_grad_of(pre + "attn.qkv.weight")
             if ba.n > 0:
                 ops.gemm_nt(dY2, self.wT[i]["proj"], ba.gemm_rows, D, D, ops.EPI_BIAS_BF16, out0=self.dao)
-            ops.gemv_acc(self.wT[i]["proj"], D, D, scr, self.G(pre + "attn.v_bias"),
-                         x_acc=self.G(pre + "attn.proj.bias"), zero=self.bias_scr[(i & 1) ^ 1])
+            gemv = (self.wT[i]["proj"], D, D, scr, self.G(pre + "attn.v_bias"))
+            gemv_kw = dict(x_acc=self.G(pre + "attn.proj.bias"), zero=self.bias_scr[(i & 1) ^ 1])
+            gemv_rides = ride and i > 0 and not has_g
+            if not gemv_rides:
+                ops.gemv_acc(*gemv, **gemv_kw)
             if ba.n > 0:
                 def wg_proj(grouped=False):
                     if not grouped:
@@ -892,14 +908,20 @@
                 ops.gemm_nt(self.dqkv, self.wT[i]["qkv"], ba.gemm_rows, D, 3 * D, ops.EPI_BIAS_BF16, out0=self.dh_small)
             if i > 0:
                 self._inject_dmap(i - 1)
+            pad_zeroed = False
             if fuse and i > 0:
                 pb, bb = f"blocks.{i - 1}.", br[2 * i - 1]
                 self._before_overwrite("dY")
+                tasks1 = [ops.task_gemv_acc(*gemv, **gemv_kw)] if gemv_rides else []
+                if ride and bb.n > 0 and bb.gemm_rows > bb.rows:
+                    tasks1.append(ops.task_zero(dY[bb.rows:bb.gemm_rows]))
+                    pad_zeroed = True
                 ops.layernorm_bwd_branch(self.dh_small, xin, self.P(pre + "norm1.weight"), a["mean1"], a["rstd1"], dx,
                                          self.G(pre + "norm1.weight"), self.G(pre + "norm1.bias"), M, D, None,
                                          self.P(pb + "gamma_2") if (pb + "gamma_2") in self.segs else None, dY, None,
                                          self.G(pb + "mlp.fc2.bias"), rowmask=bb.rowmask, keep_prob=bb.keep_prob,
-                                         rows_per_sample=T, in_map=ba.cmap, out_map=bb.cmap, dropout=self._drop(2 * i - 1))
+                                         rows_per_sample=T, in_map=ba.cmap, out_map=bb.cmap, dropout=self._drop(2 * i - 1),
+                                         tasks=tasks1)
             elif ba.n > 0:
                 ops.layernorm_bwd(self.dh_small, xin, self.P(pre + "norm1.weight"), a["mean1"], a["rstd1"], dx,
                                   self.G(pre + "norm1.weight"), self.G(pre + "norm1.bias"), ba.rows, D, accumulate=True,
```

Result: no change. 7563 (-0.0%).
